# pfnet-research/superpixel-align

Hardware: AMD Instinct MI355X
Metric: images/sec superpixel-align labelling (1024x2048) (higher is better)
Workload: dtype f32 as 2 x f16 planes, f32 accumulate

## Files before the change

include/spalign.h:

```cpp
#ifndef SPALIGN_H
#define SPALIGN_H

#include <stddef.h>
#include <stdint.h>

#ifdef __cplusplus
extern "C" {
#endif

#define SPA_OK 0
#define SPA_ERR_ARG (-1)
#define SPA_ERR_HIP (-2)
#define SPA_ERR_NOGPU (-3)
#define SPA_ERR_LAYOUT (-4)
#define SPA_ERR_CAPACITY (-5)

#define SPA_ST_SLIC_EMPTY_SEGMENT 0x01u
#define SPA_ST_SLIC_UNCOVERED 0x02u
#define SPA_ST_CONN_OVERSIZE 0x04u
#define SPA_ST_POOL_SLOT_OVERFLOW 0x08u
#define SPA_ST_KMEANS_BARRIER 0x10u
#define SPA_ST_LABEL_RANGE 0x20u
#define SPA_ST_RNG_UNDERRUN 0x40u
#define SPA_ST_NP_SHUFFLE 0x80u

#define SPA_CELL_SLOTS 16

typedef struct spa_ctx spa_ctx;

int spa_version(void);
const char *spa_last_error(void);
int spa_ctx_create(int device, spa_ctx **out);
void spa_ctx_destroy(spa_ctx *ctx);
int spa_status(spa_ctx *ctx, uint32_t *status_host, void *stream);
int spa_status_peek_async(spa_ctx *ctx, uint32_t *status_pinned, void *stream);
int spa_status_take_async(spa_ctx *ctx, uint32_t *status_pinned, void *stream);

int spa_prof_enable(spa_ctx *ctx, int on);
int spa_prof_slots(void);
const char *spa_prof_name(int slot);
int spa_prof_read(spa_ctx *ctx, int slot, double *total_ms_host, int *launches_host);
int spa_debug_peek(spa_ctx *ctx, int which, size_t offset, size_t bytes, void *host);
int spa_ws_generation(spa_ctx *ctx);
int spa_debug_set(spa_ctx *ctx, int32_t key, int32_t value);
int spa_wino4_tile_decode(int32_t B, int32_t H, int32_t W, int32_t dilation, int32_t interleaved, int64_t t, int32_t *out);
int spa_debug_lds_probe(spa_ctx *ctx, float *out, int32_t n_wg, int32_t steps, int32_t mode, void *stream);

int spa_drn_normalise(spa_ctx *ctx, const float *x, int32_t B, int32_t H, int32_t W, void *out,
                      int32_t out_dtype, const double *mean3_host, const double *std3_host, void *stream);
int spa_bias_act(spa_ctx *ctx, void *y, int32_t dtype, int64_t rows, int32_t C, const void *bias,
                 const void *residual, int32_t relu, void *stream);
int spa_bias_act_amax(spa_ctx *ctx, float *y, int64_t rows, int32_t C, const float *bias,
                      const float *residual, int32_t relu, void *amax, void *stream);

int spa_drn_stem_d(spa_ctx *ctx, const float *x, int32_t B, int32_t H, int32_t W,
                   const float *w0, const float *b0, const float *w1, const float *b1,
                   const double *mean3_host, const double *std3_host, void *y, int32_t out_dtype,
                   float *xn_scratch, void *stream);

int spa_conv3x3_bf16(spa_ctx *ctx, const void *x, int32_t B, int32_t H, int32_t W, int32_t Cin,
                     const void *wt, int32_t Cout, const float *bias, const void *residual,
                     int32_t relu, int32_t dilation, void *y, void *stream);

int spa_conv_bf16_light(spa_ctx *ctx, const void *x, int32_t B, int32_t Hi, int32_t Wi, int32_t Cin, const void *wt,
                        int32_t taps, int32_t stride, int32_t Cout, const float *bias, const void *residual,
                        int32_t relu, int32_t dilation, void *y, void *stream);

int spa_conv3x3_f32(spa_ctx *ctx, const float *x, int32_t B, int32_t H, int32_t W, int32_t Cin,
                    const float *wt, int32_t Cout, const float *bias, const float *residual,
                    int32_t relu, int32_t dilation, float *y, void *stream);
int spa_conv1x1_f32(spa_ctx *ctx, const float *x, int32_t B, int32_t H, int32_t W, int32_t Cin,
                    const float *wt, int32_t Cout, const float *bias, const float *residual,
                    int32_t relu, float *y, void *stream);

int64_t spa_wino_tiles(int32_t B, int32_t H, int32_t W, int32_t dilation);
int spa_conv3x3_wino_f32(spa_ctx *ctx, const float *x, int32_t B, int32_t H, int32_t W, int32_t Cin,
                         const float *u, int32_t Cout, const float *bias, const float *residual,
                         int32_t relu, int32_t dilation, float *v_scratch, float *m_scratch, float *y,
                         void *stream);

int64_t spa_wino4_tiles(int32_t B, int32_t H, int32_t W, int32_t dilation);
int spa_conv3x3_wino4_f32(spa_ctx *ctx, const float *x, int32_t B, int32_t H, int32_t W, int32_t Cin,
                          const float *u, int32_t Cout, const float *bias, const float *residual,
                          int32_t relu, int32_t dilation, float *v_scratch, float *m_scratch, float *y,
                          void *stream);

int spa_amax_f32(spa_ctx *ctx, const float *x, int64_t n, void *amax, void *stream);
int spa_conv3x3_wino4_f16s(spa_ctx *ctx, const float *x, int32_t B, int32_t H, int32_t W, int32_t Cin,
                           const void *u2, const float *cs, int32_t Cout, const float *bias, const float *residual,
                           int32_t relu, int32_t dilation, const void *amax_in, void *amax_out, void *v_scratch,
                           float *m_scratch, float *y, void *stream);

int spa_conv3x3_f16s(spa_ctx *ctx, const float *x, int32_t B, int32_t H, int32_t W, int32_t Cin,
                     const void *wt2, float inv_t, int32_t Cout, const float *bias, const float *residual,
                     int32_t relu, int32_t dilation, const void *amax_in, void *amax_out, float *y, void *stream);
int spa_conv1x1_f16s(spa_ctx *ctx, const float *x, int32_t B, int32_t H, int32_t W, int32_t Cin,
                     const void *wt2, float inv_t, int32_t Cout, const float *bias, const float *residual,
                     int32_t relu, const void *amax_in, void *amax_out, float *y, void *stream);

int spa_conv3x3_s2_f16s(spa_ctx *ctx, const float *x, int32_t B, int32_t Hi, int32_t Wi, int32_t Cin,
                        const void *wt2, float inv_t, int32_t Cout, int32_t csplit, const float *bias,
                        int32_t relu, const void *amax_in, void *amax_out, float *y, float *y2, void *stream);
int spa_conv3x3_s2_f32(spa_ctx *ctx, const float *x, int32_t B, int32_t Hi, int32_t Wi, int32_t Cin,
                       const float *wt, int32_t Cout, int32_t csplit, const float *bias,
                       int32_t relu, float *y, float *y2, void *stream);

int spa_drn_stem_d_amax(spa_ctx *ctx, const float *x, int32_t B, int32_t H, int32_t W,
                        const float *w0, const float *b0, const float *w1, const float *b1,
                        const double *mean3_host, const double *std3_host, float *y,
                        float *xn_scratch, void *amax_out, void *stream);
int spa_drn_stem_c_amax(spa_ctx *ctx, const float *x, int32_t B, int32_t H, int32_t W,
                        const float *w0, const float *b0, const float *w1, const float *b1,
                        const double *mean3_host, const double *std3_host, float *y, float *y0,
                        float *xn_scratch, void *amax_out, void *stream);
int spa_drn_stem_c_bf16(spa_ctx *ctx, const float *x, int32_t B, int32_t H, int32_t W,
                        const float *w0, const float *b0, const float *w1, const float *b1,
                        const double *mean3_host, const double *std3_host, void *y, void *y0,
                        float *xn_scratch, void *stream);
int spa_conv_small_f16s(spa_ctx *ctx, const float *x, int32_t B, int32_t H, int32_t W, int32_t Cin, const void *wp,
                        float inv_t, int32_t Cout, int32_t stride, int32_t n_proj, const float *bias,
                        const float *residual, int32_t relu, const void *amax_in, void *amax_out, float *y, float *y2,
                        void *stream);
int spa_drn_layer2_f16s(spa_ctx *ctx, const float *x, int32_t B, int32_t H, int32_t W, const void *wp, float inv_t,
                        const float *bias, const void *amax_in, void *amax_out, float *y, void *stream);
int spa_drn_layer2_f32(spa_ctx *ctx, const float *x, int32_t B, int32_t H, int32_t W, const float *w9,
                       const float *bias, float *y, void *stream);

int spa_resize_bicubic_u8(spa_ctx *ctx, const uint8_t *src, int32_t B, int32_t H, int32_t W, int32_t C,
                          int32_t dst_h, int32_t dst_w, float *out, void *stream);
int spa_resize_cvcubic_u8(spa_ctx *ctx, const uint8_t *src, int32_t B, int32_t H, int32_t W, int32_t C,
                          int32_t dst_h, int32_t dst_w, float *out, void *stream);


typedef struct {
    int32_t n_centroids;
    int32_t grid_ny, grid_nx;
    int32_t start_y, start_x;
    int32_t step_y, step_x;
    int32_t win_step_y, win_step_x;
    float step;
    int32_t min_size, max_size;
    int32_t max_labels;
} spa_slic_plan;
int spa_slic_make_plan(int32_t H, int32_t W, int32_t n_segments, spa_slic_plan *plan_host);

int spa_rgb2lab(spa_ctx *ctx, const float *rgb, int32_t B, int32_t H, int32_t W,
                float ratio, float *lab, void *stream);

int spa_slic_core(spa_ctx *ctx, const float *lab, int32_t B, int32_t H, int32_t W,
                  int32_t n_segments, int32_t max_iter, int32_t *labels, float *centres,
                  void *stream);

int spa_enforce_connectivity(spa_ctx *ctx, const int32_t *labels_in, int32_t B, int32_t H,
                             int32_t W, int32_t min_size, int32_t max_size,
                             int32_t *labels_out, int32_t *n_labels, void *stream);

int spa_rgb2lab_u8_f64(spa_ctx *ctx, const float *rgb, int32_t B, int32_t H, int32_t W, double ratio,
                       double *lab, void *stream);
int spa_slic_core_f64(spa_ctx *ctx, const double *lab, int32_t B, int32_t H, int32_t W,
                      int32_t n_segments, int32_t max_iter, int32_t *labels, double *centres,
                      void *stream);
int spa_slic_u8(spa_ctx *ctx, const float *rgb, int32_t B, int32_t H, int32_t W, int32_t n_segments,
                double compactness, int32_t max_iter, int32_t *labels, int32_t *n_labels, void *stream);

int spa_slic(spa_ctx *ctx, const float *rgb, int32_t B, int32_t H, int32_t W,
             int32_t n_segments, float compactness, int32_t max_iter,
             int32_t *labels, int32_t *n_labels, void *stream);

int spa_felzenszwalb(spa_ctx *ctx, const float *rgb, int32_t B, int32_t H, int32_t W,
                     double scale, double sigma, int32_t min_size, int32_t *labels,
                     int32_t *n_labels, void *stream);

int spa_felzenszwalb_u8(spa_ctx *ctx, const float *rgb, int32_t B, int32_t H, int32_t W,
                        double scale, double sigma, int32_t min_size, int32_t *labels,
                        int32_t *n_labels, void *stream);


int spa_segment_offsets(spa_ctx *ctx, const int32_t *n_labels, int32_t B, int32_t *offsets,
                        void *stream);

int spa_segment_stats(spa_ctx *ctx, const int32_t *labels, int32_t B, int32_t H, int32_t W,
                      const int32_t *offsets, int32_t Ncap,
                      double y_rel_pos, double x_rel_pos, double y_rel_sigma, double x_rel_sigma,
                      int32_t *count, double *centroid, double *prior, void *stream);

typedef struct spa_pyrandom spa_pyrandom;
int spa_pyrandom_create(uint64_t seed, spa_pyrandom **out);
void spa_pyrandom_destroy(spa_pyrandom *rng);
int spa_pyrandom_shuffle_select_host(spa_pyrandom *rng, const int32_t *count_host, int32_t N,
                                     int32_t n_anchors, int32_t *ranks_host,
                                     int32_t *n_valid_host);
typedef struct spa_nprandom spa_nprandom;
int spa_nprandom_create(uint32_t seed, spa_nprandom **out);
void spa_nprandom_destroy(spa_nprandom *rng);
int spa_nprandom_shuffle_host(spa_nprandom *rng, int64_t *a_host, int64_t n);
int spa_nprandom_state(spa_nprandom *rng, uint32_t *state628_host);
int spa_nprandom_set_state(spa_nprandom *rng, const uint32_t *state628_host);
int spa_np_kmeans_init_dev(spa_ctx *ctx, void *state_dev, const double *w, const int32_t *n_ptr, int32_t Ncap,
                           int32_t k, const int32_t *gate, int64_t *init_other, int32_t *m_out, void *stream);
int spa_kmeans_retry_update(spa_ctx *ctx, const int32_t *assign, const int32_t *offsets, int32_t B, const int32_t *gate,
                            int32_t *pending, int32_t *made, uint8_t *fail_out, void *stream);

int spa_pyrandom_dev_seed(spa_ctx *ctx, uint64_t seed, void *stream);
int spa_pyrandom_dev_generate(spa_ctx *ctx, int64_t want, void *stream);
int spa_anchor_ranks_dev(spa_ctx *ctx, const int32_t *count, const int32_t *n_ptr, int32_t Ncap,
                         int32_t n_anchors, int64_t total_pixels, int32_t *ranks, int32_t *n_valid,
                         void *stream);

int spa_select_anchor_pixels(spa_ctx *ctx, const int32_t *labels, int32_t B, int32_t H,
                             int32_t W, const int32_t *offsets, int32_t Ncap,
                             const int32_t *ranks, const int32_t *n_valid, int32_t n_anchors,
                             int32_t *anchors, void *stream);

typedef struct {
    int32_t C, fh, fw;
    int64_t stride_b, stride_c, stride_y, stride_x;
    int32_t dtype;
} spa_fmap_desc;


int spa_pool_anchor(spa_ctx *ctx, const void *fmap, const spa_fmap_desc *desc,
                    int32_t B, int32_t img_h, const int32_t *offsets, int32_t Ncap,
                    const int32_t *anchors, const int32_t *n_valid, int32_t n_anchors,
                    int32_t n_neighbors, const double *centroid, int32_t append_pos,
                    void *X, int32_t x_dtype, int64_t ld, void *stream);

int spa_pool_mean(spa_ctx *ctx, const void *fmap, const spa_fmap_desc *desc,
                  const int32_t *labels, int32_t B, int32_t H, int32_t W,
                  const int32_t *offsets, int32_t Ncap, const int32_t *count,
                  int32_t sampling, const double *centroid, int32_t append_pos,
                  void *X, int32_t x_dtype, int64_t ld, void *stream);

int spa_kmeans_weighted(spa_ctx *ctx, const void *X, int32_t x_dtype, int64_t ld, int32_t D,
                        const double *w, const int32_t *n_ptr, int32_t Ncap, int32_t k,
                        int32_t max_iter, const int64_t *init_other, int32_t *assign,
                        int32_t *info, void *stream);
int spa_kmeans_weighted_gated(spa_ctx *ctx, const void *X, int32_t x_dtype, int64_t ld, int32_t D,
                              const double *w, const int32_t *n_ptr, int32_t Ncap, int32_t k,
                              int32_t max_iter, const int64_t *init_other, const int32_t *gate, int32_t *assign,
                              int32_t *info, void *stream);

int spa_paint(spa_ctx *ctx, const int32_t *labels, const int32_t *assign,
              const int32_t *offsets, int32_t B, int32_t H, int32_t W,
              uint8_t *cluster, uint8_t *road, void *stream);
// ... 129 lines not shown
```

superpixel-align_amd/_lib.py:

```python
import ctypes
import os
import subprocess

_HERE = os.path.dirname(os.path.abspath(__file__))
LIB_PATH = os.environ.get('SPA_LIB_PATH') or os.path.join(_HERE, 'libspalign.so')
_LIB = None

SPA_OK = 0
STATUS_BITS = {
    0x01: 'SLIC: a seed lost all of its pixels (NaN centre, dead for the rest of the sweeps, as in scikit-image)',
    0x02: 'SLIC: a pixel fell outside every 2S search window',
    0x04: 'connectivity: a component reached max_size (cut in BFS order by the exact replay path)',
    0x08: 'mean pooling: more than 16 superpixels touch one feature pixel',
    0x10: 'k-means: grid barrier timed out',
    0x20: 'a superpixel label outside [0, n_labels) was met',
    0x40: 'anchor selection: the device random stream ran dry',
    0x80: 'k-means initial assignment on the device: more than 65 536 points at or below the median weight',
}

INFO_BITS = 0x01 | 0x04

c_i32 = ctypes.c_int32
c_i64 = ctypes.c_int64
c_f32 = ctypes.c_float
c_f64 = ctypes.c_double
c_p = ctypes.c_void_p


class SlicPlan(ctypes.Structure):
    _fields_ = [('n_centroids', c_i32), ('grid_ny', c_i32), ('grid_nx', c_i32),
                ('start_y', c_i32), ('start_x', c_i32), ('step_y', c_i32), ('step_x', c_i32),
                ('win_step_y', c_i32), ('win_step_x', c_i32), ('step', c_f32),
                ('min_size', c_i32), ('max_size', c_i32), ('max_labels', c_i32)]


class FmapDesc(ctypes.Structure):
    _fields_ = [('C', c_i32), ('fh', c_i32), ('fw', c_i32),
                ('stride_b', c_i64), ('stride_c', c_i64), ('stride_y', c_i64), ('stride_x', c_i64),
                ('dtype', c_i32)]


PROTOTYPES = {
    'spa_version': (ctypes.c_int, []),
    'spa_last_error': (ctypes.c_char_p, []),
    'spa_ctx_create': (ctypes.c_int, [ctypes.c_int, ctypes.POINTER(c_p)]),
    'spa_ctx_destroy': (None, [c_p]),
    'spa_status': (ctypes.c_int, [c_p, ctypes.POINTER(ctypes.c_uint32), c_p]),
    'spa_status_peek_async': (ctypes.c_int, [c_p, c_p, c_p]),
    'spa_status_take_async': (ctypes.c_int, [c_p, c_p, c_p]),
    'spa_prof_enable': (ctypes.c_int, [c_p, ctypes.c_int]),
    'spa_prof_slots': (ctypes.c_int, []),
    'spa_prof_name': (ctypes.c_char_p, [ctypes.c_int]),
    'spa_prof_read': (ctypes.c_int, [c_p, ctypes.c_int, ctypes.POINTER(c_f64),
                                     ctypes.POINTER(ctypes.c_int)]),
    'spa_drn_normalise': (ctypes.c_int, [c_p, c_p, c_i32, c_i32, c_i32, c_p, c_i32, c_p, c_p, c_p]),
    'spa_bias_act': (ctypes.c_int, [c_p, c_p, c_i32, c_i64, c_i32, c_p, c_p, c_i32, c_p]),
    'spa_drn_stem_d': (ctypes.c_int, [c_p, c_p, c_i32, c_i32, c_i32, c_p, c_p, c_p, c_p, c_p, c_p, c_p, c_i32, c_p, c_p]),
    'spa_conv3x3_bf16': (ctypes.c_int, [c_p, c_p, c_i32, c_i32, c_i32, c_i32, c_p, c_i32, c_p, c_p, c_i32, c_i32, c_p, c_p]),
    'spa_conv_bf16_light': (ctypes.c_int, [c_p, c_p, c_i32, c_i32, c_i32, c_i32, c_p, c_i32, c_i32, c_i32, c_p, c_p, c_i32, c_i32, c_p, c_p]),
    'spa_conv3x3_f32': (ctypes.c_int, [c_p, c_p, c_i32, c_i32, c_i32, c_i32, c_p, c_i32, c_p, c_p, c_i32, c_i32, c_p, c_p]),
    'spa_conv1x1_f32': (ctypes.c_int, [c_p, c_p, c_i32, c_i32, c_i32, c_i32, c_p, c_i32, c_p, c_p, c_i32, c_p, c_p]),
    'spa_wino_tiles': (ctypes.c_int64, [c_i32, c_i32, c_i32, c_i32]),
    'spa_conv3x3_wino_f32': (ctypes.c_int, [c_p, c_p, c_i32, c_i32, c_i32, c_i32, c_p, c_i32, c_p, c_p, c_i32, c_i32, c_p, c_p, c_p, c_p]),
    'spa_wino4_tiles': (ctypes.c_int64, [c_i32, c_i32, c_i32, c_i32]),
    'spa_conv3x3_wino4_f32': (ctypes.c_int, [c_p, c_p, c_i32, c_i32, c_i32, c_i32, c_p, c_i32, c_p, c_p, c_i32, c_i32, c_p, c_p, c_p, c_p]),
    'spa_conv3x3_f16s': (ctypes.c_int, [c_p, c_p, c_i32, c_i32, c_i32, c_i32, c_p, c_f32, c_i32, c_p, c_p, c_i32, c_i32, c_p, c_p, c_p, c_p]),
    'spa_conv1x1_f16s': (ctypes.c_int, [c_p, c_p, c_i32, c_i32, c_i32, c_i32, c_p, c_f32, c_i32, c_p, c_p, c_i32, c_p, c_p, c_p, c_p]),
    'spa_conv3x3_s2_f16s': (ctypes.c_int, [c_p, c_p, c_i32, c_i32, c_i32, c_i32, c_p, c_f32, c_i32, c_i32, c_p, c_i32, c_p, c_p, c_p, c_p, c_p]),
    'spa_bias_act_amax': (ctypes.c_int, [c_p, c_p, c_i64, c_i32, c_p, c_p, c_i32, c_p, c_p]),
    'spa_drn_stem_d_amax': (ctypes.c_int, [c_p, c_p, c_i32, c_i32, c_i32, c_p, c_p, c_p, c_p, c_p, c_p, c_p, c_p, c_p, c_p]),
    'spa_drn_stem_c_amax': (ctypes.c_int, [c_p, c_p, c_i32, c_i32, c_i32, c_p, c_p, c_p, c_p, c_p, c_p, c_p, c_p, c_p, c_p, c_p]),
    'spa_drn_stem_c_bf16': (ctypes.c_int, [c_p, c_p, c_i32, c_i32, c_i32, c_p, c_p, c_p, c_p, c_p, c_p, c_p, c_p, c_p, c_p]),
    'spa_conv_small_f16s': (ctypes.c_int, [c_p, c_p, c_i32, c_i32, c_i32, c_i32, c_p, c_f32, c_i32, c_i32, c_i32, c_p, c_p, c_i32, c_p, c_p, c_p, c_p, c_p]),
    'spa_drn_layer2_f16s': (ctypes.c_int, [c_p, c_p, c_i32, c_i32, c_i32, c_p, c_f32, c_p, c_p, c_p, c_p, c_p]),
    'spa_drn_layer2_f32': (ctypes.c_int, [c_p, c_p, c_i32, c_i32, c_i32, c_p, c_p, c_p, c_p]),
    'spa_conv3x3_s2_f32': (ctypes.c_int, [c_p, c_p, c_i32, c_i32, c_i32, c_i32, c_p, c_i32, c_i32, c_p, c_i32, c_p, c_p, c_p]),
    'spa_amax_f32': (ctypes.c_int, [c_p, c_p, c_i64, c_p, c_p]),
    'spa_conv3x3_wino4_f16s': (ctypes.c_int, [c_p, c_p, c_i32, c_i32, c_i32, c_i32, c_p, c_p, c_i32, c_p, c_p, c_i32, c_i32, c_p, c_p, c_p, c_p, c_p, c_p]),
    'spa_resize_bicubic_u8': (ctypes.c_int, [c_p, c_p, c_i32, c_i32, c_i32, c_i32, c_i32, c_i32, c_p, c_p]),
    'spa_resize_cvcubic_u8': (ctypes.c_int, [c_p, c_p, c_i32, c_i32, c_i32, c_i32, c_i32, c_i32, c_p, c_p]),
    'spa_debug_peek': (ctypes.c_int, [c_p, ctypes.c_int, ctypes.c_size_t, ctypes.c_size_t, c_p]),
    'spa_debug_set': (ctypes.c_int, [c_p, ctypes.c_int32, ctypes.c_int32]),
    'spa_wino4_tile_decode': (ctypes.c_int, [c_i32, c_i32, c_i32, c_i32, c_i32, c_i64, ctypes.POINTER(ctypes.c_int32)]),
    'spa_ws_generation': (ctypes.c_int, [c_p]),
    'spa_debug_lds_probe': (ctypes.c_int, [c_p, c_p, c_i32, c_i32, c_i32, c_p]),
    'spa_slic_make_plan':(ctypes.c_int, [c_i32, c_i32, c_i32, ctypes.POINTER(SlicPlan)]),
    'spa_rgb2lab': (ctypes.c_int, [c_p, c_p, c_i32, c_i32, c_i32, c_f32, c_p, c_p]),
    'spa_slic_core': (ctypes.c_int, [c_p, c_p, c_i32, c_i32, c_i32, c_i32, c_i32, c_p, c_p, c_p]),
    'spa_enforce_connectivity': (ctypes.c_int, [c_p, c_p, c_i32, c_i32, c_i32, c_i32, c_i32, c_p,
                                                c_p, c_p]),
    'spa_slic': (ctypes.c_int, [c_p, c_p, c_i32, c_i32, c_i32, c_i32, c_f32, c_i32, c_p, c_p, c_p]),
    'spa_felzenszwalb': (ctypes.c_int, [c_p, c_p, c_i32, c_i32, c_i32, c_f64, c_f64, c_i32, c_p, c_p, c_p]),
    'spa_rgb2lab_u8_f64': (ctypes.c_int, [c_p, c_p, c_i32, c_i32, c_i32, c_f64, c_p, c_p]),
    'spa_slic_core_f64': (ctypes.c_int, [c_p, c_p, c_i32, c_i32, c_i32, c_i32, c_i32, c_p, c_p, c_p]),
    'spa_slic_u8': (ctypes.c_int, [c_p, c_p, c_i32, c_i32, c_i32, c_i32, c_f64, c_i32, c_p, c_p, c_p]),
    'spa_felzenszwalb_u8': (ctypes.c_int, [c_p, c_p, c_i32, c_i32, c_i32, c_f64, c_f64, c_i32, c_p, c_p, c_p]),
    'spa_overlap_refine': (ctypes.c_int, [c_p, c_p, c_p, c_i32, c_i64, c_i32, c_f64, c_p, c_p]),
    'spa_segment_offsets':(ctypes.c_int, [c_p, c_p, c_i32, c_p, c_p]),
    'spa_segment_stats': (ctypes.c_int, [c_p, c_p, c_i32, c_i32, c_i32, c_p, c_i32, c_f64, c_f64,
                                         c_f64, c_f64, c_p, c_p, c_p, c_p]),
    'spa_pyrandom_create': (ctypes.c_int, [ctypes.c_uint64, ctypes.POINTER(c_p)]),
    'spa_pyrandom_destroy': (None, [c_p]),
    'spa_pyrandom_shuffle_select_host': (ctypes.c_int, [c_p, c_p, c_i32, c_i32, c_p, c_p]),
    'spa_nprandom_create': (ctypes.c_int, [ctypes.c_uint32, ctypes.POINTER(c_p)]),
    'spa_nprandom_destroy': (None, [c_p]),
    'spa_nprandom_shuffle_host': (ctypes.c_int, [c_p, c_p, c_i64]),
    'spa_nprandom_state': (ctypes.c_int, [c_p, c_p]),
    'spa_nprandom_set_state': (ctypes.c_int, [c_p, c_p]),
    'spa_np_kmeans_init_dev': (ctypes.c_int, [c_p, c_p, c_p, c_p, c_i32, c_i32, c_p, c_p, c_p, c_p]),
    'spa_kmeans_retry_update': (ctypes.c_int, [c_p, c_p, c_p, c_i32, c_p, c_p, c_p, c_p, c_p]),
    'spa_pyrandom_dev_seed': (ctypes.c_int, [c_p, ctypes.c_uint64, c_p]),
    'spa_pyrandom_dev_generate': (ctypes.c_int, [c_p, c_i64, c_p]),
    'spa_anchor_ranks_dev': (ctypes.c_int, [c_p, c_p, c_p, c_i32, c_i32, c_i64, c_p, c_p, c_p]),
    'spa_select_anchor_pixels': (ctypes.c_int, [c_p, c_p, c_i32, c_i32, c_i32, c_p, c_i32, c_p, c_p,
                                                c_i32, c_p, c_p]),
    'spa_pool_anchor': (ctypes.c_int, [c_p, c_p, ctypes.POINTER(FmapDesc), c_i32, c_i32, c_p, c_i32,
                                       c_p, c_p, c_i32, c_i32, c_p, c_i32, c_p, c_i32, c_i64, c_p]),
    'spa_pool_mean': (ctypes.c_int, [c_p, c_p, ctypes.POINTER(FmapDesc), c_p, c_i32, c_i32, c_i32,
                                     c_p, c_i32, c_p, c_i32, c_p, c_i32, c_p, c_i32, c_i64, c_p]),
    'spa_kmeans_weighted': (ctypes.c_int, [c_p, c_p, c_i32, c_i64, c_i32, c_p, c_p, c_i32, c_i32,
                                           c_i32, c_p, c_p, c_p, c_p]),
    'spa_kmeans_weighted_gated': (ctypes.c_int, [c_p, c_p, c_i32, c_i64, c_i32, c_p, c_p, c_i32, c_i32,
                                                 c_i32, c_p, c_p, c_p, c_p, c_p]),
    'spa_paint': (ctypes.c_int, [c_p, c_p, c_p, c_p, c_i32, c_i32, c_i32, c_p, c_p, c_p]),
    'spa_confusion': (ctypes.c_int, [c_p, c_p, c_p, c_i32, c_i64, c_p, c_p]),
    'spa_png_deflate_u8': (ctypes.c_int, [c_p, c_p, c_i32, c_i32, c_i32, c_p, c_p, c_i32, c_i32, c_p, c_i64, c_p, c_p,
                                          c_p]),
    'spa_png_deflate_bound': (ctypes.c_int64, [c_i32, c_i32]),
    'spa_jpeg_encode_rgb8': (ctypes.c_int, [c_p, c_p, c_i32, c_i32, c_i32, c_i32, c_p, c_p, c_i64, c_p, c_p]),
    'spa_jpeg_scan_bound': (ctypes.c_int64, [c_i32, c_i32, c_i32]),
    'spa_figure_compose_u8': (ctypes.c_int, [c_p, c_p, c_i32, c_i32, c_i32, c_i32, c_p, c_p, c_p, c_i32, c_i32, c_i32, c_i32,
                                             c_p, c_i32, c_i32, c_p]),
    'spa_figure_canvas_shape': (ctypes.c_int, [c_i32, c_i32, c_i32, c_i32, c_i32, c_i32, ctypes.POINTER(c_i32),
                                               ctypes.POINTER(c_i32)]),
    'spa_segnet_encode': (ctypes.c_int, [c_p, c_p, c_i32, c_i32, c_i32, c_i32, c_i32, c_p, c_p, c_p, c_p, c_p, c_p, c_p]),
    'spa_segnet_decode': (ctypes.c_int, [c_p, c_p, c_p, c_i32, c_i32, c_i32, c_i32, c_p, c_p, c_p, c_p, c_p, c_p]),
    'spa_segnet_encode_bf16': (ctypes.c_int, [c_p, c_p, c_i32, c_i32, c_i32, c_i32, c_i32, c_p, c_p, c_p, c_p, c_p, c_p,
                                              c_p]),
    'spa_segnet_decode_bf16': (ctypes.c_int, [c_p, c_p, c_p, c_i32, c_i32, c_i32, c_i32, c_p, c_p, c_p, c_p, c_p, c_p]),
    'spa_segnet_encode_f16x3': (ctypes.c_int, [c_p, c_p, c_i32, c_i32, c_i32, c_i32, c_i32, c_p, c_p, c_p, c_p, c_p, c_p,
                                               c_p]),
    'spa_segnet_decode_f16x3': (ctypes.c_int, [c_p, c_p, c_p, c_i32, c_i32, c_i32, c_i32, c_p, c_p, c_p, c_p, c_p, c_p]),
    'spa_segnet_decode_logits': (ctypes.c_int, [c_p, c_p, c_p, c_i32, c_i32, c_i32, c_i32, c_p, c_p, c_p, c_p, c_p, c_p]),
    'spa_segnet_decode_logits_bf16': (ctypes.c_int, [c_p, c_p, c_p, c_i32, c_i32, c_i32, c_i32, c_p, c_p, c_p, c_p, c_p,
                                                     c_p]),
    'spa_segnet_decode_logits_f16x3': (ctypes.c_int, [c_p, c_p, c_p, c_i32, c_i32, c_i32, c_i32, c_p, c_p, c_p, c_p, c_p,
                                                      c_p]),
    'spa_segnet_overlay': (ctypes.c_int, [c_p, c_p, c_i32, c_i32, c_i32, c_i32, c_i32, c_p, c_p, c_f64, c_p, c_p, c_p]),
    'spa_segnet_score': (ctypes.c_int, [c_p, c_p, c_i32, c_i32, c_i32, c_i32, c_i32, c_p, c_p, c_p]),
    'spa_segnet_label_eval': (ctypes.c_int, [c_p, c_p, c_i32, c_i32, c_i32, c_i32, c_i32, c_p, c_p, c_p, c_p, c_p]),
    'spa_segnet_train_input': (ctypes.c_int, [c_p, c_p, c_i32, c_i32, c_i32, c_i32, c_i32, c_i32, c_p, c_p, c_i32, c_p,
                                              c_p, c_i32, c_p, c_p, c_p, c_p, c_p]),
    'spa_segnet_train_label': (ctypes.c_int, [c_p, c_p, c_i32, c_i32, c_i32, c_i32, c_i32, c_i32, c_i32, c_p, c_p, c_p,
                                              c_p, c_p]),
    'spa_segnet_train_input_ptrs': (ctypes.c_int, [c_p, c_p, c_i32, c_i32, c_i32, c_i32, c_i32, c_i32, c_p, c_p, c_i32,
                                                   c_p, c_p, c_i32, c_p, c_p, c_p, c_p, c_p]),
    'spa_segnet_train_label_ptrs': (ctypes.c_int, [c_p, c_p, c_i32, c_i32, c_i32, c_i32, c_i32, c_i32, c_i32, c_p, c_p,
                                                   c_p, c_p, c_p]),
    'spa_segnet_train_forward': (ctypes.c_int, [c_p, c_p, c_p, c_i32, c_i32, c_i32, c_i32, c_i32, c_p, c_p, c_p, c_p,
                                                c_p, c_p]),
    'spa_segnet_train_dgrad': (ctypes.c_int, [c_p, c_p, c_p, c_p, c_i32, c_i32, c_i32, c_p, c_p]),
    'spa_segnet_train_wgrad': (ctypes.c_int, [c_p, c_p, c_p, c_p, c_i32, c_i32, c_i32, c_i32, c_i32, c_p, c_p, c_p,
                                              c_p]),
    'spa_segnet_train_forward_bf16': (ctypes.c_int, [c_p, c_p, c_p, c_i32, c_i32, c_i32, c_i32, c_i32, c_p, c_p, c_p,
                                                     c_p, c_p, c_p]),
    'spa_segnet_train_dgrad_bf16': (ctypes.c_int, [c_p, c_p, c_p, c_p, c_i32, c_i32, c_i32, c_p, c_p]),
    'spa_segnet_train_wgrad_bf16': (ctypes.c_int, [c_p, c_p, c_p, c_p, c_i32, c_i32, c_i32, c_i32, c_i32, c_p, c_p,
                                                   c_p, c_p]),
    'spa_segnet_train_forward_f16x3': (ctypes.c_int, [c_p, c_p, c_p, c_i32, c_i32, c_i32, c_i32, c_i32, c_p, c_p, c_p,
                                                      c_p, c_p, c_p]),
    'spa_segnet_train_dgrad_f16x3': (ctypes.c_int, [c_p, c_p, c_p, c_p, c_i32, c_i32, c_i32, c_p, c_p]),
    'spa_segnet_train_wgrad_f16x3': (ctypes.c_int, [c_p, c_p, c_p, c_p, c_i32, c_i32, c_i32, c_i32, c_i32, c_p, c_p,
                                                    c_p, c_p]),
    'spa_segnet_train_bn_forward': (ctypes.c_int, [c_p, c_p, c_p, c_p, c_p, c_p, c_i32, c_i32, c_i32, c_p, c_p, c_p]),
    'spa_segnet_train_bn_backward_sums': (ctypes.c_int, [c_p, c_p, c_p, c_p, c_p, c_p, c_p, c_i32, c_i32, c_i32, c_p,
                                                         c_p]),
    'spa_segnet_train_bn_backward_dy': (ctypes.c_int, [c_p, c_p, c_p, c_p, c_p, c_p, c_p, c_p, c_p, c_f64, c_i32, c_i32,
                                                       c_i32, c_p, c_p]),
    'spa_segnet_train_classifier_forward': (ctypes.c_int, [c_p, c_p, c_p, c_p, c_i32, c_i32, c_i32, c_p, c_p]),
    'spa_segnet_train_classifier_backward': (ctypes.c_int, [c_p, c_p, c_p, c_p, c_i32, c_i32, c_i32, c_p, c_p, c_p,
                                                            c_p]),
}


class SpalignError(RuntimeError):
    pass


def build(force=False):
    csrc = os.path.join(_HERE, 'csrc')
    if force:
        subprocess.check_call(['make', '-s', '-C', csrc, 'clean'])
    subprocess.check_call(['make', '-s', '-j8', '-C', csrc])
    return LIB_PATH


def lib():
    global _LIB
    if _LIB is None:
        if not os.path.exists(LIB_PATH):
            raise SpalignError('%s is missing: run `python -c "import __graft_entry__ as g; '
                               'g.build()"` (there is no CPU fallback)' % LIB_PATH)
        import torch
        L = ctypes.CDLL(LIB_PATH)
        for name, (res, args) in PROTOTYPES.items():
            fn = getattr(L, name)
            fn.restype = res
            fn.argtypes = args
        _LIB = L
    return _LIB


def check(rc):
    if rc != SPA_OK:
        raise SpalignError('libspalign error %d: %s' % (rc, lib().spa_last_error().decode()))


def make_plan(H, W, n_segments):
    p = SlicPlan()
    check(lib().spa_slic_make_plan(H, W, n_segments, ctypes.byref(p)))
    return p
```

superpixel-align_amd/csrc/spa_common.h:

```cpp
#pragma once
#include <hip/hip_runtime.h>
#include <stdint.h>
#include <stdio.h>
#include <string.h>

#include "../../include/spalign.h"

#define SPA_WAVE 64

void spa_set_error(const char *fmt, ...);

#define SPA_HIP(call)                                                                  \
    do {                                                                               \
        hipError_t e_ = (call);                                                        \
        if (e_ != hipSuccess) {                                                        \
            spa_set_error("%s failed: %s (%s:%d)", #call, hipGetErrorString(e_),      \
                          __FILE__, __LINE__);                                         \
            return SPA_ERR_HIP;                                                        \
        }                                                                              \
    } while (0)

#define SPA_ARG(cond)                                                                  \
    do {                                                                               \
        if (!(cond)) {                                                                 \
            spa_set_error("invalid argument: %s (%s:%d)", #cond, __FILE__, __LINE__);  \
            return SPA_ERR_ARG;                                                        \
        }                                                                              \
    } while (0)

#define SPA_LAUNCH_CHECK()                                                             \
    do {                                                                               \
        hipError_t e_ = hipGetLastError();                                             \
        if (e_ != hipSuccess) {                                                        \
            spa_set_error("kernel launch failed: %s (%s:%d)", hipGetErrorString(e_),   \
                          __FILE__, __LINE__);                                         \
            return SPA_ERR_HIP;                                                        \
        }                                                                              \
    } while (0)

enum {
    WS_LAB = 0,
    WS_CENTRES,
    WS_PRE,
    WS_PARENT,
    WS_SIZE,
    WS_FINAL,
    WS_CLAIM,
    WS_QUEUE,
    WS_BLK,
    WS_SMALL,
    WS_CONNMISC,
    WS_BBOX,
    WS_CELLSLOT,
    WS_KM_PART,
    WS_KM_MISC,
    WS_NLABELS,
    WS_SBOX,
    WS_TODO,
    WS_ROWMASK,
    WS_FINEMASK,
    WS_SLIC_ORDER,
    WS_OVERLAP,
    WS_STEM_IN,
    WS_SRGB_LUT,
    WS_FZ_KEYS,
    WS_FZ_VALS,
    WS_FZ_STATE,
    WS_FZ_TMP,
    WS_STEM_WPACK,
    WS_ZERO_LINE,
    WS_RESIZE_TAB,
    WS_RESIZE_TMP,
    WS_RNG_STATE,
    WS_RNG_RING,
    WS_RNG_JBUF,
    WS_RNG_JOFF,
    WS_RUNS,
    WS_DEBUG,
    WS_SEGNET_BNPART,
    WS_SEGNET_WROT,
    WS_SEGNET_WGRAD,
    WS_SEGNET_WBF16,
    WS_SEGNET_WF16X3,
    WS_SEGNET_AMAX,
    WS_SEGNET_BNRED,
    WS_PNG_ROWS,
    WS_JPEG_INTERVALS,
    WS_COUNT
};

enum {
    PROF_RGB2LAB = 0, PROF_SLIC_ASSIGN, PROF_SLIC_UPDATE, PROF_CONNECT, PROF_STATS,
    PROF_CELL_WEIGHTS, PROF_POOL_MEAN, PROF_POOL_ANCHOR, PROF_KMEANS, PROF_PAINT,
    PROF_DRN_STEM, PROF_DRN_BIAS_ACT, PROF_DRN_CONV, PROF_DRN_CONV32, PROF_DRN_GEMM32, PROF_DRN_GEMM32_N, PROF_WINO_IN, PROF_WINO_OUT, PROF_DRN_GEMM16, PROF_DRN_GEMM16_N, PROF_DRN_CONV16, PROF_DRN_CONV16_128, PROF_DRN_CONV16_256, PROF_DRN_CONV16_1X1, PROF_DRN_CONV16_FRONT, PROF_DRN_CONV_LIGHT, PROF_SLOTS
};

struct spa_ctx {
    int device;
    int n_cu;
    uint32_t *d_status;
    unsigned status_takes;
    void *ws[WS_COUNT];
    size_t ws_bytes[WS_COUNT];
    int prof_on;
    hipEvent_t *prof_ev[PROF_SLOTS];
    int prof_cap[PROF_SLOTS], prof_used[PROF_SLOTS];
    hipStream_t aux[2];
    hipEvent_t ev_fork, ev_join[2];
    int aux_ready;
    int km_attr_done[2];
    int conn_attr_done;
    int conn_claim_ready;
    size_t conn_claim_bytes;
    int upd_wg_per_cu, upd_wg_per_cu8;
    int slic_force_general;
    int zero_line_ready, conv_attr_done, conv32_attr_done, fz_attr_done, gemm16_attr_done, gemm16s_attr_done, gemm16p_attr_done, nprng_attr_done;
    int rng_seeded;
    int ws_generation;
    int dbg_slic_ldsx;
    int convp_on;
    int wino_operands;
    int convs2_on;
    int convs2_attr_done;
    int rs_key[4], rs_ks[2];
};

#ifdef __HIPCC__
__device__ __forceinline__ unsigned spa_split16_pair(float x0, float x1, float sc, unsigned &l)
{
    unsigned h, lo;
    asm("v_fma_mixlo_f16 %0, %2, %4, 0 op_sel_hi:[0,0,0]\n\t"
        "v_fma_mixhi_f16 %0, %3, %4, 0 op_sel_hi:[0,0,0]\n\t"
        "v_fma_mixlo_f16 %1, %2, %4, -%0 op_sel_hi:[0,0,1]\n\t"
        "v_fma_mixhi_f16 %1, %3, %4, -%0 op_sel:[0,0,1] op_sel_hi:[0,0,1]"
        : "=&v"(h), "=&v"(lo) : "v"(x0), "v"(x1), "v"(sc));
    l = lo;
    return h;
}
#endif

int spa_aux_streams(spa_ctx *ctx);

void spa_prof_mark(spa_ctx *ctx, int slot, int end, hipStream_t s);
struct SpaProfScope {
    spa_ctx *c; int slot; hipStream_t s;
    SpaProfScope(spa_ctx *c_, int slot_, hipStream_t s_) : c(c_), slot(slot_), s(s_) { if (c->prof_on && slot >= 0) spa_prof_mark(c, slot, 0, s); }
    ~SpaProfScope() { if (c->prof_on && slot >= 0) spa_prof_mark(c, slot, 1, s); }
};

int spa_ws_reserve(spa_ctx *ctx, int which, size_t bytes, void **out);
void spa_zero_word(void *word, hipStream_t s);

static inline hipStream_t spa_stream(void *s) { return (hipStream_t)s; }

__device__ __forceinline__ double spa_det_log_pos(double x)
{
    unsigned long long b = (unsigned long long)__double_as_longlong(x);
    int e = (int)((b >> 52) & 0x7ff) - 1023;
    b = (b & 0x000fffffffffffffULL) | 0x3ff0000000000000ULL;
    double m = __longlong_as_double((long long)b);
    if (m > 1.4142135623730951) { m = m * 0.5; e += 1; }
    double s = (m - 1.0) / (m + 1.0);
    double z = s * s;
    double p = 1.0 / 25.0;
    p = p * z + 1.0 / 23.0;
    p = p * z + 1.0 / 21.0;
    p = p * z + 1.0 / 19.0;
    p = p * z + 1.0 / 17.0;
    p = p * z + 1.0 / 15.0;
    p = p * z + 1.0 / 13.0;
    p = p * z + 1.0 / 11.0;
    p = p * z + 1.0 / 9.0;
    p = p * z + 1.0 / 7.0;
    p = p * z + 1.0 / 5.0;
    p = p * z + 1.0 / 3.0;
    p = p * z + 1.0;
    double lnm = 2.0 * s * p;
    double ed = (double)e;
    return ed * 6.93147180369123816490e-01 + (ed * 1.90821492927058770002e-10 + lnm);
}

__device__ __forceinline__ double spa_det_exp(double t)
{
    double kf = floor(t * 1.44269504088896338700e+00 + 0.5);
    double r = (t - kf * 6.93147180369123816490e-01) - kf * 1.90821492927058770002e-10;
    double p = 1.0 / 87178291200.0;
    p = p * r + 1.0 / 6227020800.0;
    p = p * r + 1.0 / 479001600.0;
    p = p * r + 1.0 / 39916800.0;
    p = p * r + 1.0 / 3628800.0;
    p = p * r + 1.0 / 362880.0;
    p = p * r + 1.0 / 40320.0;
    p = p * r + 1.0 / 5040.0;
    p = p * r + 1.0 / 720.0;
    p = p * r + 1.0 / 120.0;
    p = p * r + 1.0 / 24.0;
    p = p * r + 1.0 / 6.0;
    p = p * r + 0.5;
    p = p * r + 1.0;
    p = p * r + 1.0;
    int k = (int)kf;
    unsigned long long b = (unsigned long long)(k + 1023) << 52;
    return p * __longlong_as_double((long long)b);
}

__device__ __forceinline__ unsigned spa_lane() { return __lane_id(); }
__device__ __forceinline__ unsigned spa_rank_in_mask(unsigned long long mask)
{
    return __builtin_amdgcn_mbcnt_hi((unsigned)(mask >> 32), __builtin_amdgcn_mbcnt_lo((unsigned)mask, 0u));
}
```

superpixel-align_amd/csrc/spa_conv32.hip:

```cpp
#include "spa_common.h"

typedef float f32x4 __attribute__((ext_vector_type(4)));
typedef float f32x8 __attribute__((ext_vector_type(8)));
typedef _Float16 f16x8 __attribute__((ext_vector_type(8)));

#define C32_BN 256
#define C32_BK 32
#define C32_THREADS 512
#define C32_TILE_BYTES (256 * C32_BK * 4)
#define C32_HALO 4
#define C32_XSEG_BYTES ((256 + 2 * C32_HALO) * C32_BK * 4)

template <int HAS_RES, int BM, int TAPS, int BN, bool SPLIT = false, int S = 1>
__global__ __launch_bounds__(C32_THREADS) void k_conv3x3_f32(const float *__restrict__ X, const float *__restrict__ Wt,
                                                             const float *__restrict__ bias,
                                                             const float *__restrict__ R, float *__restrict__ Y,
                                                             const char *__restrict__ zero_line, int B, int H, int W,
                                                             int Cin, int Cout, int dil, int relu, int xtiles,
                                                             int ntiles, int total_tiles, int zcount, long long xz,
                                                             long long wz, long long yz,
                                                             const unsigned *__restrict__ amax_in = nullptr,
                                                             unsigned *__restrict__ amax_out = nullptr, float inv_t = 1.f,
                                                             int Hi = 0, int Wi = 0, float *__restrict__ Y2 = nullptr, int csplit = 0)
{
// ... 349 lines not shown
        if (bm == 64 && bn == 256) {
            const int bit64 = TAPS == 9 ? 32 : 64;
            if (!(ctx->conv32_attr_done & bit64)) {
                SPA_HIP(hipFuncSetAttribute((const void *)k_conv3x3_f32<0, 64, TAPS, 256, true>, hipFuncAttributeMaxDynamicSharedMemorySize, 2 * 64 * 128 + 2 * (256 + 2 * C32_HALO) * 128));
                SPA_HIP(hipFuncSetAttribute((const void *)k_conv3x3_f32<1, 64, TAPS, 256, true>, hipFuncAttributeMaxDynamicSharedMemorySize, 2 * 64 * 128 + 2 * (256 + 2 * C32_HALO) * 128));
                ctx->conv32_attr_done |= bit64;
            }
            if (residual) C32_LAUNCH_S(1, 64, 256); else C32_LAUNCH_S(0, 64, 256);
            SPA_LAUNCH_CHECK();
            return SPA_OK;
        }
        SPA_ARG(bn == (bm == 256 ? 256 : 128));
        if (residual) { if (bm == 256) C32_LAUNCH_S(1, 256, 256); else if (bm == 128) C32_LAUNCH_S(1, 128, 128); else C32_LAUNCH_S(1, 64, 128); }
        else { if (bm == 256) C32_LAUNCH_S(0, 256, 256); else if (bm == 128) C32_LAUNCH_S(0, 128, 128); else C32_LAUNCH_S(0, 64, 128); }
        SPA_LAUNCH_CHECK();
        return SPA_OK;
    }
    if (residual) { if (bm == 256) C32_LAUNCH(1, 256, 256); else if (bm == 128) C32_LAUNCH(1, 128, 128); else C32_LAUNCH(1, 64, 128); }
    else { if (bm == 256) C32_LAUNCH(0, 256, 256); else if (bm == 128) C32_LAUNCH(0, 128, 128); else C32_LAUNCH(0, 64, 128); }
#undef C32_LAUNCH
    SPA_LAUNCH_CHECK();
    return SPA_OK;
}

extern "C" int spa_conv3x3_f32(spa_ctx *ctx, const float *x, int32_t B, int32_t H, int32_t W, int32_t Cin,
                               const float *wt, int32_t Cout, const float *bias, const float *residual,
                               int32_t relu, int32_t dilation, float *y, void *stream)
{
    return conv_f32_launch<9>(ctx, x, B, H, W, Cin, wt, Cout, bias, residual, relu, dilation, y, stream);
}

extern "C" int spa_conv1x1_f32(spa_ctx *ctx, const float *x, int32_t B, int32_t H, int32_t W, int32_t Cin,
                               const float *wt, int32_t Cout, const float *bias, const float *residual,
                               int32_t relu, float *y, void *stream)
{
    return conv_f32_launch<1>(ctx, x, B, H, W, Cin, wt, Cout, bias, residual, relu, 1, y, stream);
}

extern "C" int spa_conv3x3_f16s(spa_ctx *ctx, const float *x, int32_t B, int32_t H, int32_t W, int32_t Cin,
                                const void *wt2, float inv_t, int32_t Cout, const float *bias, const float *residual,
                                int32_t relu, int32_t dilation, const void *amax_in, void *amax_out, float *y, void *stream)
{
    SPA_ARG(amax_in);
    return conv_f32_launch<9>(ctx, x, B, H, W, Cin, (const float *)wt2, Cout, bias, residual, relu, dilation, y, stream, true, 1,
                              0, 0, 0, amax_in, amax_out, inv_t);
}

extern "C" int spa_conv1x1_f16s(spa_ctx *ctx, const float *x, int32_t B, int32_t H, int32_t W, int32_t Cin,
                                const void *wt2, float inv_t, int32_t Cout, const float *bias, const float *residual,
                                int32_t relu, const void *amax_in, void *amax_out, float *y, void *stream)
{
    SPA_ARG(amax_in);
    return conv_f32_launch<1>(ctx, x, B, H, W, Cin, (const float *)wt2, Cout, bias, residual, relu, 1, y, stream, true, 1,
                              0, 0, 0, amax_in, amax_out, inv_t);
}

bool conv3x3_s2_tile_takes(int32_t Cin, int32_t Cout, int32_t csplit, const float *y2);
int conv3x3_s2_tile_launch(spa_ctx *ctx, const float *x, int32_t B, int32_t Hi, int32_t Wi, int32_t Cin, const void *wt2, float inv_t,
                           int32_t csplit, const float *bias, int32_t relu, const void *amax_in, void *amax_out, float *y, float *y2,
                           hipStream_t s);

extern "C" int spa_conv3x3_s2_f16s(spa_ctx *ctx, const float *x, int32_t B, int32_t Hi, int32_t Wi, int32_t Cin,
                                   const void *wt2, float inv_t, int32_t Cout, int32_t csplit, const float *bias,
                                   int32_t relu, const void *amax_in, void *amax_out, float *y, float *y2, void *stream)
{
    SPA_ARG(ctx && x && wt2 && bias && y && amax_in && B > 0 && Hi > 0 && Wi > 0 && inv_t > 0.f);
    SPA_ARG(Cin % C32_BK == 0 && Cout % 128 == 0 && csplit % 64 == 0 && csplit > 0 && csplit <= Cout && (y2 || csplit == Cout));
    SPA_ARG(((uintptr_t)x % 16) == 0 && ((uintptr_t)wt2 % 16) == 0 && ((uintptr_t)y % 16) == 0 && ((uintptr_t)y2 % 16) == 0 && ((uintptr_t)bias % 16) == 0);
    hipStream_t s = spa_stream(stream);
    char *zero;
    int rc = spa_ws_reserve(ctx, WS_ZERO_LINE, 4096, (void **)&zero);
    if (rc != SPA_OK) return rc;
    if (!ctx->zero_line_ready) {
        SPA_HIP(hipMemsetAsync(zero, 0, 4096, s));
        ctx->zero_line_ready = 1;
    }
    if (amax_out) spa_zero_word(amax_out, s);
    if (ctx->convs2_on && conv3x3_s2_tile_takes(Cin, Cout, csplit, y2)) {
        SpaProfScope prof_(ctx, PROF_DRN_CONV16_FRONT, s);
        return conv3x3_s2_tile_launch(ctx, x, B, Hi, Wi, Cin, wt2, inv_t, csplit, bias, relu, amax_in, amax_out, y, y2, s);
    }
    const int H = (Hi + 1) / 2, W = (Wi + 1) / 2;
    const int bm = Cout % 256 == 0 ? 256 : 128, bn = 128;
    const int xtiles = (W + bn - 1) / bn, ntiles = Cout / bm;
    const long long total = (long long)B * H * xtiles * ntiles;
    SPA_ARG(total < (1ll << 31));
    SPA_ARG((long long)(2 * W + 1024) * Cin * 4 < (1ll << 31));
    const size_t lds = 2 * (size_t)bm * 128 + 2 * (size_t)(2 * bn + 2 * C32_HALO + 8) * 128;
    if (!(ctx->conv32_attr_done & 4)) {
        SPA_HIP(hipFuncSetAttribute((const void *)k_conv3x3_f32<0, 256, 9, 128, true, 2>, hipFuncAttributeMaxDynamicSharedMemorySize, 2 * 256 * 128 + 2 * (256 + 2 * C32_HALO + 8) * 128));
        SPA_HIP(hipFuncSetAttribute((const void *)k_conv3x3_f32<0, 128, 9, 128, true, 2>, hipFuncAttributeMaxDynamicSharedMemorySize, 2 * 128 * 128 + 2 * (256 + 2 * C32_HALO + 8) * 128));
        ctx->conv32_attr_done |= 4;
    }
    SpaProfScope prof_(ctx, PROF_DRN_CONV16_FRONT, s);
    const int per_cu = lds > 80 * 1024 ? 1 : (lds > 53 * 1024 ? 2 : 3);
    long long grid = (long long)ctx->n_cu * per_cu;
    if (grid > total) grid = total;
    if (bm == 256)
        hipLaunchKernelGGL((k_conv3x3_f32<0, 256, 9, 128, true, 2>), dim3((unsigned)grid), dim3(C32_THREADS), lds, s, x, (const float *)wt2, bias,
                           (const float *)nullptr, y, (const char *)zero, B, H, W, Cin, Cout, 1, relu, xtiles, ntiles, (int)total, 1, 0ll, 0ll, 0ll,
                           (const unsigned *)amax_in, (unsigned *)amax_out, inv_t, Hi, Wi, y2, csplit);
    else
        hipLaunchKernelGGL((k_conv3x3_f32<0, 128, 9, 128, true, 2>), dim3((unsigned)grid), dim3(C32_THREADS), lds, s, x, (const float *)wt2, bias,
                           (const float *)nullptr, y, (const char *)zero, B, H, W, Cin, Cout, 1, relu, xtiles, ntiles, (int)total, 1, 0ll, 0ll, 0ll,
                           (const unsigned *)amax_in, (unsigned *)amax_out, inv_t, Hi, Wi, y2, csplit);
    SPA_LAUNCH_CHECK();
    return SPA_OK;
}

extern "C" int spa_conv3x3_s2_f32(spa_ctx *ctx, const float *x, int32_t B, int32_t Hi, int32_t Wi, int32_t Cin,
                                  const float *wt, int32_t Cout, int32_t csplit, const float *bias,
                                  int32_t relu, float *y, float *y2, void *stream)
{
    SPA_ARG(ctx && x && wt && bias && y && B > 0 && Hi > 0 && Wi > 0);
    SPA_ARG(Cin % C32_BK == 0 && Cout % 128 == 0 && csplit % 64 == 0 && csplit > 0 && csplit <= Cout && (y2 || csplit == Cout));
    SPA_ARG(((uintptr_t)x % 16) == 0 && ((uintptr_t)wt % 16) == 0 && ((uintptr_t)y % 16) == 0 && ((uintptr_t)y2 % 16) == 0 && ((uintptr_t)bias % 16) == 0);
    hipStream_t s = spa_stream(stream);
    char *zero;
    int rc = spa_ws_reserve(ctx, WS_ZERO_LINE, 4096, (void **)&zero);
    if (rc != SPA_OK) return rc;
    if (!ctx->zero_line_ready) {
        SPA_HIP(hipMemsetAsync(zero, 0, 4096, s));
        ctx->zero_line_ready = 1;
    }
    const int H = (Hi + 1) / 2, W = (Wi + 1) / 2;
    const int bm = Cout % 256 == 0 ? 256 : 128, bn = 128;
    const int xtiles = (W + bn - 1) / bn, ntiles = Cout / bm;
    const long long total = (long long)B * H * xtiles * ntiles;
    SPA_ARG(total < (1ll << 31));
    SPA_ARG((long long)(2 * W + 1024) * Cin * 4 < (1ll << 31));
    const size_t lds = 2 * (size_t)bm * 128 + 2 * (size_t)(2 * bn + 2 * C32_HALO) * 128;
    if (!(ctx->conv32_attr_done & 128)) {
        SPA_HIP(hipFuncSetAttribute((const void *)k_conv3x3_f32<0, 256, 9, 128, false, 2>, hipFuncAttributeMaxDynamicSharedMemorySize, 2 * 256 * 128 + 2 * (256 + 2 * C32_HALO) * 128));
        SPA_HIP(hipFuncSetAttribute((const void *)k_conv3x3_f32<0, 128, 9, 128, false, 2>, hipFuncAttributeMaxDynamicSharedMemorySize, 2 * 128 * 128 + 2 * (256 + 2 * C32_HALO) * 128));
        ctx->conv32_attr_done |= 128;
    }
    SpaProfScope prof_(ctx, PROF_DRN_CONV32, s);
    const int per_cu = lds > 80 * 1024 ? 1 : (lds > 53 * 1024 ? 2 : 3);
    long long grid = (long long)ctx->n_cu * per_cu;
    if (grid > total) grid = total;
    if (bm == 256)
        hipLaunchKernelGGL((k_conv3x3_f32<0, 256, 9, 128, false, 2>), dim3((unsigned)grid), dim3(C32_THREADS), lds, s, x, wt, bias,
                           (const float *)nullptr, y, (const char *)zero, B, H, W, Cin, Cout, 1, relu, xtiles, ntiles, (int)total, 1, 0ll, 0ll, 0ll,
                           (const unsigned *)nullptr, (unsigned *)nullptr, 1.f, Hi, Wi, y2, csplit);
    else
        hipLaunchKernelGGL((k_conv3x3_f32<0, 128, 9, 128, false, 2>), dim3((unsigned)grid), dim3(C32_THREADS), lds, s, x, wt, bias,
                           (const float *)nullptr, y, (const char *)zero, B, H, W, Cin, Cout, 1, relu, xtiles, ntiles, (int)total, 1, 0ll, 0ll, 0ll,
                           (const unsigned *)nullptr, (unsigned *)nullptr, 1.f, Hi, Wi, y2, csplit);
    SPA_LAUNCH_CHECK();
    return SPA_OK;
}

int conv1x1_f32_raw(spa_ctx *ctx, const float *x, long long rows, int32_t Cin, const float *wt, int32_t Cout,
                    float *y, void *stream, int zcount)
{
    SPA_ARG(rows > 0 && rows % 256 == 0 && rows / 256 < (1ll << 31) && zcount >= 1);
    return conv_f32_launch<1>(ctx, x, 1, (int32_t)(rows / 256), 256, Cin, wt, Cout, nullptr, nullptr, 0, 1, y, stream, true,
                              zcount, rows * Cin, (long long)Cout * Cin, rows * Cout);
}
```

superpixel-align_amd/csrc/spa_ctx.hip:

```cpp
#include <math.h>
#include <stdarg.h>
#include <stdlib.h>

#include "spa_common.h"

static thread_local char g_err[512] = "";

void spa_set_error(const char *fmt, ...)
{
    va_list ap;
    va_start(ap, fmt);
    vsnprintf(g_err, sizeof(g_err), fmt, ap);
    va_end(ap);
}

extern "C" const char *spa_last_error(void) { return g_err; }
extern "C" int spa_version(void) { return 100; }

extern "C" int spa_ctx_create(int device, spa_ctx **out)
{
    SPA_ARG(out != nullptr);
    int n = 0;
    if (hipGetDeviceCount(&n) != hipSuccess || n <= 0) {
        spa_set_error("no HIP device visible: libspalign has no CPU fallback");
        return SPA_ERR_NOGPU;
    }
    if (device < 0) SPA_HIP(hipGetDevice(&device));
    SPA_ARG(device < n);
    SPA_HIP(hipSetDevice(device));
    hipDeviceProp_t prop;
    SPA_HIP(hipGetDeviceProperties(&prop, device));
    if (strncmp(prop.gcnArchName, "gfx950", 6) != 0) {
        spa_set_error("device %d is %s; libspalign is built for gfx950 (MI355X) only", device,
                      prop.gcnArchName);
        return SPA_ERR_NOGPU;
    }
    spa_ctx *ctx = (spa_ctx *)calloc(1, sizeof(spa_ctx));
    ctx->device = device;
    ctx->n_cu = prop.multiProcessorCount;
    if (const char *e = getenv("SPA_SLIC_GENERAL")) ctx->slic_force_general = atoi(e) != 0;
    ctx->convp_on = getenv("SPA_CONVP") ? atoi(getenv("SPA_CONVP")) != 0 : 1;
    ctx->convs2_on = 1;
    ctx->wino_operands = 2;
    SPA_HIP(hipMalloc((void **)&ctx->d_status, 32 * sizeof(uint32_t)));
    SPA_HIP(hipMemset(ctx->d_status, 0, 32 * sizeof(uint32_t)));
    *out = ctx;
    return SPA_OK;
}

extern "C" void spa_ctx_destroy(spa_ctx *ctx)
{
    if (!ctx) return;
    for (int i = 0; i < PROF_SLOTS; ++i) {
        for (int j = 0; j < ctx->prof_cap[i]; ++j) (void)hipEventDestroy(ctx->prof_ev[i][j]);
        free(ctx->prof_ev[i]);
    }
    for (int i = 0; i < WS_COUNT; ++i)
        if (ctx->ws[i]) (void)hipFree(ctx->ws[i]);
    if (ctx->d_status) (void)hipFree(ctx->d_status);
    if (ctx->aux_ready) {
        for (int i = 0; i < 2; ++i) { (void)hipStreamDestroy(ctx->aux[i]); (void)hipEventDestroy(ctx->ev_join[i]); }
        (void)hipEventDestroy(ctx->ev_fork);
    }
    free(ctx);
}

__global__ void k_zero_word(unsigned *w) { *w = 0u; }
void spa_zero_word(void *word, hipStream_t s) { hipLaunchKernelGGL(k_zero_word, dim3(1), dim3(1), 0, s, (unsigned *)word); }

int spa_ws_reserve(spa_ctx *ctx, int which, size_t bytes, void **out)
{
    if (bytes == 0) bytes = 16;
    if (ctx->ws_bytes[which] < bytes) {
        SPA_HIP(hipDeviceSynchronize());
        if (ctx->ws[which]) SPA_HIP(hipFree(ctx->ws[which]));
        ctx->ws[which] = nullptr;
        ctx->ws_bytes[which] = 0;
        size_t want = bytes + bytes / 8;
        SPA_HIP(hipMalloc(&ctx->ws[which], want));
        ctx->ws_bytes[which] = want;
        ++ctx->ws_generation;
    }
    *out = ctx->ws[which];
    return SPA_OK;
}

extern "C" int spa_status(spa_ctx *ctx, uint32_t *status_host, void *stream)
{
    SPA_ARG(ctx && status_host);
    hipStream_t s = spa_stream(stream);
    SPA_HIP(hipMemcpyAsync(status_host, ctx->d_status, sizeof(uint32_t), hipMemcpyDeviceToHost, s));
    SPA_HIP(hipMemsetAsync(ctx->d_status, 0, sizeof(uint32_t), s));
    SPA_HIP(hipStreamSynchronize(s));
    return SPA_OK;
}

extern "C" int spa_status_peek_async(spa_ctx *ctx, uint32_t *status_pinned, void *stream)
{
    SPA_ARG(ctx && status_pinned);
    SPA_HIP(hipMemcpyAsync(status_pinned, ctx->d_status, sizeof(uint32_t), hipMemcpyDeviceToHost, spa_stream(stream)));
    return SPA_OK;
}

__global__ void k_status_take(uint32_t *status, uint32_t *taken) { *taken = atomicExch(status, 0u); }

extern "C" int spa_status_take_async(spa_ctx *ctx, uint32_t *status_pinned, void *stream)
{
    SPA_ARG(ctx && status_pinned);
    uint32_t *slot = ctx->d_status + 16 + (ctx->status_takes++ & 15);
    hipLaunchKernelGGL(k_status_take, dim3(1), dim3(1), 0, spa_stream(stream), ctx->d_status, slot);
    SPA_HIP(hipMemcpyAsync(status_pinned, slot, sizeof(uint32_t), hipMemcpyDeviceToHost, spa_stream(stream)));
    return SPA_OK;
}

static int regular_grid_1hw(int64_t H, int64_t W, int64_t n_points, int64_t start[3],
                            int64_t step[3], int has_step[3])
{
    int64_t shape[3] = {1, H, W};
    int order[3] = {0, 1, 2};
    for (int i = 1; i < 3; ++i) {
        int o = order[i], j = i - 1;
        while (j >= 0 && shape[order[j]] > shape[o]) { order[j + 1] = order[j]; --j; }
        order[j + 1] = o;
    }
    double sorted[3];
    for (int i = 0; i < 3; ++i) sorted[i] = (double)shape[order[i]];
    double space = (double)H * (double)W;
    if (space <= (double)n_points) {
        for (int i = 0; i < 3; ++i) { start[i] = 0; step[i] = 1; has_step[i] = 0; }
        return 0;
    }
    double ss[3];
    ss[0] = ss[1] = ss[2] = pow(space / (double)n_points, 1.0 / 3.0);
    bool small = false;
    for (int i = 0; i < 3; ++i) small = small || (sorted[i] < ss[i]);
    if (small) {
        for (int dim = 0; dim < 3; ++dim) {
            ss[dim] = sorted[dim];
            double sp = 1.0;
            for (int j = dim + 1; j < 3; ++j) sp *= sorted[j];
            if (dim == 2) return -1;
            double v = pow(sp / (double)n_points, 1.0 / (double)(2 - dim));
            for (int j = dim + 1; j < 3; ++j) ss[j] = v;
            bool ok = true;
            for (int j = 0; j < 3; ++j) ok = ok && (sorted[j] >= ss[j]);
            if (ok) break;
        }
    }
    for (int p = 0; p < 3; ++p) {
        int d = order[p];
        start[d] = (int64_t)floor(ss[p] / 2.0);
        step[d] = (int64_t)nearbyint(ss[p]);
        has_step[d] = 1;
    }
    return 0;
}

static int64_t range_len(int64_t n, int64_t start, int64_t step)
{
    return start >= n ? 0 : (n - start + step - 1) / step;
}

extern "C" int spa_slic_make_plan(int32_t H, int32_t W, int32_t n_segments, spa_slic_plan *plan)
{
    SPA_ARG(plan && H > 0 && W > 0 && n_segments > 0);
    int64_t st[3], sp[3];
    int has[3];
    if (regular_grid_1hw(H, W, n_segments, st, sp, has) != 0) {
        spa_set_error("n_segments=%d too large for a %dx%d image", n_segments, H, W);
        return SPA_ERR_ARG;
    }
    int64_t ny = range_len(H, st[1], sp[1]), nx = range_len(W, st[2], sp[2]);
    SPA_ARG(ny > 0 && nx > 0);
    int64_t n = ny * nx;
    plan->n_centroids = (int32_t)n;
    plan->grid_ny = (int32_t)ny;
    plan->grid_nx = (int32_t)nx;
    plan->start_y = (int32_t)st[1];
    plan->start_x = (int32_t)st[2];
    plan->step_y = (int32_t)sp[1];
    plan->step_x = (int32_t)sp[2];
    double stmax = 1.0;
    if (has[1] && (double)sp[1] > stmax) stmax = (double)sp[1];
    if (has[2] && (double)sp[2] > stmax) stmax = (double)sp[2];
    plan->step = (float)stmax;
    int64_t st2[3], sp2[3];
    int has2[3];
    if (regular_grid_1hw(H, W, n, st2, sp2, has2) != 0) return SPA_ERR_ARG;
    plan->win_step_y = has2[1] ? (int32_t)sp2[1] : 1;
    plan->win_step_x = has2[2] ? (int32_t)sp2[2] : 1;
    double seg = ((double)H * (double)W) / (double)n;
    plan->min_size = (int32_t)(0.5 * seg);
    plan->max_size = (int32_t)(3.0 * seg);
    int64_t ml = plan->min_size > 0 ? ((int64_t)H * W) / plan->min_size + 1 : (int64_t)H * W;
    if (ml > (int64_t)H * W) ml = (int64_t)H * W;
    plan->max_labels = (int32_t)ml;
    return SPA_OK;
}

void spa_prof_mark(spa_ctx *ctx, int slot, int end, hipStream_t s)
{
    int idx = ctx->prof_used[slot] * 2 + end;
    if (idx >= ctx->prof_cap[slot]) {
        int ncap = ctx->prof_cap[slot] ? ctx->prof_cap[slot] * 2 : 256;
        ctx->prof_ev[slot] = (hipEvent_t *)realloc(ctx->prof_ev[slot], (size_t)ncap * sizeof(hipEvent_t));
        for (int j = ctx->prof_cap[slot]; j < ncap; ++j) (void)hipEventCreate(&ctx->prof_ev[slot][j]);
        ctx->prof_cap[slot] = ncap;
    }
    (void)hipEventRecord(ctx->prof_ev[slot][idx], s);
    if (end) ctx->prof_used[slot] += 1;
}

extern "C" int spa_prof_enable(spa_ctx *ctx, int on)
{
    SPA_ARG(ctx);
    ctx->prof_on = on ? 1 : 0;
    for (int i = 0; i < PROF_SLOTS; ++i) ctx->prof_used[i] = 0;
    return SPA_OK;
}

extern "C" int spa_prof_slots(void) { return PROF_SLOTS; }

extern "C" const char *spa_prof_name(int slot)
{
    static const char *names[PROF_SLOTS] = {"k_rgb2lab", "k_slic_assign", "k_slic_update",
        "connectivity(all)", "segment_stats(all)", "k_cell_weights", "k_pool_mean", "k_pool_anchor",
        "k_kmeans", "k_paint", "k_drn_stem_d(+normalise)", "k_bias_act(all)", "k_conv3x3_bf16(all)", "k_conv3x3_f32<taps 9>(all)", "k_conv3x3_f32<0, 256, 1, 256>", "k_conv3x3_f32<taps 1, narrow tiles>(all)", "k_wino_in", "k_wino_out", "k_gemm_f16x3_stag<256, 256>", "k_gemm_f16x3<128, 128>", "k_conv3x3_p16<64, 256> (split planes, 64-channel layers)", "k_conv3x3_p16<128, 128> (split planes, 128-channel layers)", "k_conv3x3_f32<split, 256-channel tile>", "k_conv3x3_f32<split, 1x1>", "split-plane front (stride-2 openers + projections, layer 2, DRN-C layers 1-2)", "k_conv_bf16_light(all)"};
    return (slot >= 0 && slot < PROF_SLOTS) ? names[slot] : "";
}

extern "C" int spa_prof_read(spa_ctx *ctx, int slot, double *total_ms, int *launches)
{
    SPA_ARG(ctx && total_ms && launches && slot >= 0 && slot < PROF_SLOTS);
    SPA_HIP(hipDeviceSynchronize());
    double t = 0.0;
    for (int j = 0; j < ctx->prof_used[slot]; ++j) {
        float ms = 0.0f;
        SPA_HIP(hipEventElapsedTime(&ms, ctx->prof_ev[slot][2 * j], ctx->prof_ev[slot][2 * j + 1]));
        t += ms;
    }
    *total_ms = t;
    *launches = ctx->prof_used[slot];
    return SPA_OK;
}

int spa_aux_streams(spa_ctx *ctx)
{
    if (ctx->aux_ready) return SPA_OK;
    int prio_lo = 0, prio_hi = 0;
    SPA_HIP(hipDeviceGetStreamPriorityRange(&prio_lo, &prio_hi));
    for (int i = 0; i < 2; ++i) {
        SPA_HIP(hipStreamCreateWithPriority(&ctx->aux[i], hipStreamNonBlocking, i == 1 ? prio_hi : prio_lo));
        SPA_HIP(hipEventCreateWithFlags(&ctx->ev_join[i], hipEventDisableTiming));
    }
    SPA_HIP(hipEventCreateWithFlags(&ctx->ev_fork, hipEventDisableTiming));
    ctx->aux_ready = 1;
    return SPA_OK;
}


typedef float dbg_f32x2 __attribute__((ext_vector_type(2)));
__global__ __launch_bounds__(256) void k_debug_lds_probe(float *__restrict__ out, int steps, int mode, float seed)
{
    __shared__ __attribute__((aligned(16))) float tab[32 * 32];
    __shared__ uint4 other[256 * 3];
    const int tid = threadIdx.x;
    other[tid * 3] = make_uint4(tid, blockIdx.x, 0u, 0u);
    for (int e = tid; e < steps * 32; e += 256) {
        const float t = seed * (float)(blockIdx.x % 977) - (float)(e & 31) * 1.25f - (float)(e >> 5);
        tab[e] = ((e * 7 + (int)blockIdx.x) % 11 == 0) ? INFINITY : t * t;
    }
    __syncthreads();
    dbg_f32x2 acc0 = {0.0f, 0.0f}, acc1 = {0.0f, 0.0f};
    float best[4] = {INFINITY, INFINITY, INFINITY, INFINITY};
    int bl[4] = {-1, -1, -1, -1};
    const float fy = (float)(tid >> 3);
#pragma unroll 1
    for (int jj = 0; jj < steps; ++jj) {
        const uint4 e0 = other[(jj * 3) % 768];
        const float *q = tab + jj * 32 + (mode == 2 ? 0 : (tid & 7) * 4);
        float4 d;
        if (mode == 1) { d.x = ((const volatile float *)q)[0]; d.y = ((const volatile float *)q)[1]; d.z = ((const volatile float *)q)[2]; d.w = ((const volatile float *)q)[3]; }
        else d = *(const float4 *)q;
        const float ty = (float)(e0.x & 31u) - fy;
        const float dy = (jj & 3) == 3 ? INFINITY : ty * ty;
        const dbg_f32x2 p0 = (dbg_f32x2{dy, dy} + dbg_f32x2{d.x, d.y}) * dbg_f32x2{0.37f, 0.37f} + acc0 * dbg_f32x2{0.001f, 0.001f};
        const dbg_f32x2 p1 = (dbg_f32x2{dy, dy} + dbg_f32x2{d.z, d.w}) * dbg_f32x2{0.37f, 0.37f} + acc1 * dbg_f32x2{0.001f, 0.001f};
        const float dd[4] = {p0.x, p0.y, p1.x, p1.y};
#pragma unroll
        for (int i = 0; i < 4; ++i) {
            const bool take = best[i] > dd[i];
            best[i] = take ? dd[i] : best[i];
            bl[i] = take ? jj : bl[i];
        }
        if (p0.x < 1e30f) acc0 = p0;
        if (p1.x < 1e30f) acc1 = p1;
    }
    float4 r = make_float4(best[0] + (float)bl[0], best[1] + (float)bl[1], best[2] + (float)bl[2], best[3] + (float)bl[3]);
    *(float4 *)(out + ((long long)blockIdx.x * 256 + tid) * 4) = r;
}

extern "C" int spa_debug_lds_probe(spa_ctx *ctx, float *out, int32_t n_wg, int32_t steps, int32_t mode, void *stream)
{
    SPA_ARG(ctx && out && n_wg > 0 && steps > 0 && steps <= 32 && mode >= 0 && mode <= 2);
    hipLaunchKernelGGL(k_debug_lds_probe, dim3((unsigned)n_wg), dim3(256), 0, spa_stream(stream), out, steps, mode, 0.731f);
    SPA_LAUNCH_CHECK();
    return SPA_OK;
}

extern "C" int spa_ws_generation(spa_ctx *ctx) { return ctx ? ctx->ws_generation : -1; }

extern "C" int spa_debug_set(spa_ctx *ctx, int32_t key, int32_t value)
{
    SPA_ARG(ctx && (key == 1 || key == 2 || key == 3 || key == 4) && (value == 0 || value == 1 || (key == 4 && value == 2)));
    if (key == 1) ctx->convp_on = value;
    else if (key == 4) ctx->wino_operands = value;
    else if (key == 3) ctx->convs2_on = value;
    else {
#ifdef SPA_DIAG
        ctx->dbg_slic_ldsx = value;
#else
        SPA_ARG(!"spa_debug_set key 2 (the reproducer variant of k_slic_assign) exists in diagnostic builds only: make EXTRA=-DSPA_DIAG");
#endif
    }
    return SPA_OK;
}

extern "C" int spa_debug_peek(spa_ctx *ctx, int which, size_t offset, size_t bytes, void *host)
{
    if (which == -1) which = WS_DEBUG;
    SPA_ARG(ctx && host && which >= 0 && which < WS_COUNT && offset + bytes <= ctx->ws_bytes[which]);
    SPA_HIP(hipDeviceSynchronize());
    SPA_HIP(hipMemcpy(host, (const char *)ctx->ws[which] + offset, bytes, hipMemcpyDeviceToHost));
    return SPA_OK;
}
```

superpixel-align_amd/csrc/spa_gemm16.hip:

```cpp
#include "spa_common.h"
#include "spa_wino_dev.h"

typedef _Float16 f16x8 __attribute__((ext_vector_type(8)));
typedef float f32x4 __attribute__((ext_vector_type(4)));
typedef float f32x8 __attribute__((ext_vector_type(8)));

#define G16_THREADS 512
__device__ __forceinline__ void g16_lds_barrier()
{
    __builtin_amdgcn_sched_barrier(0);
    asm volatile("s_waitcnt lgkmcnt(0)\n\ts_barrier" ::: "memory");
    __builtin_amdgcn_sched_barrier(0);
}

template <int BM, int BN>
__global__ __launch_bounds__(G16_THREADS, 2) void k_gemm_f16x3(const char *__restrict__ X, const char *__restrict__ Wt,
                                                            float *__restrict__ Y, int rows_per_z, int Cin, int Cout,
                                                            int ntiles, int total_tiles, int zcount, long long xz,
                                                            long long wz, long long yz, const unsigned *__restrict__ amax)
{
    extern __shared__ __attribute__((aligned(1024))) char lds16[];
    const int tid = threadIdx.x, lane = tid & 63;
    const int wave = __builtin_amdgcn_readfirstlane(tid >> 6);
    const long long all_tiles = (long long)zcount * total_tiles;
// ... 171 lines not shown
        const int nt = id % ntiles, pt = id / ntiles;
        zz = __builtin_amdgcn_readfirstlane(z);
        r0 = __builtin_amdgcn_readfirstlane(pt * BN);
        n0 = __builtin_amdgcn_readfirstlane(nt * BM);
        if (!PLANES) zscale_s = __uint_as_float(__builtin_amdgcn_readfirstlane(__float_as_uint(sb * __uint_as_float((unsigned)(127 - psum) << 23))));
    };
    constexpr int WN = 4;
    constexpr int MI = BM == 256 ? 8 : 4;
    constexpr int NJ = BN / WN / 16;
    constexpr int WROWS = MI * 16;
    constexpr int RS = 3;
    static_assert(BM / WROWS * WN == 8, "8 waves");
    static_assert(MI * NJ <= 63, "vmcnt range");
    static_assert(RS <= NJ && MI == 8, "split schedule: 4 element pairs over 8 groups of matrix instructions");

    char *wbuf = lds16, *xbuf = lds16 + 2 * (BM * 128);
    const int sub = lane >> 3, cs = lane & 7;
    const int chunk_byte = (cs ^ sub) << 4;
    const int nk = Cin / 32;
    const char *s_w = nullptr, *s_x = nullptr;
    const unsigned lane_off = (unsigned)((wave * 8 + sub) * Cin * 4 + chunk_byte);
    auto stage_bases = [&]() {
        s_w = Wt + ((long long)zz * wz + (long long)n0 * Cin) * 4;
        s_x = X + ((long long)zz * xz + (long long)r0 * Cin) * 4;
    };
    auto stage = [&](int t, int buf) {
        const char *wk = s_w + (long long)t * 128;
        char *dw = wbuf + buf * (BM * 128) + wave * 1024;
#pragma unroll
        for (int r = 0; r < BM / 64; ++r)
            __builtin_amdgcn_global_load_lds((const __attribute__((address_space(1))) void *)(wk + (long long)r * 64 * Cin * 4 + lane_off),
                                             (__attribute__((address_space(3))) void *)(dw + r * 8192), 16, 0, 0);
        const char *xk = s_x + (long long)t * 128;
        char *dx = xbuf + buf * (BN * 128) + wave * 1024;
#pragma unroll
        for (int r = 0; r < BN / 64; ++r)
            __builtin_amdgcn_global_load_lds((const __attribute__((address_space(1))) void *)(xk + (long long)r * 64 * Cin * 4 + lane_off),
                                             (__attribute__((address_space(3))) void *)(dx + r * 8192), 16, 0, 0);
    };
    const int wm = wave / WN, wn = wave % WN;
    const int frow = lane & 15, fk = lane >> 4;
    if ((int)blockIdx.x >= all_i) return;
    const int my_tiles = (all_i - (int)blockIdx.x + gstep - 1) / gstep;
    const int S = my_tiles * nk;

    int s_vid = (int)blockIdx.x, s_t = 0, s_q = 0;
    locate(s_vid);
    stage_bases();
    int c_r0 = r0, c_n0 = n0, c_z = zz, c_t = 0, c_vid = s_vid;
    float c_zscale = zscale_s;
    auto stage_next = [&]() {
        if (s_q < S) {
            stage(s_t, s_q & 1);
            ++s_q;
            if (++s_t == nk) { s_t = 0; s_vid += gstep; if (s_vid < all_i) { locate(s_vid); stage_bases(); } }
        }
    };
    stage_next();
    asm volatile("s_waitcnt vmcnt(0)" ::: "memory");
    g16_lds_barrier();
    if (late) g16_lds_barrier();
    bool stored = false;

    typedef unsigned u32x4 __attribute__((ext_vector_type(4)));
    f32x4 acc[MI][NJ];
#pragma unroll
    for (int i = 0; i < MI; ++i)
#pragma unroll
        for (int j = 0; j < NJ; ++j) acc[i][j] = (f32x4){0.f, 0.f, 0.f, 0.f};
    for (int q = 0; q < S; ++q) {
        const int buf = q & 1;
        stage_next();
        const char *lw = wbuf + buf * (BM * 128), *lx = xbuf + buf * (BN * 128);
        f16x8 wh[MI], wl[MI];
        f32x4 ra[NJ], rb[NJ];
#pragma unroll
        for (int i = 0; i < MI; ++i) {
            const int row = wm * WROWS + i * 16 + frow;
            wh[i] = *(const f16x8 *)(lw + row * 128 + ((fk ^ (row & 7)) << 4));
            wl[i] = *(const f16x8 *)(lw + row * 128 + (((4 + fk) ^ (row & 7)) << 4));
        }
#pragma unroll
        for (int j = 0; j < NJ; ++j) {
            const int row = wn * (NJ * 16) + j * 16 + frow;
            ra[j] = *(const f32x4 *)(lx + row * 128 + (((2 * fk) ^ (row & 7)) << 4));
            rb[j] = *(const f32x4 *)(lx + row * 128 + (((2 * fk + 1) ^ (row & 7)) << 4));
        }
        const float sc = c_zscale;
        u32x4 hu[NJ], lu[NJ];
        auto split_h = [&](int j, int e) {
            const float x0 = e < 2 ? ra[j][2 * e] : rb[j][2 * e - 4], x1 = e < 2 ? ra[j][2 * e + 1] : rb[j][2 * e - 3];
            hu[j][e] = wino_split_h(x0, x1, sc);
        };
        auto split_l = [&](int j, int e) {
            const float x0 = e < 2 ? ra[j][2 * e] : rb[j][2 * e - 4], x1 = e < 2 ? ra[j][2 * e + 1] : rb[j][2 * e - 3];
            lu[j][e] = wino_split_l(x0, x1, sc, hu[j][e]);
        };
        if (PLANES) {
#pragma unroll
            for (int j = 0; j < NJ; ++j) { hu[j] = __builtin_bit_cast(u32x4, ra[j]); lu[j] = __builtin_bit_cast(u32x4, rb[j]); }
        } else {
#pragma unroll
            for (int j = 0; j < RS; ++j)
#pragma unroll
                for (int e = 0; e < 4; ++e) { split_h(j, e); split_l(j, e); }
        }
        if (late) asm volatile("s_waitcnt vmcnt(0)" ::: "memory");
        g16_lds_barrier();
        float *const e_y = Y + (long long)c_z * yz + ((long long)c_r0 + wn * (NJ * 16) + (lane & 15)) * Cout + (c_n0 + wm * WROWS + (lane >> 4) * 4);
        auto store_acc = [&](int i, int j) {
            *(float4 *)(e_y + (long long)(j * 16) * Cout + i * 16) = make_float4(acc[i][j][0], acc[i][j][1], acc[i][j][2], acc[i][j][3]);
            acc[i][j] = (f32x4){0.f, 0.f, 0.f, 0.f};
        };
#pragma unroll
        for (int j = 0; j < NJ; ++j) {
            const f16x8 phj = __builtin_bit_cast(f16x8, hu[j]), plj = __builtin_bit_cast(f16x8, lu[j]);
#pragma unroll
            for (int i = 0; i < MI; ++i) {
                acc[i][j] = __builtin_amdgcn_mfma_f32_16x16x32_f16(wl[i], phj, acc[i][j], 0, 0, 0);
                acc[i][j] = __builtin_amdgcn_mfma_f32_16x16x32_f16(wh[i], plj, acc[i][j], 0, 0, 0);
                acc[i][j] = __builtin_amdgcn_mfma_f32_16x16x32_f16(wh[i], phj, acc[i][j], 0, 0, 0);
                if (!PLANES && j + RS < NJ) { if ((i & 1) == 0) split_h(j + RS, i >> 1); else split_l(j + RS, i >> 1); }
                __builtin_amdgcn_sched_barrier(0);
            }
        }
        if (++c_t == nk) {
#pragma unroll
            for (int j = 0; j < NJ; ++j)
#pragma unroll
                for (int i = 0; i < MI; ++i) store_acc(i, j);
            stored = true;
            c_t = 0; c_vid += gstep;
            if (c_vid < all_i) {
                const int sr0 = r0, sn0 = n0, sz = zz; const float szs = zscale_s;
                locate(c_vid);
                c_r0 = r0; c_n0 = n0; c_z = zz; c_zscale = zscale_s;
                r0 = sr0; n0 = sn0; zz = sz; zscale_s = szs;
            }
        }
        if (!late) {
            if (stored) asm volatile("s_waitcnt vmcnt(%0)" ::"n"(MI * NJ) : "memory");
            else asm volatile("s_waitcnt vmcnt(0)" ::: "memory");
            g16_lds_barrier();
        } else if (q + 1 < S) {
            g16_lds_barrier();
        }
        stored = false;
    }
}

int gemm_f16x3_tile(int32_t Cout) { return Cout % 256 == 0 ? 256 : 128; }

int gemm_f16x3_raw(spa_ctx *ctx, const float *x, long long rows, int32_t Cin, const void *wt, int32_t Cout, float *y,
                   void *stream, int zcount, const void *amax, int planes)
{
    SPA_ARG(ctx && x && wt && y && amax && rows > 0 && rows % 256 == 0 && rows < (1ll << 31) && zcount == 36);
    SPA_ARG(Cin % 32 == 0 && Cout % 128 == 0);
    SPA_ARG(((uintptr_t)x % 16) == 0 && ((uintptr_t)wt % 16) == 0 && ((uintptr_t)y % 16) == 0);
    hipStream_t s = spa_stream(stream);
    const int bm = gemm_f16x3_tile(Cout), bn = bm;
    SPA_ARG(!planes || bm == 256);
    const int ntiles = Cout / bm;
    const long long total = rows / bn * ntiles;
    SPA_ARG(total < (1ll << 31));
    const size_t lds = 2 * (size_t)(bm + bn) * 128;
    SpaProfScope prof_(ctx, bm == 256 ? PROF_DRN_GEMM16 : PROF_DRN_GEMM16_N, s);
    const int per_cu = lds > 80 * 1024 ? 1 : 2;
    long long grid = (long long)ctx->n_cu * per_cu;
    if (grid > total * zcount) grid = total * zcount;
    if (bm == 256) {
        if (!ctx->gemm16s_attr_done) {
            SPA_HIP(hipFuncSetAttribute((const void *)k_gemm_f16x3_stag<256, 256>, hipFuncAttributeMaxDynamicSharedMemorySize, 2 * 512 * 128));
            ctx->gemm16s_attr_done = 1;
        }
        if (planes) {
            if (!ctx->gemm16p_attr_done) {
                SPA_HIP(hipFuncSetAttribute((const void *)k_gemm_f16x3_stag<256, 256, true>, hipFuncAttributeMaxDynamicSharedMemorySize, 2 * 512 * 128));
                ctx->gemm16p_attr_done = 1;
            }
            hipLaunchKernelGGL((k_gemm_f16x3_stag<256, 256, true>), dim3((unsigned)grid), dim3(G16_THREADS), lds, s, (const char *)x, (const char *)wt, y,
                               (int)rows, Cin, Cout, ntiles, (int)total, zcount, rows * Cin, (long long)Cout * Cin, rows * Cout, (const unsigned *)amax);
        } else
        hipLaunchKernelGGL((k_gemm_f16x3_stag<256, 256>), dim3((unsigned)grid), dim3(G16_THREADS), lds, s, (const char *)x, (const char *)wt, y,
                           (int)rows, Cin, Cout, ntiles, (int)total, zcount, rows * Cin, (long long)Cout * Cin, rows * Cout, (const unsigned *)amax);
    } else {
        if (!ctx->gemm16_attr_done) {
            SPA_HIP(hipFuncSetAttribute((const void *)k_gemm_f16x3<128, 128>, hipFuncAttributeMaxDynamicSharedMemorySize, 2 * 256 * 128));
            ctx->gemm16_attr_done = 1;
        }
        hipLaunchKernelGGL((k_gemm_f16x3<128, 128>), dim3((unsigned)grid), dim3(G16_THREADS), lds, s, (const char *)x, (const char *)wt, y,
                           (int)rows, Cin, Cout, ntiles, (int)total, zcount, rows * Cin, (long long)Cout * Cin, rows * Cout, (const unsigned *)amax);
    }
    SPA_LAUNCH_CHECK();
    return SPA_OK;
}
```

superpixel-align_amd/csrc/spa_wino.hip:

```cpp
#include "spa_common.h"
#include "spa_wino_dev.h"

int conv1x1_f32_raw(spa_ctx *ctx, const float *x, long long rows, int32_t Cin, const float *wt, int32_t Cout,
                    float *y, void *stream, int zcount);

extern "C" int spa_wino4_tile_decode(int32_t B, int32_t H, int32_t W, int32_t dilation, int32_t interleaved, int64_t t, int32_t *out)
{
    SPA_ARG(out && B > 0 && H > 0 && W > 0 && dilation >= 1);
    WinoGeom g;
    wino4_geom(B, H, W, dilation, &g);
    SPA_ARG(t >= 0 && t < g.T);
    g.interleaved = interleaved != 0;
    wino_tile(g, t, out[0], out[1], out[2], out[3], out[4]);
    return SPA_OK;
}


__device__ __forceinline__ float4 f4add(float4 a, float4 b) { return make_float4(a.x + b.x, a.y + b.y, a.z + b.z, a.w + b.w); }
__device__ __forceinline__ float4 f4sub(float4 a, float4 b) { return make_float4(a.x - b.x, a.y - b.y, a.z - b.z, a.w - b.w); }

__device__ __forceinline__ long long wino_block()
{
    const long long nb = gridDim.x, id = blockIdx.x;
    const long long q = nb / 8, rem = nb % 8, xcd = id % 8, idx = id / 8;
    return (xcd < rem ? xcd * (q + 1) : rem * (q + 1) + (xcd - rem) * q) + idx;
}


__global__ __launch_bounds__(256) void k_wino_in(const float *__restrict__ X, float *__restrict__ V, WinoGeom g, int C,
                                                 long long Tpad)
{
    const int c4 = C >> 2;
    const long long id = wino_block() * 256 + threadIdx.x;
    if (id >= g.T * c4) return;
    const long long t = id / c4;
    const int c = (int)(id - t * c4) << 2;
    int b, sy, sx, ty, tx;
    wino_tile(g, t, b, sy, sx, ty, tx);
    float4 dv[4][4];
#pragma unroll
    for (int i = 0; i < 4; ++i) {
        const int y = sy + (2 * ty - 1 + i) * g.d;
#pragma unroll
        for (int j = 0; j < 4; ++j) {
            const int x = sx + (2 * tx - 1 + j) * g.d;
            const bool ok = y >= 0 && y < g.H && x >= 0 && x < g.W;
            dv[i][j] = ok ? *(const float4 *)(X + (((long long)b * g.H + y) * g.W + x) * C + c) : make_float4(0.f, 0.f, 0.f, 0.f);
        }
    }
    float4 r[4][4];
#pragma unroll
    for (int j = 0; j < 4; ++j) {
        r[0][j] = f4sub(dv[0][j], dv[2][j]);
        r[1][j] = f4add(dv[1][j], dv[2][j]);
        r[2][j] = f4sub(dv[2][j], dv[1][j]);
        r[3][j] = f4sub(dv[1][j], dv[3][j]);
    }
#pragma unroll
    for (int i = 0; i < 4; ++i) {
        const float4 v0 = f4sub(r[i][0], r[i][2]), v1 = f4add(r[i][1], r[i][2]);
        const float4 v2 = f4sub(r[i][2], r[i][1]), v3 = f4sub(r[i][1], r[i][3]);
        float *o = V + ((long long)(i * 4) * Tpad + t) * C + c;
        *(float4 *)(o) = v0;
        *(float4 *)(o + Tpad * C) = v1;
        *(float4 *)(o + 2 * Tpad * C) = v2;
        *(float4 *)(o + 3 * Tpad * C) = v3;
    }
}

template <int HAS_RES>
__global__ __launch_bounds__(256) void k_wino_out(const float *__restrict__ M, float *__restrict__ Y,
                                                  const float *__restrict__ bias, const float *__restrict__ R,
                                                  WinoGeom g, int K, long long Tpad, int relu)
{
    const int k4 = K >> 2;
    const long long id = wino_block() * 256 + threadIdx.x;
    if (id >= g.T * k4) return;
    const long long t = id / k4;
    const int k = (int)(id - t * k4) << 2;
    int b, sy, sx, ty, tx;
    wino_tile(g, t, b, sy, sx, ty, tx);
    float4 m[4][4];
#pragma unroll
    for (int i = 0; i < 4; ++i)
#pragma unroll
        for (int j = 0; j < 4; ++j) m[i][j] = *(const float4 *)(M + ((long long)(i * 4 + j) * Tpad + t) * K + k);
    float4 s[2][4];
#pragma unroll
    for (int j = 0; j < 4; ++j) {
        s[0][j] = f4add(f4add(m[0][j], m[1][j]), m[2][j]);
        s[1][j] = f4sub(f4sub(m[1][j], m[2][j]), m[3][j]);
    }
    const float4 bv = *(const float4 *)(bias + k);
#pragma unroll
    for (int i = 0; i < 2; ++i) {
        const int y = sy + (2 * ty + i) * g.d;
        if (y >= g.H) continue;
        const float4 o0 = f4add(f4add(s[i][0], s[i][1]), s[i][2]);
        const float4 o1 = f4sub(f4sub(s[i][1], s[i][2]), s[i][3]);
#pragma unroll
        for (int j = 0; j < 2; ++j) {
            const int x = sx + (2 * tx + j) * g.d;
            if (x >= g.W) continue;
            float4 v = f4add(j == 0 ? o0 : o1, bv);
            const long long off = (((long long)b * g.H + y) * g.W + x) * K + k;
            if (HAS_RES) v = f4add(v, *(const float4 *)(R + off));
            if (relu) { v.x = fmaxf(v.x, 0.f); v.y = fmaxf(v.y, 0.f); v.z = fmaxf(v.z, 0.f); v.w = fmaxf(v.w, 0.f); }
            *(float4 *)(Y + off) = v;
        }
    }
}

static void wino_geom(int B, int H, int W, int d, WinoGeom *g)
{
    g->B = B; g->H = H; g->W = W; g->d = d; g->interleaved = wino_interleave(d);
    const int hs = (H + d - 1) / d, ws = (W + d - 1) / d;
    g->th = (hs + 1) / 2; g->tw = (ws + 1) / 2;
    g->T = (long long)B * d * d * g->th * g->tw;
}

extern "C" int64_t spa_wino_tiles(int32_t B, int32_t H, int32_t W, int32_t dilation)
{
    WinoGeom g;
    wino_geom(B, H, W, dilation, &g);
    return (g.T + 255) / 256 * 256;
}

extern "C" int spa_conv3x3_wino_f32(spa_ctx *ctx, const float *x, int32_t B, int32_t H, int32_t W, int32_t Cin,
                                    const float *u, int32_t Cout, const float *bias, const float *residual,
                                    int32_t relu, int32_t dilation, float *v_scratch, float *m_scratch, float *y,
                                    void *stream)
{
    SPA_ARG(ctx && x && u && bias && y && v_scratch && m_scratch && B > 0 && H > 0 && W > 0 && dilation >= 1);
    SPA_ARG(Cin % 32 == 0 && Cout % 64 == 0);
    SPA_ARG((((uintptr_t)x | (uintptr_t)u | (uintptr_t)y | (uintptr_t)bias | (uintptr_t)residual | (uintptr_t)v_scratch |
              (uintptr_t)m_scratch) % 16) == 0);
    hipStream_t s = spa_stream(stream);
    WinoGeom g;
    wino_geom(B, H, W, dilation, &g);
    g.interleaved = ctx->wino_operands >= 1 && wino_interleave(dilation);
    const long long Tpad = (g.T + 255) / 256 * 256;
    SPA_ARG(g.T * (Cin > Cout ? Cin : Cout) / 4 < (1ll << 31) * 256);
    {
        SpaProfScope prof_(ctx, PROF_WINO_IN, s);
        const long long n = g.T * (Cin / 4);
        hipLaunchKernelGGL(k_wino_in, dim3((unsigned)((n + 255) / 256)), dim3(256), 0, s, x, v_scratch, g, Cin, Tpad);
    }
    {
        int rc = conv1x1_f32_raw(ctx, v_scratch, Tpad, Cin, u, Cout, m_scratch, stream, 16);
        if (rc != SPA_OK) return rc;
    }
    {
        SpaProfScope prof_(ctx, PROF_WINO_OUT, s);
        const long long n = g.T * (Cout / 4);
        if (residual)
            hipLaunchKernelGGL(k_wino_out<1>, dim3((unsigned)((n + 255) / 256)), dim3(256), 0, s, (const float *)m_scratch, y,
                               bias, residual, g, Cout, Tpad, relu);
        else
            hipLaunchKernelGGL(k_wino_out<0>, dim3((unsigned)((n + 255) / 256)), dim3(256), 0, s, (const float *)m_scratch, y,
                               bias, residual, g, Cout, Tpad, relu);
    }
    SPA_LAUNCH_CHECK();
    return SPA_OK;
}



template <typename V, bool PLANES = false>
__global__ __launch_bounds__(256) void k_wino4_in(const float *__restrict__ X, float *__restrict__ Vout, WinoGeom g, int C,
                                                  long long Tpad, const unsigned *__restrict__ amax = nullptr)
{
    constexpr int VN = sizeof(V) / 4;
    const int c2 = C / VN;
    const long long id = wino_block() * 256 + threadIdx.x;
    if (id >= g.T * c2) return;
    const long long t = id / c2;
    const int c = (int)(id - t * c2) * VN;
    int b, sy, sx, ty, tx;
    wino_tile(g, t, b, sy, sx, ty, tx);
    V r[6][6];
#pragma unroll
    for (int a = 0; a < 6; ++a) {
        const int y = sy + (4 * ty - 1 + a) * g.d;
        V dv[6];
#pragma unroll
        for (int j = 0; j < 6; ++j) {
            const int x = sx + (4 * tx - 1 + j) * g.d;
            const bool ok = y >= 0 && y < g.H && x >= 0 && x < g.W;
            dv[j] = ok ? *(const V *)(X + (((long long)b * g.H + y) * g.W + x) * C + c) : wino_zero<V>();
        }
        wino4_bt(dv, r[a]);
    }
#pragma unroll
    for (int j = 0; j < 6; ++j) {
        const V col[6] = {r[0][j], r[1][j], r[2][j], r[3][j], r[4][j], r[5][j]};
        V o[6];
        wino4_bt(col, o);
#pragma unroll
        for (int i = 0; i < 6; ++i) {
            if constexpr (PLANES) {
                static_assert(sizeof(V) == 16, "a thread owns half an 8-channel chunk");
                const float sc = wino_pow2(14 - wino_amax_exp(*amax) - wino4_psum(i * 6 + j));
                const unsigned h0 = wino_split_h(o[i].x, o[i].y, sc), h1 = wino_split_h(o[i].z, o[i].w, sc);
                const unsigned l0 = wino_split_l(o[i].x, o[i].y, sc, h0), l1 = wino_split_l(o[i].z, o[i].w, sc, h1);
                const bool odd = (c >> 2) & 1;
                const unsigned r0 = wino_lane_swap(odd ? h0 : l0), r1 = wino_lane_swap(odd ? h1 : l1);
                float *chunk = Vout + ((long long)(i * 6 + j) * Tpad + t) * C + (c & ~7);
                *((uint4 *)chunk + (odd ? 1 : 0)) = odd ? make_uint4(r0, r1, l0, l1) : make_uint4(h0, h1, r0, r1);
            } else {
                *(V *)(Vout + ((long long)(i * 6 + j) * Tpad + t) * C + c) = o[i];
            }
        }
    }
}

template <int HAS_RES, typename V>
__global__ __launch_bounds__(256) void k_wino4_out(const float *__restrict__ M, float *__restrict__ Y,
                                                   const float *__restrict__ bias, const float *__restrict__ R,
                                                   WinoGeom g, int K, long long Tpad, int relu)
{
    constexpr int VN = sizeof(V) / 4;
    const int k2 = K / VN;
    const long long id = wino_block() * 256 + threadIdx.x;
    if (id >= g.T * k2) return;
    const long long t = id / k2;
    const int k = (int)(id - t * k2) * VN;
    int b, sy, sx, ty, tx;
    wino_tile(g, t, b, sy, sx, ty, tx);
    V s[4][6];
#pragma unroll
    for (int j = 0; j < 6; ++j) {
        V col[6];
#pragma unroll
        for (int i = 0; i < 6; ++i) col[i] = *(const V *)(M + ((long long)(i * 6 + j) * Tpad + t) * K + k);
        V o[4];
        wino4_at(col, o);
#pragma unroll
        for (int i = 0; i < 4; ++i) s[i][j] = o[i];
    }
    const V bv = *(const V *)(bias + k);
#pragma unroll
    for (int i = 0; i < 4; ++i) {
        const int y = sy + (4 * ty + i) * g.d;
        V o[4];
        wino4_at(s[i], o);
        if (y >= g.H) continue;
#pragma unroll
        for (int j = 0; j < 4; ++j) {
            const int x = sx + (4 * tx + j) * g.d;
            if (x >= g.W) continue;
            V v = o[j] + bv;
            const long long off = (((long long)b * g.H + y) * g.W + x) * K + k;
            if (HAS_RES) v = v + *(const V *)(R + off);
            if (relu) v = wino_relu(v);
            *(V *)(Y + off) = v;
        }
    }
}


__global__ __launch_bounds__(256) void k_amax(const float4 *__restrict__ x, long long n4, unsigned *__restrict__ amax)
{
    __shared__ unsigned red[4];
    unsigned m = 0;
    for (long long i = (long long)blockIdx.x * 256 + threadIdx.x; i < n4; i += (long long)gridDim.x * 256) {
        const float4 v = x[i];
        m = max(max(m, __float_as_uint(v.x) & 0x7fffffffu), max(__float_as_uint(v.y) & 0x7fffffffu,
                max(__float_as_uint(v.z) & 0x7fffffffu, __float_as_uint(v.w) & 0x7fffffffu)));
    }
    for (int o = 32; o > 0; o >>= 1) m = max(m, (unsigned)__shfl_xor((int)m, o));
    if ((threadIdx.x & 63) == 0) red[threadIdx.x >> 6] = m;
    __syncthreads();
    if (threadIdx.x == 0) {
        m = max(max(red[0], red[1]), max(red[2], red[3]));
        if (m > *(volatile unsigned *)amax) atomicMax(amax, m);
    }
}

template <int HAS_RES, typename V = float4>
__global__ __launch_bounds__(256, 2) void k_wino4_out_s(const float *__restrict__ M, float *__restrict__ Y,
                                                     const float *__restrict__ bias, const float *__restrict__ R,
                                                     WinoGeom g, int K, long long Tpad, int relu, WinoScale cs,
                                                     const unsigned *__restrict__ amax_in, unsigned *__restrict__ amax_out)
{
    constexpr int VN = sizeof(V) / 4;
    const int k2 = K / VN;
    const long long id = wino_block() * 256 + threadIdx.x;
    unsigned mx = 0;
    if (id < g.T * k2) {
        const long long t = id / k2;
        const int k = (int)(id - t * k2) * VN;
        int b, sy, sx, ty, tx;
        wino_tile(g, t, b, sy, sx, ty, tx);
        const float inv = wino_pow2(wino_amax_exp(*amax_in) - 14);
        V s[4][6];
#pragma unroll
        for (int j = 0; j < 6; ++j) {
            V col[6];
#pragma unroll
            for (int i = 0; i < 6; ++i)
                col[i] = (cs.c[i * 6 + j] * inv) * wino_nt_load((const V *)(M + ((long long)(i * 6 + j) * Tpad + t) * K + k));
            V o[4];
            wino4_at(col, o);
#pragma unroll
            for (int i = 0; i < 4; ++i) s[i][j] = o[i];
        }
        const V bv = *(const V *)(bias + k);
#pragma unroll
        for (int i = 0; i < 4; ++i) {
            const int y = sy + (4 * ty + i) * g.d;
            V o[4];
            wino4_at(s[i], o);
            if (y >= g.H) continue;
#pragma unroll
            for (int j = 0; j < 4; ++j) {
                const int x = sx + (4 * tx + j) * g.d;
                if (x >= g.W) continue;
                V v = o[j] + bv;
                const long long off = (((long long)b * g.H + y) * g.W + x) * K + k;
                if (HAS_RES) v = v + *(const V *)(R + off);
                if (relu) v = wino_relu(v);
                *(V *)(Y + off) = v;
                mx = max(mx, wino_absmax_bits(v));
            }
        }
    }
    if (amax_out) {
        for (int o = 32; o > 0; o >>= 1) mx = max(mx, (unsigned)__shfl_xor((int)mx, o));
        if ((threadIdx.x & 63) == 0 && mx > *(volatile unsigned *)amax_out) atomicMax(amax_out, mx);
    }
}

extern "C" int64_t spa_wino4_tiles(int32_t B, int32_t H, int32_t W, int32_t dilation)
{
    WinoGeom g;
    wino4_geom(B, H, W, dilation, &g);
    return (g.T + 255) / 256 * 256;
}

extern "C" int spa_conv3x3_wino4_f32(spa_ctx *ctx, const float *x, int32_t B, int32_t H, int32_t W, int32_t Cin,
                                     const float *u, int32_t Cout, const float *bias, const float *residual,
                                     int32_t relu, int32_t dilation, float *v_scratch, float *m_scratch, float *y,
                                     void *stream)
{
    SPA_ARG(ctx && x && u && bias && y && v_scratch && m_scratch && B > 0 && H > 0 && W > 0 && dilation >= 1);
    SPA_ARG(Cin % 32 == 0 && Cout % 64 == 0);
    SPA_ARG((((uintptr_t)x | (uintptr_t)u | (uintptr_t)y | (uintptr_t)bias | (uintptr_t)residual | (uintptr_t)v_scratch |
              (uintptr_t)m_scratch) % 16) == 0);
    hipStream_t s = spa_stream(stream);
    WinoGeom g;
    wino4_geom(B, H, W, dilation, &g);
    g.interleaved = ctx->wino_operands >= 1 && wino_interleave(dilation);
    const long long Tpad = (g.T + 255) / 256 * 256;
    SPA_ARG(g.T * (Cin > Cout ? Cin : Cout) / 2 < (1ll << 31) * 256);
    {
        SpaProfScope prof_(ctx, PROF_WINO_IN, s);
        const long long n = g.T * (Cin / 4);
        hipLaunchKernelGGL((k_wino4_in<float4, false>), dim3((unsigned)((n + 255) / 256)), dim3(256), 0, s, x, v_scratch, g, Cin, Tpad,
                           (const unsigned *)nullptr);
    }
    {
        int rc = conv1x1_f32_raw(ctx, v_scratch, Tpad, Cin, u, Cout, m_scratch, stream, 36);
        if (rc != SPA_OK) return rc;
    }
    {
        SpaProfScope prof_(ctx, PROF_WINO_OUT, s);
        const long long n = g.T * (Cout / 4);
        if (residual)
            hipLaunchKernelGGL((k_wino4_out<1, float4>), dim3((unsigned)((n + 255) / 256)), dim3(256), 0, s, (const float *)m_scratch, y,
                               bias, residual, g, Cout, Tpad, relu);
        else
            hipLaunchKernelGGL((k_wino4_out<0, float4>), dim3((unsigned)((n + 255) / 256)), dim3(256), 0, s, (const float *)m_scratch, y,
                               bias, residual, g, Cout, Tpad, relu);
    }
    SPA_LAUNCH_CHECK();
    return SPA_OK;
}

int gemm_f16x3_raw(spa_ctx *ctx, const float *x, long long rows, int32_t Cin, const void *wt, int32_t Cout, float *y,
                   void *stream, int zcount, const void *amax, int planes);
int gemm_f16x3_tile(int32_t Cout);

extern "C" int spa_amax_f32(spa_ctx *ctx, const float *x, int64_t n, void *amax, void *stream)
{
    SPA_ARG(ctx && x && amax && n > 0 && n % 4 == 0 && ((uintptr_t)x % 16) == 0);
    hipStream_t s = spa_stream(stream);
    spa_zero_word(amax, s);
    long long blocks = (n / 4 + 255) / 256;
    if (blocks > 4096) blocks = 4096;
    hipLaunchKernelGGL(k_amax, dim3((unsigned)blocks), dim3(256), 0, s, (const float4 *)x, (long long)(n / 4), (unsigned *)amax);
    SPA_LAUNCH_CHECK();
    return SPA_OK;
}

extern "C" int spa_conv3x3_wino4_f16s(spa_ctx *ctx, const float *x, int32_t B, int32_t H, int32_t W, int32_t Cin,
                                      const void *u2, const float *cs, int32_t Cout, const float *bias,
                                      const float *residual, int32_t relu, int32_t dilation, const void *amax_in,
                                      void *amax_out, void *v_scratch, float *m_scratch, float *y, void *stream)
{
    SPA_ARG(ctx && x && u2 && cs && bias && y && v_scratch && m_scratch && amax_in && B > 0 && H > 0 && W > 0 && dilation >= 1);
    SPA_ARG(Cin % 32 == 0 && Cout % 128 == 0);
    SPA_ARG((((uintptr_t)x | (uintptr_t)u2 | (uintptr_t)y | (uintptr_t)bias | (uintptr_t)residual | (uintptr_t)v_scratch |
              (uintptr_t)m_scratch) % 16) == 0);
    hipStream_t s = spa_stream(stream);
    WinoGeom g;
    wino4_geom(B, H, W, dilation, &g);
    g.interleaved = ctx->wino_operands >= 1 && wino_interleave(dilation);
    const int planes = ctx->wino_operands >= 2 && gemm_f16x3_tile(Cout) == 256 && Cout >= 512;
    const long long Tpad = (g.T + 255) / 256 * 256;
    SPA_ARG(g.T * (Cin > Cout ? Cin : Cout) / 4 < (1ll << 31) * 256);
    WinoScale sc;
    for (int i = 0; i < 36; ++i) sc.c[i] = cs[i];
    if (amax_out) spa_zero_word(amax_out, s);
    {
        SpaProfScope prof_(ctx, PROF_WINO_IN, s);
        const long long n = g.T * (Cin / 4);
        if (planes)
            hipLaunchKernelGGL((k_wino4_in<float4, true>), dim3((unsigned)((n + 255) / 256)), dim3(256), 0, s, x, (float *)v_scratch, g, Cin, Tpad,
                               (const unsigned *)amax_in);
        else
            hipLaunchKernelGGL((k_wino4_in<float4, false>), dim3((unsigned)((n + 255) / 256)), dim3(256), 0, s, x, (float *)v_scratch, g, Cin, Tpad,
                               (const unsigned *)nullptr);
    }
    {
        int rc = gemm_f16x3_raw(ctx, (const float *)v_scratch, Tpad, Cin, u2, Cout, m_scratch, stream, 36, amax_in, planes);
        if (rc != SPA_OK) return rc;
    }
    {
        SpaProfScope prof_(ctx, PROF_WINO_OUT, s);
        const long long n = g.T * (Cout / 4);
        if (residual)
            hipLaunchKernelGGL((k_wino4_out_s<1>), dim3((unsigned)((n + 255) / 256)), dim3(256), 0, s, (const float *)m_scratch, y,
                               bias, residual, g, Cout, Tpad, relu, sc, (const unsigned *)amax_in, (unsigned *)amax_out);
        else
            hipLaunchKernelGGL((k_wino4_out_s<0>), dim3((unsigned)((n + 255) / 256)), dim3(256), 0, s, (const float *)m_scratch, y,
                               bias, residual, g, Cout, Tpad, relu, sc, (const unsigned *)amax_in, (unsigned *)amax_out);
    }
    SPA_LAUNCH_CHECK();
    return SPA_OK;
}
```

superpixel-align_amd/csrc/spa_wino_dev.h:

```cpp
#pragma once
#include "spa_common.h"

struct WinoGeom { int B, H, W, d, th, tw; long long T; int interleaved; };
typedef float wino_v4 __attribute__((ext_vector_type(4)));
__device__ __forceinline__ float4 wino_nt_load(const float4 *p) { const wino_v4 v = __builtin_nontemporal_load((const wino_v4 *)p); return make_float4(v[0], v[1], v[2], v[3]); }

__host__ __device__ __forceinline__ void wino_tile(const WinoGeom &g, long long t, int &b, int &sy, int &sx, int &ty, int &tx)
{
    if (g.interleaved) {
        const int rw = g.tw * g.d;
        const int gx = (int)(t % rw); t /= rw;
        sx = gx % g.d; tx = gx / g.d;
        ty = (int)(t % g.th); t /= g.th;
        sy = (int)(t % g.d);
        b = (int)(t / g.d);
        return;
    }
    tx = (int)(t % g.tw); t /= g.tw;
    ty = (int)(t % g.th); t /= g.th;
    sx = (int)(t % g.d); t /= g.d;
    sy = (int)(t % g.d);
    b = (int)(t / g.d);
}

__device__ __forceinline__ unsigned wino_absmax_bits(float4 v) { return max(max(__float_as_uint(v.x) & 0x7fffffffu, __float_as_uint(v.y) & 0x7fffffffu), max(__float_as_uint(v.z) & 0x7fffffffu, __float_as_uint(v.w) & 0x7fffffffu)); }
__device__ __forceinline__ float4 operator+(float4 a, float4 b) { return make_float4(a.x + b.x, a.y + b.y, a.z + b.z, a.w + b.w); }
__device__ __forceinline__ float4 operator-(float4 a, float4 b) { return make_float4(a.x - b.x, a.y - b.y, a.z - b.z, a.w - b.w); }
__device__ __forceinline__ float4 operator*(float s, float4 a) { return make_float4(s * a.x, s * a.y, s * a.z, s * a.w); }
template <typename V> __device__ __forceinline__ V wino_zero();
template <> __device__ __forceinline__ float4 wino_zero<float4>() { return make_float4(0.f, 0.f, 0.f, 0.f); }
__device__ __forceinline__ float4 wino_relu(float4 v) { return make_float4(fmaxf(v.x, 0.f), fmaxf(v.y, 0.f), fmaxf(v.z, 0.f), fmaxf(v.w, 0.f)); }

template <typename V>
__device__ __forceinline__ void wino4_bt(const V (&x)[6], V (&y)[6])
{
    y[0] = 2.0f * (x[0] + x[4]) + 3.0f * (x[3] - x[1]) - 4.0f * x[2];
    y[1] = 2.0f * (x[4] - x[1]) + x[2] + 5.0f * x[3];
    y[2] = 5.0f * x[2] - 2.0f * (x[1] + x[4]) - x[3];
    y[3] = 2.0f * (x[1] - x[3]) + x[2] - x[4];
    y[4] = (x[1] - x[3]) + 2.0f * (x[4] - x[2]);
    y[5] = 2.0f * (x[1] + x[5]) + 3.0f * (x[4] - x[2]) - 4.0f * x[3];
}

template <typename V>
__device__ __forceinline__ void wino4_at(const V (&x)[6], V (&y)[4])
{
    y[0] = ((x[0] + x[1]) + x[2]) + (x[3] + x[4]);
    y[1] = (x[1] - x[2]) + (0.5f * x[3] - 2.0f * x[4]);
    y[2] = (x[1] + x[2]) + (0.25f * x[3] + 4.0f * x[4]);
    y[3] = ((x[1] - x[2]) + (0.125f * x[3] - 8.0f * x[4])) + x[5];
}

struct WinoScale { float c[36]; };

__device__ __forceinline__ int wino_amax_exp(unsigned bits)
{
    int e = (int)(bits >> 23) - 127;
    e = e < -100 ? -100 : (e > 100 ? 100 : e);
    return bits == 0u ? 0 : e;
}
__device__ __forceinline__ float wino_pow2(int k) { return __uint_as_float((unsigned)(127 + k) << 23); }

__device__ __forceinline__ unsigned wino_split_h(float x0, float x1, float sc)
{
    unsigned h;
    asm volatile("v_fma_mixlo_f16 %0, %1, %3, 0 op_sel_hi:[0,0,0]\n\t"
                 "v_fma_mixhi_f16 %0, %2, %3, 0 op_sel_hi:[0,0,0]"
                 : "=&v"(h) : "v"(x0), "v"(x1), "s"(sc));
    return h;
}
__device__ __forceinline__ unsigned wino_split_l(float x0, float x1, float sc, unsigned h)
{
    unsigned l;
    asm volatile("v_fma_mixlo_f16 %0, %1, %3, -%4 op_sel_hi:[0,0,1]\n\t"
                 "v_fma_mixhi_f16 %0, %2, %3, -%4 op_sel:[0,0,1] op_sel_hi:[0,0,1]"
                 : "=&v"(l) : "v"(x0), "v"(x1), "s"(sc), "v"(h));
    return l;
}
__device__ __forceinline__ unsigned wino_lane_swap(unsigned v)
{
    return (unsigned)__builtin_amdgcn_update_dpp(0, (int)v, 0xB1 , 0xF, 0xF, false);
}
__host__ __device__ __forceinline__ int wino4_psum(int z)
{
    const int zi = z / 6, zj = z - zi * 6;
    return ((0x433444 >> (4 * zi)) & 15) + ((0x433444 >> (4 * zj)) & 15);
}

static inline int wino_interleave(int d) { return d > 2; }

static inline void wino4_geom(int B, int H, int W, int d, WinoGeom *g)
{
    g->B = B; g->H = H; g->W = W; g->d = d; g->interleaved = wino_interleave(d);
    const int hs = (H + d - 1) / d, ws = (W + d - 1) / d;
    g->th = (hs + 3) / 4; g->tw = (ws + 3) / 4;
    g->T = (long long)B * d * d * g->th * g->tw;
}
```

superpixel-align_amd/engine.py:

```python
import ctypes

import numpy as np
import torch

from . import _lib
from ._lib import FmapDesc, SpalignError, check


def _ptr(t):
    return ctypes.c_void_p(t.data_ptr()) if t is not None else ctypes.c_void_p(0)


def _stream(device=None):
    return ctypes.c_void_p(torch.cuda.current_stream(device).cuda_stream)


def _req(t, dtype, what):
    if not (isinstance(t, torch.Tensor) and t.is_cuda and t.dtype == dtype and t.is_contiguous()):
        raise SpalignError('%s must be a contiguous CUDA tensor of dtype %s' % (what, dtype))
    return t


def _out(out, shape, dtype, device):
    if out is None:
        return torch.empty(shape, dtype=dtype, device=device, memory_format=torch.channels_last)
    if not (out.is_cuda and out.dtype == dtype and tuple(out.shape) == tuple(shape) and out.is_contiguous(memory_format=torch.channels_last)):
        raise SpalignError('out must be a channels-last CUDA tensor of dtype %s and shape %s' % (dtype, tuple(shape)))
    return out


def _scratch(scratch, v_shape, m_shape, device):
    if scratch is None:
        return (torch.empty(v_shape, dtype=torch.float32, device=device), torch.empty(m_shape, dtype=torch.float32, device=device))
    v, m = scratch
    for t, shape in ((v, v_shape), (m, m_shape)):
        if not (t.is_cuda and t.dtype == torch.float32 and tuple(t.shape) == tuple(shape) and t.is_contiguous()):
            raise SpalignError('scratch must be two contiguous float32 CUDA tensors of shapes %s, %s' % (v_shape, m_shape))
    return v, m


class Engine(object):

    def __init__(self, device=None):
        if not torch.cuda.is_available():
            raise SpalignError('no GPU visible: the superpixel-align hot path has no CPU fallback')
        self.device = torch.device('cuda', torch.cuda.current_device() if device is None else device)
        self._lib = _lib.lib()
        h = ctypes.c_void_p()
        check(self._lib.spa_ctx_create(self.device.index, ctypes.byref(h)))
        self._ctx = h
        self._in_tables = {}
        self._stream_own = {}

    def _s(self):
        return _stream(self.device)

    def close(self):
        if getattr(self, '_ctx', None):
            self._lib.spa_ctx_destroy(self._ctx)
            self._ctx = None

    def __del__(self):
        try:
            self.close()
        except Exception:
            pass

    def status(self):
        v = ctypes.c_uint32(0)
        check(self._lib.spa_status(self._ctx, ctypes.byref(v), self._s()))
        return v.value

    def status_peek_async(self, word=None):
        if word is None:
            word = torch.zeros(1, dtype=torch.int32).pin_memory()
        check(self._lib.spa_status_peek_async(self._ctx, ctypes.c_void_p(word.data_ptr()), self._s()))
        return word

    def status_take_async(self, word=None):
        if word is None:
            word = torch.zeros(1, dtype=torch.int32).pin_memory()
        check(self._lib.spa_status_take_async(self._ctx, ctypes.c_void_p(word.data_ptr()), self._s()))
        return word

    def raise_on_word(self, word, ignore=_lib.INFO_BITS):
        st = int(word.item()) & 0xffffffff
        self.last_info = st & _lib.INFO_BITS
        st &= ~ignore
        if st:
            self.status()
            msgs = [m for bit, m in _lib.STATUS_BITS.items() if st & bit]
            raise SpalignError('device status 0x%x: %s' % (st, '; '.join(msgs)))

    def raise_on_status(self, ignore=_lib.INFO_BITS):
        st = self.status()
        self.last_info = st & _lib.INFO_BITS
        st &= ~ignore
        if st:
            msgs = [m for bit, m in _lib.STATUS_BITS.items() if st & bit]
            raise SpalignError('device status 0x%x: %s' % (st, '; '.join(msgs)))

    def ws_generation(self):
        return int(self._lib.spa_ws_generation(self._ctx))

    def debug_set(self, key, value):
        check(self._lib.spa_debug_set(self._ctx, int(key), int(value)))
        self.__dict__.setdefault('_debug', {})[int(key)] = int(value)

    def debug_get(self, key, default):
        return self.__dict__.get('_debug', {}).get(int(key), default)

    def prof_enable(self, on=True):
        check(self._lib.spa_prof_enable(self._ctx, 1 if on else 0))
        self._prof_on = bool(on)

    def prof_is_on(self):
        return bool(getattr(self, '_prof_on', False))

    def prof_read(self):
        out = {}
        for slot in range(self._lib.spa_prof_slots()):
            ms, n = ctypes.c_double(0), ctypes.c_int(0)
            check(self._lib.spa_prof_read(self._ctx, slot, ctypes.byref(ms), ctypes.byref(n)))
            if n.value:
                out[self._lib.spa_prof_name(slot).decode()] = (ms.value, n.value)
        return out

    def drn_normalise(self, x, dtype=torch.float32):
        x = _req(x, torch.float32, 'x')
        B, C, H, W = x.shape
        assert C == 3
        out = torch.empty((B, 3, H, W), dtype=dtype, device=x.device, memory_format=torch.channels_last)
        mean = (ctypes.c_double * 3)(0.485, 0.456, 0.406)
        std = (ctypes.c_double * 3)(0.229, 0.224, 0.225)
        check(self._lib.spa_drn_normalise(self._ctx, _ptr(x), B, H, W, _ptr(out),
                                          0 if dtype == torch.float32 else 1, mean, std, self._s()))
        return out

    def drn_stem_d(self, x, w0, b0, w1p, b1, dtype=torch.float32, split=False, want_layer0=False):
        x = _req(x, torch.float32, 'x')
        B, C, H, W = x.shape
        assert C == 3
        for t, shape in ((w0, (16, 147)), (b0, (16,)), (w1p, (16, 144)), (b1, (16,))):
            _req(t, torch.float32, 'stem weights')
            assert tuple(t.shape) == shape
        out = torch.empty((B, 16, H, W), dtype=dtype, device=x.device, memory_format=torch.channels_last)
        mean = (ctypes.c_double * 3)(0.485, 0.456, 0.406)
        std = (ctypes.c_double * 3)(0.229, 0.224, 0.225)
        scratch = torch.empty((B, H, W, 3), dtype=dtype, device=x.device)
        if split and dtype == torch.float32:
            am = torch.empty(1, dtype=torch.int32, device=x.device)
            if want_layer0:
                out0 = torch.empty((B, 16, H, W), dtype=dtype, device=x.device, memory_format=torch.channels_last)
                check(self._lib.spa_drn_stem_c_amax(self._ctx, _ptr(x), B, H, W, _ptr(w0), _ptr(b0), _ptr(w1p), _ptr(b1),
                                                    mean, std, _ptr(out), _ptr(out0), _ptr(scratch), _ptr(am), self._s()))
                out._spa_amax = am
                return out, out0
            check(self._lib.spa_drn_stem_d_amax(self._ctx, _ptr(x), B, H, W, _ptr(w0), _ptr(b0), _ptr(w1p), _ptr(b1),
                                                mean, std, _ptr(out), _ptr(scratch), _ptr(am), self._s()))
            out._spa_amax = am
            return out
        if want_layer0:
            assert dtype == torch.bfloat16, 'want_layer0: the split-plane float32 kernel or the bf16 kernel'
            out0 = torch.empty((B, 16, H, W), dtype=dtype, device=x.device, memory_format=torch.channels_last)
            check(self._lib.spa_drn_stem_c_bf16(self._ctx, _ptr(x), B, H, W, _ptr(w0), _ptr(b0), _ptr(w1p), _ptr(b1),
                                                mean, std, _ptr(out), _ptr(out0), _ptr(scratch), self._s()))
            return out, out0
        check(self._lib.spa_drn_stem_d(self._ctx, _ptr(x), B, H, W, _ptr(w0), _ptr(b0), _ptr(w1p), _ptr(b1),
                                       mean, std, _ptr(out), 0 if dtype == torch.float32 else 1, _ptr(scratch),
                                       self._s()))
        return out

    @staticmethod
    def layer2_planes(weight):
        assert tuple(weight.shape) == (32, 16, 3, 3)
        w = weight.detach().float()
        amax = float(w.abs().max().clamp_min(1e-30))
        t = 2.0 ** (14 - int(np.floor(np.log2(amax))))
        ws = (w.double() * t).float().reshape(32, 16, 9)
        frag = torch.zeros((2, 5, 64, 8), dtype=torch.float32, device=w.device)
        for s_ in range(5):
            for g in range(4):
                tap = 2 * s_ + g // 2
                if tap > 8:
                    continue
                c0 = 8 * (g & 1)
                for ct in range(2):
                    frag[ct, s_, g * 16:(g + 1) * 16, :] = ws[ct * 16:(ct + 1) * 16, c0:c0 + 8, tap]
        h = frag.half()
        l = (frag - h.float()).half()
        return torch.stack([h, l], dim=1).contiguous(), float(1.0 / t)
# ... 27 lines not shown
        assert x.dtype == torch.float32 and x.is_contiguous(memory_format=torch.channels_last)
        assert wt.dtype == torch.float32 and wt.is_contiguous() and tuple(wt.shape) == (Cout, 9, Cin)
        assert bias.dtype == torch.float32 and bias.is_contiguous() and bias.numel() == Cout
        Ho, Wo = (Hi + 1) // 2, (Wi + 1) // 2
        y = _out(out, (B, csplit, Ho, Wo), torch.float32, x.device)
        y2 = _out(out2, (B, Cout - csplit, Ho, Wo), torch.float32, x.device) if csplit < Cout else None
        check(self._lib.spa_conv3x3_s2_f32(self._ctx, _ptr(x), B, Hi, Wi, Cin, _ptr(wt), Cout, int(csplit), _ptr(bias),
                                           1 if relu else 0, _ptr(y), _ptr(y2), self._s()))
        return y, y2

    @staticmethod
    def small_planes(weight, proj_weight=None):
        Cout, Cin = int(weight.shape[0]), int(weight.shape[1])
        assert tuple(weight.shape[2:]) == (3, 3) and Cin in (16, 32) and Cout % 16 == 0
        w = weight.detach().float()
        amax = float(w.abs().max())
        if proj_weight is not None:
            assert tuple(proj_weight.shape[1:]) == (Cin, 1, 1) and proj_weight.shape[0] % 16 == 0 and Cin == 16
            amax = max(amax, float(proj_weight.detach().float().abs().max()))
        t = 2.0 ** (14 - int(np.floor(np.log2(max(amax, 1e-30)))))
        ws = (w.double() * t).float().reshape(Cout, Cin, 9)
        steps = 5 if Cin == 16 else 9
        frag = torch.zeros((Cout // 16, steps, 64, 8), dtype=torch.float32, device=w.device)
        for s_ in range(steps):
            for g in range(4):
                tap, c0 = (2 * s_ + g // 2, 8 * (g & 1)) if Cin == 16 else (s_, 8 * g)
                if tap > 8:
                    continue
                for ct in range(Cout // 16):
                    frag[ct, s_, g * 16:(g + 1) * 16, :] = ws[ct * 16:(ct + 1) * 16, c0:c0 + 8, tap]
        h = frag.half()
        parts = [torch.stack([h, (frag - h.float()).half()], dim=1).reshape(-1)]
        if proj_weight is not None:
            Cp = int(proj_weight.shape[0])
            ps = (proj_weight.detach().double() * t).float().reshape(Cp, Cin)
            pf = torch.zeros((Cp // 16, 64, 8), dtype=torch.float32, device=w.device)
            for g in range(2):
                for pt in range(Cp // 16):
                    pf[pt, g * 16:(g + 1) * 16, :] = ps[pt * 16:(pt + 1) * 16, 8 * g:8 * g + 8]
            ph = pf.half()
            parts.append(torch.stack([ph, (pf - ph.float()).half()], dim=1).reshape(-1))
        return torch.cat(parts).contiguous(), float(1.0 / t)

    def conv_small_f16s(self, x, wp, inv_t, bias, cout, stride=1, n_proj=0, residual=None, relu=True, amax_in=None, out=None, out2=None):
        B, Cin, H, W = x.shape
        assert x.dtype == torch.float32 and x.is_contiguous(memory_format=torch.channels_last)
        assert wp.dtype == torch.float16 and wp.is_contiguous() and bias.dtype == torch.float32 and bias.numel() == cout + n_proj
        Ho, Wo = (H + stride - 1) // stride, (W + stride - 1) // stride
        if amax_in is None:
            amax_in = self.amax(x)
        y = _out(out, (B, cout, Ho, Wo), torch.float32, x.device)
        y2 = _out(out2, (B, n_proj, Ho, Wo), torch.float32, x.device) if n_proj else None
        if residual is not None:
            assert residual.dtype == torch.float32 and residual.shape == y.shape and residual.is_contiguous(memory_format=torch.channels_last)
        am = torch.empty(1, dtype=torch.int32, device=x.device)
        check(self._lib.spa_conv_small_f16s(self._ctx, _ptr(x), B, H, W, Cin, _ptr(wp), ctypes.c_float(inv_t), int(cout), int(stride),
                                            int(n_proj), _ptr(bias), _ptr(residual), 1 if relu else 0, _ptr(amax_in), _ptr(am),
                                            _ptr(y), _ptr(y2), self._s()))
        y._spa_amax = am
        return y, y2

    def bias_act_(self, y, bias, residual=None, relu=True, track_amax=False):
        B, C, H, W = y.shape
        if track_amax and y.dtype == torch.float32:
            am = torch.empty(1, dtype=torch.int32, device=y.device)
            check(self._lib.spa_bias_act_amax(self._ctx, _ptr(y), B * H * W, C, _ptr(bias), _ptr(residual), 1 if relu else 0,
                                              _ptr(am), self._s()))
            y._spa_amax = am
            return y
        check(self._lib.spa_bias_act(self._ctx, _ptr(y), 0 if y.dtype == torch.float32 else 1, B * H * W, C,
                                     _ptr(bias), _ptr(residual), 1 if relu else 0, self._s()))
        return y

    def conv3x3_f32(self, x, wt, bias, residual=None, relu=True, dilation=1, out=None):
        B, Cin, H, W = x.shape
        Cout = wt.shape[0]
        assert x.dtype == torch.float32 and x.is_contiguous(memory_format=torch.channels_last)
        taps = wt.shape[1]
        assert wt.dtype == torch.float32 and wt.is_contiguous() and tuple(wt.shape) == (Cout, taps, Cin) and taps in (1, 9)
        assert bias.dtype == torch.float32 and bias.is_contiguous()
        y = _out(out, (B, Cout, H, W), torch.float32, x.device)
        if residual is not None:
            assert residual.dtype == torch.float32 and residual.shape == y.shape and \
                residual.is_contiguous(memory_format=torch.channels_last)
        if taps == 1:
            check(self._lib.spa_conv1x1_f32(self._ctx, _ptr(x), B, H, W, Cin, _ptr(wt), Cout, _ptr(bias),
                                            _ptr(residual), 1 if relu else 0, _ptr(y), self._s()))
        else:
            check(self._lib.spa_conv3x3_f32(self._ctx, _ptr(x), B, H, W, Cin, _ptr(wt), Cout, _ptr(bias),
                                            _ptr(residual), 1 if relu else 0, int(dilation), _ptr(y), self._s()))
        return y

    @staticmethod
    def split_planes(wt):
        Cout, taps, Cin = wt.shape
        amax = float(wt.abs().max().clamp_min(1e-30))
        t = 2.0 ** (14 - int(np.floor(np.log2(amax))))
        ws = (wt.double() * t).float()
        h = ws.half()
        l = (ws - h.float()).half()
        wt2 = torch.stack([h.view(Cout, taps, Cin // 32, 32), l.view(Cout, taps, Cin // 32, 32)], dim=3).contiguous()
        return wt2, float(1.0 / t)

    def conv3x3_f16s(self, x, wt2, inv_t, bias, residual=None, relu=True, dilation=1, amax_in=None, track_amax=True, out=None):
        B, Cin, H, W = x.shape
        Cout, taps = wt2.shape[0], wt2.shape[1]
        assert x.dtype == torch.float32 and x.is_contiguous(memory_format=torch.channels_last)
        assert wt2.dtype == torch.float16 and wt2.is_contiguous() and tuple(wt2.shape) == (Cout, taps, Cin // 32, 2, 32) and taps in (1, 9)
        assert bias.dtype == torch.float32 and bias.is_contiguous()
        y = _out(out, (B, Cout, H, W), torch.float32, x.device)
        if residual is not None:
            assert residual.dtype == torch.float32 and residual.shape == y.shape and \
                residual.is_contiguous(memory_format=torch.channels_last)
        if amax_in is None:
            amax_in = self.amax(x)
        amax_out = torch.empty(1, dtype=torch.int32, device=x.device) if track_amax else None
        if taps == 1:
            H, W = 1, H * W
            check(self._lib.spa_conv1x1_f16s(self._ctx, _ptr(x), B, H, W, Cin, _ptr(wt2), ctypes.c_float(inv_t), Cout, _ptr(bias),
                                             _ptr(residual), 1 if relu else 0, _ptr(amax_in), _ptr(amax_out), _ptr(y), self._s()))
        else:
            check(self._lib.spa_conv3x3_f16s(self._ctx, _ptr(x), B, H, W, Cin, _ptr(wt2), ctypes.c_float(inv_t), Cout, _ptr(bias),
                                             _ptr(residual), 1 if relu else 0, int(dilation), _ptr(amax_in), _ptr(amax_out),
                                             _ptr(y), self._s()))
        return y, amax_out

    def conv3x3_s2_f16s(self, x, wt2, inv_t, bias, csplit, relu=True, amax_in=None, out=None, out2=None):
        B, Cin, Hi, Wi = x.shape
        Cout = wt2.shape[0]
        assert x.dtype == torch.float32 and x.is_contiguous(memory_format=torch.channels_last)
        assert wt2.dtype == torch.float16 and wt2.is_contiguous() and tuple(wt2.shape) == (Cout, 9, Cin // 32, 2, 32)
        assert bias.dtype == torch.float32 and bias.is_contiguous() and bias.numel() == Cout
        Ho, Wo = (Hi + 1) // 2, (Wi + 1) // 2
        y = _out(out, (B, csplit, Ho, Wo), torch.float32, x.device)
        y2 = _out(out2, (B, Cout - csplit, Ho, Wo), torch.float32, x.device) if csplit < Cout else None
        if amax_in is None:
            amax_in = self.amax(x)
        amax_out = torch.empty(1, dtype=torch.int32, device=x.device)
        check(self._lib.spa_conv3x3_s2_f16s(self._ctx, _ptr(x), B, Hi, Wi, Cin, _ptr(wt2), ctypes.c_float(inv_t), Cout, int(csplit),
                                            _ptr(bias), 1 if relu else 0, _ptr(amax_in), _ptr(amax_out), _ptr(y), _ptr(y2), self._s()))
        return y, y2, amax_out

    @staticmethod
    def winograd_weights(weight, tile=2):
        if tile == 2:
            G = [[1, 0, 0], [.5, .5, .5], [.5, -.5, .5], [0, 0, 1]]
        else:
            G = [[1 / 2, 0, 0], [1 / 6, 1 / 6, 1 / 6], [1 / 6, -1 / 6, 1 / 6], [16 / 15, 8 / 15, 4 / 15],
                 [1 / 30, -1 / 15, 2 / 15], [0, 0, 1 / 2]]
        G = torch.tensor(G, dtype=torch.float64, device=weight.device)
        u = torch.einsum('ij,kcjl,ml->imkc', G, weight.detach().double(), G)
        return u.reshape(G.shape[0] ** 2, weight.shape[0], weight.shape[1]).float().contiguous()

    def conv3x3_wino_f32(self, x, u, bias, residual=None, relu=True, dilation=1, out=None, scratch=None):
        B, Cin, H, W = x.shape
        npos, Cout = u.shape[0], u.shape[1]
        assert npos in (16, 36)
        assert x.dtype == torch.float32 and x.is_contiguous(memory_format=torch.channels_last)
        assert u.dtype == torch.float32 and u.is_contiguous() and tuple(u.shape) == (npos, Cout, Cin)
        assert bias.dtype == torch.float32 and bias.is_contiguous()
        y = _out(out, (B, Cout, H, W), torch.float32, x.device)
        if residual is not None:
            assert residual.dtype == torch.float32 and residual.shape == y.shape and \
                residual.is_contiguous(memory_format=torch.channels_last)
        tiles, fn = (self._lib.spa_wino_tiles, self._lib.spa_conv3x3_wino_f32) if npos == 16 else \
            (self._lib.spa_wino4_tiles, self._lib.spa_conv3x3_wino4_f32)
        T = int(tiles(B, H, W, int(dilation)))
        v, m = _scratch(scratch, (npos, T, Cin), (npos, T, Cout), x.device)
        check(fn(self._ctx, _ptr(x), B, H, W, Cin, _ptr(u), Cout, _ptr(bias), _ptr(residual),
                 1 if relu else 0, int(dilation), _ptr(v), _ptr(m), _ptr(y), self._s()))
        return y

    @staticmethod
    def winograd_weights_split(weight):
        u = Engine.winograd_weights(weight, 4)
        Cout, Cin = u.shape[1], u.shape[2]
        amax = u.abs().amax(dim=(1, 2)).double().clamp_min(1e-30)
        t = torch.exp2(14.0 - torch.floor(torch.log2(amax)))
        us = (u.double() * t.view(36, 1, 1)).float()
        h = us.half()
        l = (us - h.float()).half()
        u2 = torch.stack([h.view(36, Cout, Cin // 32, 32), l.view(36, Cout, Cin // 32, 32)], dim=3).contiguous()
        p = torch.tensor([4, 4, 4, 3, 3, 4], dtype=torch.float64, device=u.device)
        cs = (torch.exp2(p.view(6, 1) + p.view(1, 6)).reshape(36) / t).float().cpu().numpy().copy()
        return u2, cs

    def amax(self, x):
        assert x.dtype == torch.float32 and x.numel() % 4 == 0
        a = torch.empty(1, dtype=torch.int32, device=x.device)
        check(self._lib.spa_amax_f32(self._ctx, _ptr(x), x.numel(), _ptr(a), self._s()))
        return a

    def conv3x3_wino_f16s(self, x, u2, cs, bias, residual=None, relu=True, dilation=1, amax_in=None, track_amax=True, _keep=None,
                          out=None, scratch=None):
        B, Cin, H, W = x.shape
        Cout = u2.shape[1]
        assert x.dtype == torch.float32 and x.is_contiguous(memory_format=torch.channels_last)
        assert u2.dtype == torch.float16 and u2.is_contiguous() and tuple(u2.shape) == (36, Cout, Cin // 32, 2, 32)
        assert bias.dtype == torch.float32 and bias.is_contiguous() and cs.dtype == np.float32 and cs.shape == (36,)
        y = _out(out, (B, Cout, H, W), torch.float32, x.device)
        if residual is not None:
            assert residual.dtype == torch.float32 and residual.shape == y.shape and \
                residual.is_contiguous(memory_format=torch.channels_last)
        if amax_in is None:
            amax_in = self.amax(x)
        amax_out = torch.empty(1, dtype=torch.int32, device=x.device) if track_amax else None
        T = int(self._lib.spa_wino4_tiles(B, H, W, int(dilation)))
        v, m = _scratch(scratch, (36, T, Cin), (36, T, Cout), x.device)
        if _keep is not None:
            _keep['v'], _keep['m'] = v, m
        check(self._lib.spa_conv3x3_wino4_f16s(self._ctx, _ptr(x), B, H, W, Cin, _ptr(u2), cs.ctypes.data, Cout, _ptr(bias),
                                               _ptr(residual), 1 if relu else 0, int(dilation), _ptr(amax_in), _ptr(amax_out),
                                               _ptr(v), _ptr(m), _ptr(y), self._s()))
        return y, amax_out

    def conv3x3_bf16(self, x, wt, bias, residual=None, relu=True, dilation=1):
        B, Cin, H, W = x.shape
        Cout = wt.shape[0]
        assert x.dtype == torch.bfloat16 and x.is_contiguous(memory_format=torch.channels_last)
        assert wt.dtype == torch.bfloat16 and wt.is_contiguous() and tuple(wt.shape) == (Cout, 9, Cin)
        assert bias.dtype == torch.float32 and bias.is_contiguous()
        y = torch.empty((B, Cout, H, W), dtype=torch.bfloat16, device=x.device, memory_format=torch.channels_last)
        if residual is not None:
            assert residual.dtype == torch.bfloat16 and residual.shape == y.shape and \
                residual.is_contiguous(memory_format=torch.channels_last)
        check(self._lib.spa_conv3x3_bf16(self._ctx, _ptr(x), B, H, W, Cin, _ptr(wt), Cout, _ptr(bias),
                                         _ptr(residual), 1 if relu else 0, int(dilation), _ptr(y), self._s()))
        return y

    def conv_bf16_light(self, x, wt, bias, residual=None, relu=True, stride=1, dilation=1, out=None):
        B, Cin, H, W = x.shape
        Cout, taps = wt.shape[0], wt.shape[1]
        assert x.dtype == torch.bfloat16 and x.is_contiguous(memory_format=torch.channels_last)
        assert wt.dtype == torch.bfloat16 and wt.is_contiguous() and tuple(wt.shape) == (Cout, taps, Cin) and taps in (1, 9)
        assert bias.dtype == torch.float32 and bias.is_contiguous()
        Ho, Wo = (H + stride - 1) // stride, (W + stride - 1) // stride
        y = _out(out, (B, Cout, Ho, Wo), torch.bfloat16, x.device)
        if residual is not None:
            assert residual.dtype == torch.bfloat16 and residual.shape == y.shape and \
                residual.is_contiguous(memory_format=torch.channels_last)
        check(self._lib.spa_conv_bf16_light(self._ctx, _ptr(x), B, H, W, Cin, _ptr(wt), int(taps), int(stride), Cout, _ptr(bias),
                                            _ptr(residual), 1 if relu else 0, int(dilation), _ptr(y), self._s()))
        return y

    def resize_bicubic_u8(self, src, shape):
        src = _req(src, torch.uint8, 'src')
        B, H, W, C = src.shape
        h, w = int(shape[0]), int(shape[1])
        out = torch.empty((B, C, h, w), dtype=torch.float32, device=src.device)
        check(self._lib.spa_resize_bicubic_u8(self._ctx, _ptr(src), B, H, W, C, h, w, _ptr(out), self._s()))
        return out

    def resize_cvcubic_u8(self, src, shape):
        src = _req(src, torch.uint8, 'src')
        B, H, W, C = src.shape
        h, w = int(shape[0]), int(shape[1])
        out = torch.empty((B, C, h, w), dtype=torch.float32, device=src.device)
        check(self._lib.spa_resize_cvcubic_u8(self._ctx, _ptr(src), B, H, W, C, h, w, _ptr(out), self._s()))
        return out

    def resize_u8(self, src, shape, backend='pil'):
        return self.resize_cvcubic_u8(src, shape) if backend == 'cv2' else self.resize_bicubic_u8(src, shape)

    def rgb2lab(self, rgb, ratio=0.1):
        rgb = _req(rgb, torch.float32, 'rgb')
        B, C, H, W = rgb.shape
        assert C == 3
        lab = torch.empty_like(rgb)
        check(self._lib.spa_rgb2lab(self._ctx, _ptr(rgb), B, H, W, ratio, _ptr(lab), self._s()))
        return lab

    def slic_core(self, lab, n_segments, max_iter=10, want_centres=False):
        lab = _req(lab, torch.float32, 'lab')
        B, C, H, W = lab.shape
        assert C == 3
        labels = torch.empty((B, H, W), dtype=torch.int32, device=lab.device)
        centres = None
        if want_centres:
            nC = _lib.make_plan(H, W, n_segments).n_centroids
            centres = torch.empty((B, nC, 6), dtype=torch.float32, device=lab.device)
        check(self._lib.spa_slic_core(self._ctx, _ptr(lab), B, H, W, n_segments, max_iter,
                                      _ptr(labels), _ptr(centres), self._s()))
        return (labels, centres) if want_centres else labels

    def enforce_connectivity(self, labels, min_size, max_size):
        labels = _req(labels, torch.int32, 'labels')
        B, H, W = labels.shape
        out = torch.empty_like(labels)
        n_labels = torch.empty((B,), dtype=torch.int32, device=labels.device)
        check(self._lib.spa_enforce_connectivity(self._ctx, _ptr(labels), B, H, W, min_size, max_size,
                                                 _ptr(out), _ptr(n_labels), self._s()))
        return out, n_labels

    def slic(self, rgb, n_segments, compactness=10.0, max_iter=10):
        rgb = _req(rgb, torch.float32, 'rgb')
        B, C, H, W = rgb.shape
        assert C == 3
        labels = torch.empty((B, H, W), dtype=torch.int32, device=rgb.device)
        n_labels = torch.empty((B,), dtype=torch.int32, device=rgb.device)
        check(self._lib.spa_slic(self._ctx, _ptr(rgb), B, H, W, n_segments, compactness, max_iter,
                                 _ptr(labels), _ptr(n_labels), self._s()))
        return labels, n_labels

    def slic_u8(self, rgb, n_segments, compactness=10.0, max_iter=10):
        rgb = _req(rgb, torch.float32, 'rgb')
        B, C, H, W = rgb.shape
        assert C == 3
        labels = torch.empty((B, H, W), dtype=torch.int32, device=rgb.device)
        n_labels = torch.empty((B,), dtype=torch.int32, device=rgb.device)
        check(self._lib.spa_slic_u8(self._ctx, _ptr(rgb), B, H, W, n_segments, float(compactness), max_iter,
                                    _ptr(labels), _ptr(n_labels), self._s()))
        return labels, n_labels

    def rgb2lab_u8_f64(self, rgb, compactness=10.0):
        rgb = _req(rgb, torch.float32, 'rgb')
        B, C, H, W = rgb.shape
        lab = torch.empty((B, 3, H, W), dtype=torch.float64, device=rgb.device)
        check(self._lib.spa_rgb2lab_u8_f64(self._ctx, _ptr(rgb), B, H, W, 1.0 / float(compactness), _ptr(lab), self._s()))
        return lab

    def slic_core_f64(self, lab, n_segments, max_iter=10, want_centres=False):
        lab = _req(lab, torch.float64, 'lab')
        B, C, H, W = lab.shape
        labels = torch.empty((B, H, W), dtype=torch.int32, device=lab.device)
        cen = None
        if want_centres:
            cen = torch.empty((B, _lib.make_plan(H, W, n_segments).n_centroids, 6), dtype=torch.float64, device=lab.device)
        check(self._lib.spa_slic_core_f64(self._ctx, _ptr(lab), B, H, W, n_segments, max_iter, _ptr(labels),
                                          _ptr(cen), self._s()))
        return (labels, cen) if want_centres else labels

    def felzenszwalb(self, rgb, scale=300.0, sigma=0.8, min_size=20, uint8_image=False, out=None):
        rgb = _req(rgb, torch.float32, 'rgb')
        B, C, H, W = rgb.shape
        assert C == 3
        if out is not None:
            labels, n_labels = _req(out[0], torch.int32, 'labels'), _req(out[1], torch.int32, 'n_labels')
            assert labels.shape == (B, H, W) and n_labels.shape == (B,)
        else:
            labels = torch.empty((B, H, W), dtype=torch.int32, device=rgb.device)
            n_labels = torch.empty((B,), dtype=torch.int32, device=rgb.device)
        fn = self._lib.spa_felzenszwalb_u8 if uint8_image else self._lib.spa_felzenszwalb
        check(fn(self._ctx, _ptr(rgb), B, H, W, scale, sigma, min_size, _ptr(labels), _ptr(n_labels), self._s()))
        return labels, n_labels

    def overlap_refine(self, labels, road, max_labels, threshold):
        labels = _req(labels, torch.int32, 'labels')
        road = _req(road, torch.uint8, 'road')
        B = labels.shape[0]
        npix = labels[0].numel()
        assert road.shape == labels.shape
        out = torch.empty(labels.shape, dtype=torch.uint8, device=labels.device)
        check(self._lib.spa_overlap_refine(self._ctx, _ptr(labels), _ptr(road), B, npix, int(max_labels),
                                           float(threshold), _ptr(out), self._s()))
        return out

    def segment_offsets(self, n_labels):
        n_labels = _req(n_labels, torch.int32, 'n_labels')
        B = n_labels.numel()
        off = torch.empty((B + 1,), dtype=torch.int32, device=n_labels.device)
        check(self._lib.spa_segment_offsets(self._ctx, _ptr(n_labels), B, _ptr(off), self._s()))
        return off

    def segment_stats(self, labels, offsets, ncap, prior_params=None, want_centroid=True):
        labels = _req(labels, torch.int32, 'labels')
        offsets = _req(offsets, torch.int32, 'offsets')
# ... 727 lines not shown
```

Measured before the change: 443.7.

## Pad Winograd scratch plane pitch and map tiles per wavefront in F(4x4) transforms

Adds a per-plane pitch to the F(4x4,3x3) Winograd V/M scratch buffers so the 36 transform planes can be padded apart, likely to avoid cache or channel aliasing between planes. The GEMM and conv1x1 raw launchers take explicit plane strides. Input and output transform kernels gain a wave-mode indexing where each 64-lane wavefront handles one tile, decoded once via readfirstlane with magic-number division instead of 64-bit per-lane division. Both modes are on by default, can be switched off with environment variables, and change the scratch allocation API.

```diff
diff --git a/include/spalign.h b/include/spalign.h
--- a/include/spalign.h
+++ b/include/spalign.h
@@ -44,6 +44,7 @@
 int spa_ws_generation(spa_ctx *ctx);
 int spa_debug_set(spa_ctx *ctx, int32_t key, int32_t value);
 int spa_wino4_tile_decode(int32_t B, int32_t H, int32_t W, int32_t dilation, int32_t interleaved, int64_t t, int32_t *out);
+int spa_wino4_tile_decode_wave(int32_t B, int32_t H, int32_t W, int32_t dilation, int32_t interleaved, int64_t t, int32_t *out);
 int spa_debug_lds_probe(spa_ctx *ctx, float *out, int32_t n_wg, int32_t steps, int32_t mode, void *stream);
 
 int spa_drn_normalise(spa_ctx *ctx, const float *x, int32_t B, int32_t H, int32_t W, void *out,
@@ -80,16 +81,18 @@
                          void *stream);
 
 int64_t spa_wino4_tiles(int32_t B, int32_t H, int32_t W, int32_t dilation);
+int64_t spa_wino4_pitch(int32_t B, int32_t H, int32_t W, int32_t dilation, int32_t C);
+int64_t spa_wino4_scratch_pitch(spa_ctx *ctx, int32_t B, int32_t H, int32_t W, int32_t dilation, int32_t C);
 int spa_conv3x3_wino4_f32(spa_ctx *ctx, const float *x, int32_t B, int32_t H, int32_t W, int32_t Cin,
                           const float *u, int32_t Cout, const float *bias, const float *residual,
-                          int32_t relu, int32_t dilation, float *v_scratch, float *m_scratch, float *y,
-                          void *stream);
+                          int32_t relu, int32_t dilation, float *v_scratch, float *m_scratch, int64_t v_pitch,
+                          int64_t m_pitch, float *y, void *stream);
 
 int spa_amax_f32(spa_ctx *ctx, const float *x, int64_t n, void *amax, void *stream);
 int spa_conv3x3_wino4_f16s(spa_ctx *ctx, const float *x, int32_t B, int32_t H, int32_t W, int32_t Cin,
                            const void *u2, const float *cs, int32_t Cout, const float *bias, const float *residual,
                            int32_t relu, int32_t dilation, const void *amax_in, void *amax_out, void *v_scratch,
-                           float *m_scratch, float *y, void *stream);
+                           float *m_scratch, int64_t v_pitch, int64_t m_pitch, float *y, void *stream);
 
 int spa_conv3x3_f16s(spa_ctx *ctx, const float *x, int32_t B, int32_t H, int32_t W, int32_t Cin,
                      const void *wt2, float inv_t, int32_t Cout, const float *bias, const float *residual,
diff --git a/superpixel-align_amd/_lib.py b/superpixel-align_amd/_lib.py
--- a/superpixel-align_amd/_lib.py
+++ b/superpixel-align_amd/_lib.py
@@ -63,7 +63,9 @@
     'spa_wino_tiles': (ctypes.c_int64, [c_i32, c_i32, c_i32, c_i32]),
     'spa_conv3x3_wino_f32': (ctypes.c_int, [c_p, c_p, c_i32, c_i32, c_i32, c_i32, c_p, c_i32, c_p, c_p, c_i32, c_i32, c_p, c_p, c_p, c_p]),
     'spa_wino4_tiles': (ctypes.c_int64, [c_i32, c_i32, c_i32, c_i32]),
-    'spa_conv3x3_wino4_f32': (ctypes.c_int, [c_p, c_p, c_i32, c_i32, c_i32, c_i32, c_p, c_i32, c_p, c_p, c_i32, c_i32, c_p, c_p, c_p, c_p]),
+    'spa_wino4_pitch': (ctypes.c_int64, [c_i32, c_i32, c_i32, c_i32, c_i32]),
+    'spa_wino4_scratch_pitch': (ctypes.c_int64, [c_p, c_i32, c_i32, c_i32, c_i32, c_i32]),
+    'spa_conv3x3_wino4_f32': (ctypes.c_int, [c_p, c_p, c_i32, c_i32, c_i32, c_i32, c_p, c_i32, c_p, c_p, c_i32, c_i32, c_p, c_p, c_i64, c_i64, c_p, c_p]),
     'spa_conv3x3_f16s': (ctypes.c_int, [c_p, c_p, c_i32, c_i32, c_i32, c_i32, c_p, c_f32, c_i32, c_p, c_p, c_i32, c_i32, c_p, c_p, c_p, c_p]),
     'spa_conv1x1_f16s': (ctypes.c_int, [c_p, c_p, c_i32, c_i32, c_i32, c_i32, c_p, c_f32, c_i32, c_p, c_p, c_i32, c_p, c_p, c_p, c_p]),
     'spa_conv3x3_s2_f16s': (ctypes.c_int, [c_p, c_p, c_i32, c_i32, c_i32, c_i32, c_p, c_f32, c_i32, c_i32, c_p, c_i32, c_p, c_p, c_p, c_p, c_p]),
@@ -76,12 +78,13 @@
     'spa_drn_layer2_f32': (ctypes.c_int, [c_p, c_p, c_i32, c_i32, c_i32, c_p, c_p, c_p, c_p]),
     'spa_conv3x3_s2_f32': (ctypes.c_int, [c_p, c_p, c_i32, c_i32, c_i32, c_i32, c_p, c_i32, c_i32, c_p, c_i32, c_p, c_p, c_p]),
     'spa_amax_f32': (ctypes.c_int, [c_p, c_p, c_i64, c_p, c_p]),
-    'spa_conv3x3_wino4_f16s': (ctypes.c_int, [c_p, c_p, c_i32, c_i32, c_i32, c_i32, c_p, c_p, c_i32, c_p, c_p, c_i32, c_i32, c_p, c_p, c_p, c_p, c_p, c_p]),
+    'spa_conv3x3_wino4_f16s': (ctypes.c_int, [c_p, c_p, c_i32, c_i32, c_i32, c_i32, c_p, c_p, c_i32, c_p, c_p, c_i32, c_i32, c_p, c_p, c_p, c_p, c_i64, c_i64, c_p, c_p]),
     'spa_resize_bicubic_u8': (ctypes.c_int, [c_p, c_p, c_i32, c_i32, c_i32, c_i32, c_i32, c_i32, c_p, c_p]),
     'spa_resize_cvcubic_u8': (ctypes.c_int, [c_p, c_p, c_i32, c_i32, c_i32, c_i32, c_i32, c_i32, c_p, c_p]),
     'spa_debug_peek': (ctypes.c_int, [c_p, ctypes.c_int, ctypes.c_size_t, ctypes.c_size_t, c_p]),
     'spa_debug_set': (ctypes.c_int, [c_p, ctypes.c_int32, ctypes.c_int32]),
     'spa_wino4_tile_decode': (ctypes.c_int, [c_i32, c_i32, c_i32, c_i32, c_i32, c_i64, ctypes.POINTER(ctypes.c_int32)]),
+    'spa_wino4_tile_decode_wave': (ctypes.c_int, [c_i32, c_i32, c_i32, c_i32, c_i32, c_i64, ctypes.POINTER(ctypes.c_int32)]),
     'spa_ws_generation': (ctypes.c_int, [c_p]),
     'spa_debug_lds_probe': (ctypes.c_int, [c_p, c_p, c_i32, c_i32, c_i32, c_p]),
     'spa_slic_make_plan':(ctypes.c_int, [c_i32, c_i32, c_i32, ctypes.POINTER(SlicPlan)]),
diff --git a/superpixel-align_amd/csrc/spa_common.h b/superpixel-align_amd/csrc/spa_common.h
--- a/superpixel-align_amd/csrc/spa_common.h
+++ b/superpixel-align_amd/csrc/spa_common.h
@@ -120,6 +120,8 @@
     int dbg_slic_ldsx;
     int convp_on;
     int wino_operands;
+    int wino_pad;
+    int wino_wave;
     int convs2_on;
     int convs2_attr_done;
     int rs_key[4], rs_ks[2];
diff --git a/superpixel-align_amd/csrc/spa_conv32.hip b/superpixel-align_amd/csrc/spa_conv32.hip
--- a/superpixel-align_amd/csrc/spa_conv32.hip
+++ b/superpixel-align_amd/csrc/spa_conv32.hip
@@ -525,9 +525,10 @@
 }
 
 int conv1x1_f32_raw(spa_ctx *ctx, const float *x, long long rows, int32_t Cin, const float *wt, int32_t Cout,
-                    float *y, void *stream, int zcount)
+                    float *y, void *stream, int zcount, long long xz, long long yz)
 {
     SPA_ARG(rows > 0 && rows % 256 == 0 && rows / 256 < (1ll << 31) && zcount >= 1);
+    SPA_ARG(xz >= rows * Cin && yz >= rows * Cout && xz % 4 == 0 && yz % 4 == 0);
     return conv_f32_launch<1>(ctx, x, 1, (int32_t)(rows / 256), 256, Cin, wt, Cout, nullptr, nullptr, 0, 1, y, stream, true,
-                              zcount, rows * Cin, (long long)Cout * Cin, rows * Cout);
-}
+                              zcount, xz, (long long)Cout * Cin, yz);
+}
diff --git a/superpixel-align_amd/csrc/spa_ctx.hip b/superpixel-align_amd/csrc/spa_ctx.hip
--- a/superpixel-align_amd/csrc/spa_ctx.hip
+++ b/superpixel-align_amd/csrc/spa_ctx.hip
@@ -42,6 +42,8 @@
     ctx->convp_on = getenv("SPA_CONVP") ? atoi(getenv("SPA_CONVP")) != 0 : 1;
     ctx->convs2_on = 1;
     ctx->wino_operands = 2;
+    ctx->wino_wave = getenv("SPA_WINO_WAVE") ? atoi(getenv("SPA_WINO_WAVE")) != 0 : 1;
+    ctx->wino_pad = getenv("SPA_WINO_PAD") ? atoi(getenv("SPA_WINO_PAD")) != 0 : 1;
     SPA_HIP(hipMalloc((void **)&ctx->d_status, 32 * sizeof(uint32_t)));
     SPA_HIP(hipMemset(ctx->d_status, 0, 32 * sizeof(uint32_t)));
     *out = ctx;
@@ -312,8 +314,11 @@
 
 extern "C" int spa_debug_set(spa_ctx *ctx, int32_t key, int32_t value)
 {
-    SPA_ARG(ctx && (key == 1 || key == 2 || key == 3 || key == 4) && (value == 0 || value == 1 || (key == 4 && value == 2)));
+    SPA_ARG(ctx && key >= 1 && key <= 6);
+    SPA_ARG(value == 0 || value == 1 || (key == 4 && value == 2));
     if (key == 1) ctx->convp_on = value;
+    else if (key == 6) ctx->wino_wave = value;
+    else if (key == 5) ctx->wino_pad = value;
     else if (key == 4) ctx->wino_operands = value;
     else if (key == 3) ctx->convs2_on = value;
     else {
diff --git a/superpixel-align_amd/csrc/spa_gemm16.hip b/superpixel-align_amd/csrc/spa_gemm16.hip
--- a/superpixel-align_amd/csrc/spa_gemm16.hip
+++ b/superpixel-align_amd/csrc/spa_gemm16.hip
@@ -347,9 +347,10 @@
 int gemm_f16x3_tile(int32_t Cout) { return Cout % 256 == 0 ? 256 : 128; }
 
 int gemm_f16x3_raw(spa_ctx *ctx, const float *x, long long rows, int32_t Cin, const void *wt, int32_t Cout, float *y,
-                   void *stream, int zcount, const void *amax, int planes)
+                   void *stream, int zcount, const void *amax, int planes, long long xz, long long yz)
 {
     SPA_ARG(ctx && x && wt && y && amax && rows > 0 && rows % 256 == 0 && rows < (1ll << 31) && zcount == 36);
+    SPA_ARG(xz >= rows * Cin && yz >= rows * Cout && xz % 4 == 0 && yz % 4 == 0);
     SPA_ARG(Cin % 32 == 0 && Cout % 128 == 0);
     SPA_ARG(((uintptr_t)x % 16) == 0 && ((uintptr_t)wt % 16) == 0 && ((uintptr_t)y % 16) == 0);
     hipStream_t s = spa_stream(stream);
@@ -374,17 +375,17 @@
                 ctx->gemm16p_attr_done = 1;
             }
             hipLaunchKernelGGL((k_gemm_f16x3_stag<256, 256, true>), dim3((unsigned)grid), dim3(G16_THREADS), lds, s, (const char *)x, (const char *)wt, y,
-                               (int)rows, Cin, Cout, ntiles, (int)total, zcount, rows * Cin, (long long)Cout * Cin, rows * Cout, (const unsigned *)amax);
+                               (int)rows, Cin, Cout, ntiles, (int)total, zcount, xz, (long long)Cout * Cin, yz, (const unsigned *)amax);
         } else
         hipLaunchKernelGGL((k_gemm_f16x3_stag<256, 256>), dim3((unsigned)grid), dim3(G16_THREADS), lds, s, (const char *)x, (const char *)wt, y,
-                           (int)rows, Cin, Cout, ntiles, (int)total, zcount, rows * Cin, (long long)Cout * Cin, rows * Cout, (const unsigned *)amax);
+                           (int)rows, Cin, Cout, ntiles, (int)total, zcount, xz, (long long)Cout * Cin, yz, (const unsigned *)amax);
     } else {
         if (!ctx->gemm16_attr_done) {
             SPA_HIP(hipFuncSetAttribute((const void *)k_gemm_f16x3<128, 128>, hipFuncAttributeMaxDynamicSharedMemorySize, 2 * 256 * 128));
             ctx->gemm16_attr_done = 1;
         }
         hipLaunchKernelGGL((k_gemm_f16x3<128, 128>), dim3((unsigned)grid), dim3(G16_THREADS), lds, s, (const char *)x, (const char *)wt, y,
-                           (int)rows, Cin, Cout, ntiles, (int)total, zcount, rows * Cin, (long long)Cout * Cin, rows * Cout, (const unsigned *)amax);
+                           (int)rows, Cin, Cout, ntiles, (int)total, zcount, xz, (long long)Cout * Cin, yz, (const unsigned *)amax);
     }
     SPA_LAUNCH_CHECK();
     return SPA_OK;
diff --git a/superpixel-align_amd/csrc/spa_wino.hip b/superpixel-align_amd/csrc/spa_wino.hip
--- a/superpixel-align_amd/csrc/spa_wino.hip
+++ b/superpixel-align_amd/csrc/spa_wino.hip
@@ -2,7 +2,7 @@
 #include "spa_wino_dev.h"
 
 int conv1x1_f32_raw(spa_ctx *ctx, const float *x, long long rows, int32_t Cin, const float *wt, int32_t Cout,
-                    float *y, void *stream, int zcount);
+                    float *y, void *stream, int zcount, long long xz, long long yz);
 
 extern "C" int spa_wino4_tile_decode(int32_t B, int32_t H, int32_t W, int32_t dilation, int32_t interleaved, int64_t t, int32_t *out)
 {
@@ -15,6 +15,18 @@
     return SPA_OK;
 }
 
+extern "C" int spa_wino4_tile_decode_wave(int32_t B, int32_t H, int32_t W, int32_t dilation, int32_t interleaved, int64_t t, int32_t *out)
+{
+    SPA_ARG(out && B > 0 && H > 0 && W > 0 && dilation >= 1);
+    WinoGeom g;
+    wino4_geom(B, H, W, dilation, &g);
+    SPA_ARG(t >= 0 && t < g.T && g.T < (1ll << 31));
+    g.interleaved = interleaved != 0;
+    wino_wave_setup(&g);
+    wino_tile_wave(g, (unsigned)t, out[0], out[1], out[2], out[3], out[4]);
+    return SPA_OK;
+}
+
 
 __device__ __forceinline__ float4 f4add(float4 a, float4 b) { return make_float4(a.x + b.x, a.y + b.y, a.z + b.z, a.w + b.w); }
 __device__ __forceinline__ float4 f4sub(float4 a, float4 b) { return make_float4(a.x - b.x, a.y - b.y, a.z - b.z, a.w - b.w); }
@@ -24,6 +36,36 @@
     const long long nb = gridDim.x, id = blockIdx.x;
     const long long q = nb / 8, rem = nb % 8, xcd = id % 8, idx = id / 8;
     return (xcd < rem ? xcd * (q + 1) : rem * (q + 1) + (xcd - rem) * q) + idx;
+}
+
+__device__ __forceinline__ bool wino_thread_wave(const WinoGeom &g, int c2, int VN, WinoDiv wdiv, long long &t, int &c, int &b, int &sy,
+                                                 int &sx, int &ty, int &tx)
+{
+    const unsigned w = (unsigned)__builtin_amdgcn_readfirstlane((int)((unsigned)wino_block() * 4u + (threadIdx.x >> 6)));
+    const unsigned wpt = (unsigned)c2 >> 6;
+    const unsigned tt = wino_div(w, wdiv);
+    if ((long long)tt >= g.T) return false;
+    t = tt;
+    c = (int)((w - tt * wpt) * 64u + (threadIdx.x & 63)) * VN;
+    wino_tile_wave(g, tt, b, sy, sx, ty, tx);
+    return true;
+}
+__device__ __forceinline__ bool wino_thread_lane(const WinoGeom &g, int c2, int VN, long long &t, int &c, int &b, int &sy, int &sx,
+                                                 int &ty, int &tx)
+{
+    const long long id = wino_block() * 256 + threadIdx.x;
+    if (id >= g.T * c2) return false;
+    t = id / c2;
+    c = (int)(id - t * c2) * VN;
+    wino_tile(g, t, b, sy, sx, ty, tx);
+    return true;
+}
+template <bool WAVE>
+__device__ __forceinline__ bool wino_thread(const WinoGeom &g, int c2, int VN, WinoDiv wdiv, long long &t, int &c, int &b, int &sy, int &sx,
+                                            int &ty, int &tx)
+{
+    if constexpr (WAVE) return wino_thread_wave(g, c2, VN, wdiv, t, c, b, sy, sx, ty, tx);
+    else return wino_thread_lane(g, c2, VN, t, c, b, sy, sx, ty, tx);
 }
 
 
@@ -117,6 +159,8 @@
     const int hs = (H + d - 1) / d, ws = (W + d - 1) / d;
     g->th = (hs + 1) / 2; g->tw = (ws + 1) / 2;
     g->T = (long long)B * d * d * g->th * g->tw;
+    g->wave = 0;
+    g->row = g->sub = g->rows = wino_div_make(1);
 }
 
 extern "C" int64_t spa_wino_tiles(int32_t B, int32_t H, int32_t W, int32_t dilation)
@@ -147,7 +191,7 @@
         hipLaunchKernelGGL(k_wino_in, dim3((unsigned)((n + 255) / 256)), dim3(256), 0, s, x, v_scratch, g, Cin, Tpad);
     }
     {
-        int rc = conv1x1_f32_raw(ctx, v_scratch, Tpad, Cin, u, Cout, m_scratch, stream, 16);
+        int rc = conv1x1_f32_raw(ctx, v_scratch, Tpad, Cin, u, Cout, m_scratch, stream, 16, Tpad * Cin, Tpad * Cout);
         if (rc != SPA_OK) return rc;
     }
     {
@@ -166,18 +210,10 @@
 
 
 
-template <typename V, bool PLANES = false>
-__global__ __launch_bounds__(256) void k_wino4_in(const float *__restrict__ X, float *__restrict__ Vout, WinoGeom g, int C,
-                                                  long long Tpad, const unsigned *__restrict__ amax = nullptr)
-{
-    constexpr int VN = sizeof(V) / 4;
-    const int c2 = C / VN;
-    const long long id = wino_block() * 256 + threadIdx.x;
-    if (id >= g.T * c2) return;
-    const long long t = id / c2;
-    const int c = (int)(id - t * c2) * VN;
-    int b, sy, sx, ty, tx;
-    wino_tile(g, t, b, sy, sx, ty, tx);
+template <typename V, bool PLANES>
+__device__ __forceinline__ void wino4_in_tile(const float *__restrict__ X, float *__restrict__ Vout, const WinoGeom &g, int C, long long vz,
+                                              const unsigned *__restrict__ amax, long long t, int c, int b, int sy, int sx, int ty, int tx)
+{
     V r[6][6];
 #pragma unroll
     for (int a = 0; a < 6; ++a) {
@@ -205,34 +241,37 @@
                 const unsigned l0 = wino_split_l(o[i].x, o[i].y, sc, h0), l1 = wino_split_l(o[i].z, o[i].w, sc, h1);
                 const bool odd = (c >> 2) & 1;
                 const unsigned r0 = wino_lane_swap(odd ? h0 : l0), r1 = wino_lane_swap(odd ? h1 : l1);
-                float *chunk = Vout + ((long long)(i * 6 + j) * Tpad + t) * C + (c & ~7);
+                float *chunk = Vout + (long long)(i * 6 + j) * vz + t * C + (c & ~7);
                 *((uint4 *)chunk + (odd ? 1 : 0)) = odd ? make_uint4(r0, r1, l0, l1) : make_uint4(h0, h1, r0, r1);
             } else {
-                *(V *)(Vout + ((long long)(i * 6 + j) * Tpad + t) * C + c) = o[i];
+                *(V *)(Vout + (long long)(i * 6 + j) * vz + t * C + c) = o[i];
             }
         }
     }
 }
 
+template <typename V, bool PLANES = false, bool WAVE = false>
+__global__ __launch_bounds__(256) void k_wino4_in(const float *__restrict__ X, float *__restrict__ Vout, WinoGeom g, int C,
+                                                  long long vz, WinoDiv wdiv, const unsigned *__restrict__ amax = nullptr)
+{
+    constexpr int VN = sizeof(V) / 4;
+    const int c2 = C / VN;
+    long long t;
+    int c, b, sy, sx, ty, tx;
+    if (wino_thread<WAVE>(g, c2, VN, wdiv, t, c, b, sy, sx, ty, tx)) wino4_in_tile<V, PLANES>(X, Vout, g, C, vz, amax, t, c, b, sy, sx, ty, tx);
+}
+
 template <int HAS_RES, typename V>
-__global__ __launch_bounds__(256) void k_wino4_out(const float *__restrict__ M, float *__restrict__ Y,
-                                                   const float *__restrict__ bias, const float *__restrict__ R,
-                                                   WinoGeom g, int K, long long Tpad, int relu)
-{
-    constexpr int VN = sizeof(V) / 4;
-    const int k2 = K / VN;
-    const long long id = wino_block() * 256 + threadIdx.x;
-    if (id >= g.T * k2) return;
-    const long long t = id / k2;
-    const int k = (int)(id - t * k2) * VN;
-    int b, sy, sx, ty, tx;
-    wino_tile(g, t, b, sy, sx, ty, tx);
+__device__ __forceinline__ void wino4_out_tile(const float *__restrict__ M, float *__restrict__ Y, const float *__restrict__ bias,
+                                               const float *__restrict__ R, const WinoGeom &g, int K, long long mz, int relu,
+                                               long long t, int k, int b, int sy, int sx, int ty, int tx)
+{
     V s[4][6];
 #pragma unroll
     for (int j = 0; j < 6; ++j) {
         V col[6];
 #pragma unroll
-        for (int i = 0; i < 6; ++i) col[i] = *(const V *)(M + ((long long)(i * 6 + j) * Tpad + t) * K + k);
+        for (int i = 0; i < 6; ++i) col[i] = *(const V *)(M + (long long)(i * 6 + j) * mz + t * K + k);
         V o[4];
         wino4_at(col, o);
 #pragma unroll
@@ -258,6 +297,18 @@
     }
 }
 
+template <int HAS_RES, typename V, bool WAVE>
+__global__ __launch_bounds__(256) void k_wino4_out(const float *__restrict__ M, float *__restrict__ Y,
+                                                   const float *__restrict__ bias, const float *__restrict__ R,
+                                                   WinoGeom g, int K, long long mz, WinoDiv wdiv, int relu)
+{
+    constexpr int VN = sizeof(V) / 4;
+    const int k2 = K / VN;
+    long long t;
+    int k, b, sy, sx, ty, tx;
+    if (wino_thread<WAVE>(g, k2, VN, wdiv, t, k, b, sy, sx, ty, tx)) wino4_out_tile<HAS_RES, V>(M, Y, bias, R, g, K, mz, relu, t, k, b, sy, sx, ty, tx);
+}
+
 
 __global__ __launch_bounds__(256) void k_amax(const float4 *__restrict__ x, long long n4, unsigned *__restrict__ amax)
 {
@@ -277,54 +328,61 @@
     }
 }
 
-template <int HAS_RES, typename V = float4>
+template <int HAS_RES, typename V>
+__device__ __forceinline__ unsigned wino4_out_s_tile(const float *__restrict__ M, float *__restrict__ Y, const float *__restrict__ bias,
+                                                     const float *__restrict__ R, const WinoGeom &g, int K, long long mz, int relu,
+                                                     const WinoScale &cs, const unsigned *__restrict__ amax_in,
+                                                     long long t, int k, int b, int sy, int sx, int ty, int tx)
+{
+    unsigned mx = 0;
+    const float inv = wino_pow2(wino_amax_exp(*amax_in) - 14);
+    V s[4][6];
+#pragma unroll
+    for (int j = 0; j < 6; ++j) {
+        V col[6];
+#pragma unroll
+        for (int i = 0; i < 6; ++i)
+            col[i] = (cs.c[i * 6 + j] * inv) * wino_nt_load((const V *)(M + (long long)(i * 6 + j) * mz + t * K + k));
+        V o[4];
+        wino4_at(col, o);
+#pragma unroll
+        for (int i = 0; i < 4; ++i) s[i][j] = o[i];
+    }
+    const V bv = *(const V *)(bias + k);
+#pragma unroll
+    for (int i = 0; i < 4; ++i) {
+        const int y = sy + (4 * ty + i) * g.d;
+        V o[4];
+        wino4_at(s[i], o);
+        if (y >= g.H) continue;
+#pragma unroll
+        for (int j = 0; j < 4; ++j) {
+            const int x = sx + (4 * tx + j) * g.d;
+            if (x >= g.W) continue;
+            V v = o[j] + bv;
+            const long long off = (((long long)b * g.H + y) * g.W + x) * K + k;
+            if (HAS_RES) v = v + *(const V *)(R + off);
+            if (relu) v = wino_relu(v);
+            *(V *)(Y + off) = v;
+            mx = max(mx, wino_absmax_bits(v));
+        }
+    }
+    return mx;
+}
+
+template <int HAS_RES, bool WAVE, typename V = float4>
 __global__ __launch_bounds__(256, 2) void k_wino4_out_s(const float *__restrict__ M, float *__restrict__ Y,
                                                      const float *__restrict__ bias, const float *__restrict__ R,
-                                                     WinoGeom g, int K, long long Tpad, int relu, WinoScale cs,
+                                                     WinoGeom g, int K, long long mz, WinoDiv wdiv, int relu, WinoScale cs,
                                                      const unsigned *__restrict__ amax_in, unsigned *__restrict__ amax_out)
 {
     constexpr int VN = sizeof(V) / 4;
     const int k2 = K / VN;
-    const long long id = wino_block() * 256 + threadIdx.x;
     unsigned mx = 0;
-    if (id < g.T * k2) {
-        const long long t = id / k2;
-        const int k = (int)(id - t * k2) * VN;
-        int b, sy, sx, ty, tx;
-        wino_tile(g, t, b, sy, sx, ty, tx);
-        const float inv = wino_pow2(wino_amax_exp(*amax_in) - 14);
-        V s[4][6];
-#pragma unroll
-        for (int j = 0; j < 6; ++j) {
-            V col[6];
-#pragma unroll
-            for (int i = 0; i < 6; ++i)
-                col[i] = (cs.c[i * 6 + j] * inv) * wino_nt_load((const V *)(M + ((long long)(i * 6 + j) * Tpad + t) * K + k));
-            V o[4];
-            wino4_at(col, o);
-#pragma unroll
-            for (int i = 0; i < 4; ++i) s[i][j] = o[i];
-        }
-        const V bv = *(const V *)(bias + k);
-#pragma unroll
-        for (int i = 0; i < 4; ++i) {
-            const int y = sy + (4 * ty + i) * g.d;
-            V o[4];
-            wino4_at(s[i], o);
-            if (y >= g.H) continue;
-#pragma unroll
-            for (int j = 0; j < 4; ++j) {
-                const int x = sx + (4 * tx + j) * g.d;
-                if (x >= g.W) continue;
-                V v = o[j] + bv;
-                const long long off = (((long long)b * g.H + y) * g.W + x) * K + k;
-                if (HAS_RES) v = v + *(const V *)(R + off);
-                if (relu) v = wino_relu(v);
-                *(V *)(Y + off) = v;
-                mx = max(mx, wino_absmax_bits(v));
-            }
-        }
-    }
+    long long t;
+    int k, b, sy, sx, ty, tx;
+    if (wino_thread<WAVE>(g, k2, VN, wdiv, t, k, b, sy, sx, ty, tx))
+        mx = wino4_out_s_tile<HAS_RES, V>(M, Y, bias, R, g, K, mz, relu, cs, amax_in, t, k, b, sy, sx, ty, tx);
     if (amax_out) {
         for (int o = 32; o > 0; o >>= 1) mx = max(mx, (unsigned)__shfl_xor((int)mx, o));
         if ((threadIdx.x & 63) == 0 && mx > *(volatile unsigned *)amax_out) atomicMax(amax_out, mx);
@@ -338,47 +396,78 @@
     return (g.T + 255) / 256 * 256;
 }
 
+#define WINO_PLANE_PAD_BYTES (64 * 1024)
+extern "C" int64_t spa_wino4_pitch(int32_t B, int32_t H, int32_t W, int32_t dilation, int32_t C)
+{
+    return spa_wino4_tiles(B, H, W, dilation) * C + WINO_PLANE_PAD_BYTES / 4;
+}
+extern "C" int64_t spa_wino4_scratch_pitch(spa_ctx *ctx, int32_t B, int32_t H, int32_t W, int32_t dilation, int32_t C)
+{
+    if (!ctx) return -1;
+    return ctx->wino_pad ? spa_wino4_pitch(B, H, W, dilation, C) : spa_wino4_tiles(B, H, W, dilation) * C;
+}
+
+#define WINO_LAUNCH(wave, kwave, klane, ...) \
+    do { if (wave) hipLaunchKernelGGL(kwave, __VA_ARGS__); else hipLaunchKernelGGL(klane, __VA_ARGS__); } while (0)
+
+static void wino4_launch_geom(spa_ctx *ctx, int B, int H, int W, int d, int Cin, int Cout, WinoGeom *gi, WinoGeom *go, WinoDiv *wi, WinoDiv *wo)
+{
+    WinoGeom g;
+    wino4_geom(B, H, W, d, &g);
+    g.interleaved = ctx->wino_operands >= 1 && wino_interleave(d);
+    wino_wave_setup(&g);
+    *gi = *go = g;
+    for (int side = 0; side < 2; ++side) {
+        WinoGeom *p = side ? go : gi;
+        const int c4 = (side ? Cout : Cin) / 4;
+        const bool fits = c4 % 64 == 0 && g.T * (c4 / 64) < (1ll << 31) - 4;
+        p->wave = ctx->wino_wave && fits;
+        *(side ? wo : wi) = wino_div_make(fits ? (unsigned)(c4 / 64) : 1u);
+    }
+}
+
 extern "C" int spa_conv3x3_wino4_f32(spa_ctx *ctx, const float *x, int32_t B, int32_t H, int32_t W, int32_t Cin,
                                      const float *u, int32_t Cout, const float *bias, const float *residual,
-                                     int32_t relu, int32_t dilation, float *v_scratch, float *m_scratch, float *y,
-                                     void *stream)
+                                     int32_t relu, int32_t dilation, float *v_scratch, float *m_scratch, int64_t v_pitch,
+                                     int64_t m_pitch, float *y, void *stream)
 {
     SPA_ARG(ctx && x && u && bias && y && v_scratch && m_scratch && B > 0 && H > 0 && W > 0 && dilation >= 1);
     SPA_ARG(Cin % 32 == 0 && Cout % 64 == 0);
     SPA_ARG((((uintptr_t)x | (uintptr_t)u | (uintptr_t)y | (uintptr_t)bias | (uintptr_t)residual | (uintptr_t)v_scratch |
               (uintptr_t)m_scratch) % 16) == 0);
     hipStream_t s = spa_stream(stream);
-    WinoGeom g;
-    wino4_geom(B, H, W, dilation, &g);
-    g.interleaved = ctx->wino_operands >= 1 && wino_interleave(dilation);
+    WinoGeom g, go;
+    WinoDiv wi, wo;
+    wino4_launch_geom(ctx, B, H, W, dilation, Cin, Cout, &g, &go, &wi, &wo);
     const long long Tpad = (g.T + 255) / 256 * 256;
     SPA_ARG(g.T * (Cin > Cout ? Cin : Cout) / 2 < (1ll << 31) * 256);
+    SPA_ARG(v_pitch >= Tpad * Cin && m_pitch >= Tpad * Cout && v_pitch % 64 == 0 && m_pitch % 64 == 0);
     {
         SpaProfScope prof_(ctx, PROF_WINO_IN, s);
         const long long n = g.T * (Cin / 4);
-        hipLaunchKernelGGL((k_wino4_in<float4, false>), dim3((unsigned)((n + 255) / 256)), dim3(256), 0, s, x, v_scratch, g, Cin, Tpad,
-                           (const unsigned *)nullptr);
-    }
-    {
-        int rc = conv1x1_f32_raw(ctx, v_scratch, Tpad, Cin, u, Cout, m_scratch, stream, 36);
+        WINO_LAUNCH(g.wave, (k_wino4_in<float4, false, true>), (k_wino4_in<float4, false, false>), dim3((unsigned)((n + 255) / 256)), dim3(256), 0, s, x, v_scratch, g, Cin,
+                           (long long)v_pitch, wi, (const unsigned *)nullptr);
+    }
+    {
+        int rc = conv1x1_f32_raw(ctx, v_scratch, Tpad, Cin, u, Cout, m_scratch, stream, 36, v_pitch, m_pitch);
         if (rc != SPA_OK) return rc;
     }
     {
         SpaProfScope prof_(ctx, PROF_WINO_OUT, s);
         const long long n = g.T * (Cout / 4);
         if (residual)
-            hipLaunchKernelGGL((k_wino4_out<1, float4>), dim3((unsigned)((n + 255) / 256)), dim3(256), 0, s, (const float *)m_scratch, y,
-                               bias, residual, g, Cout, Tpad, relu);
+            WINO_LAUNCH(go.wave, (k_wino4_out<1, float4, true>), (k_wino4_out<1, float4, false>), dim3((unsigned)((n + 255) / 256)), dim3(256), 0, s, (const float *)m_scratch, y,
+                               bias, residual, go, Cout, (long long)m_pitch, wo, relu);
         else
-            hipLaunchKernelGGL((k_wino4_out<0, float4>), dim3((unsigned)((n + 255) / 256)), dim3(256), 0, s, (const float *)m_scratch, y,
-                               bias, residual, g, Cout, Tpad, relu);
+            WINO_LAUNCH(go.wave, (k_wino4_out<0, float4, true>), (k_wino4_out<0, float4, false>), dim3((unsigned)((n + 255) / 256)), dim3(256), 0, s, (const float *)m_scratch, y,
+                               bias, residual, go, Cout, (long long)m_pitch, wo, relu);
     }
     SPA_LAUNCH_CHECK();
     return SPA_OK;
 }
 
 int gemm_f16x3_raw(spa_ctx *ctx, const float *x, long long rows, int32_t Cin, const void *wt, int32_t Cout, float *y,
-                   void *stream, int zcount, const void *amax, int planes);
+                   void *stream, int zcount, const void *amax, int planes, long long xz, long long yz);
 int gemm_f16x3_tile(int32_t Cout);
 
 extern "C" int spa_amax_f32(spa_ctx *ctx, const float *x, int64_t n, void *amax, void *stream)
@@ -396,19 +485,21 @@
 extern "C" int spa_conv3x3_wino4_f16s(spa_ctx *ctx, const float *x, int32_t B, int32_t H, int32_t W, int32_t Cin,
                                       const void *u2, const float *cs, int32_t Cout, const float *bias,
                                       const float *residual, int32_t relu, int32_t dilation, const void *amax_in,
-                                      void *amax_out, void *v_scratch, float *m_scratch, float *y, void *stream)
+                                      void *amax_out, void *v_scratch, float *m_scratch, int64_t v_pitch, int64_t m_pitch,
+                                      float *y, void *stream)
 {
     SPA_ARG(ctx && x && u2 && cs && bias && y && v_scratch && m_scratch && amax_in && B > 0 && H > 0 && W > 0 && dilation >= 1);
     SPA_ARG(Cin % 32 == 0 && Cout % 128 == 0);
     SPA_ARG((((uintptr_t)x | (uintptr_t)u2 | (uintptr_t)y | (uintptr_t)bias | (uintptr_t)residual | (uintptr_t)v_scratch |
               (uintptr_t)m_scratch) % 16) == 0);
     hipStream_t s = spa_stream(stream);
-    WinoGeom g;
-    wino4_geom(B, H, W, dilation, &g);
-    g.interleaved = ctx->wino_operands >= 1 && wino_interleave(dilation);
+    WinoGeom g, go;
+    WinoDiv wi, wo;
+    wino4_launch_geom(ctx, B, H, W, dilation, Cin, Cout, &g, &go, &wi, &wo);
     const int planes = ctx->wino_operands >= 2 && gemm_f16x3_tile(Cout) == 256 && Cout >= 512;
     const long long Tpad = (g.T + 255) / 256 * 256;
     SPA_ARG(g.T * (Cin > Cout ? Cin : Cout) / 4 < (1ll << 31) * 256);
+    SPA_ARG(v_pitch >= Tpad * Cin && m_pitch >= Tpad * Cout && v_pitch % 64 == 0 && m_pitch % 64 == 0);
     WinoScale sc;
     for (int i = 0; i < 36; ++i) sc.c[i] = cs[i];
     if (amax_out) spa_zero_word(amax_out, s);
@@ -416,25 +507,25 @@
         SpaProfScope prof_(ctx, PROF_WINO_IN, s);
         const long long n = g.T * (Cin / 4);
         if (planes)
-            hipLaunchKernelGGL((k_wino4_in<float4, true>), dim3((unsigned)((n + 255) / 256)), dim3(256), 0, s, x, (float *)v_scratch, g, Cin, Tpad,
-                               (const unsigned *)amax_in);
+            WINO_LAUNCH(g.wave, (k_wino4_in<float4, true, true>), (k_wino4_in<float4, true, false>), dim3((unsigned)((n + 255) / 256)), dim3(256), 0, s, x, (float *)v_scratch, g, Cin,
+                               (long long)v_pitch, wi, (const unsigned *)amax_in);
         else
-            hipLaunchKernelGGL((k_wino4_in<float4, false>), dim3((unsigned)((n + 255) / 256)), dim3(256), 0, s, x, (float *)v_scratch, g, Cin, Tpad,
-                               (const unsigned *)nullptr);
-    }
-    {
-        int rc = gemm_f16x3_raw(ctx, (const float *)v_scratch, Tpad, Cin, u2, Cout, m_scratch, stream, 36, amax_in, planes);
+            WINO_LAUNCH(g.wave, (k_wino4_in<float4, false, true>), (k_wino4_in<float4, false, false>), dim3((unsigned)((n + 255) / 256)), dim3(256), 0, s, x, (float *)v_scratch, g, Cin,
+                               (long long)v_pitch, wi, (const unsigned *)nullptr);
+    }
+    {
+        int rc = gemm_f16x3_raw(ctx, (const float *)v_scratch, Tpad, Cin, u2, Cout, m_scratch, stream, 36, amax_in, planes, v_pitch, m_pitch);
         if (rc != SPA_OK) return rc;
     }
     {
         SpaProfScope prof_(ctx, PROF_WINO_OUT, s);
         const long long n = g.T * (Cout / 4);
         if (residual)
-            hipLaunchKernelGGL((k_wino4_out_s<1>), dim3((unsigned)((n + 255) / 256)), dim3(256), 0, s, (const float *)m_scratch, y,
-                               bias, residual, g, Cout, Tpad, relu, sc, (const unsigned *)amax_in, (unsigned *)amax_out);
+            WINO_LAUNCH(go.wave, (k_wino4_out_s<1, true>), (k_wino4_out_s<1, false>), dim3((unsigned)((n + 255) / 256)), dim3(256), 0, s, (const float *)m_scratch, y,
+                               bias, residual, go, Cout, (long long)m_pitch, wo, relu, sc, (const unsigned *)amax_in, (unsigned *)amax_out);
         else
-            hipLaunchKernelGGL((k_wino4_out_s<0>), dim3((unsigned)((n + 255) / 256)), dim3(256), 0, s, (const float *)m_scratch, y,
-                               bias, residual, g, Cout, Tpad, relu, sc, (const unsigned *)amax_in, (unsigned *)amax_out);
+            WINO_LAUNCH(go.wave, (k_wino4_out_s<0, true>), (k_wino4_out_s<0, false>), dim3((unsigned)((n + 255) / 256)), dim3(256), 0, s, (const float *)m_scratch, y,
+                               bias, residual, go, Cout, (long long)m_pitch, wo, relu, sc, (const unsigned *)amax_in, (unsigned *)amax_out);
     }
     SPA_LAUNCH_CHECK();
     return SPA_OK;
diff --git a/superpixel-align_amd/csrc/spa_wino_dev.h b/superpixel-align_amd/csrc/spa_wino_dev.h
--- a/superpixel-align_amd/csrc/spa_wino_dev.h
+++ b/superpixel-align_amd/csrc/spa_wino_dev.h
@@ -1,7 +1,18 @@
 #pragma once
 #include "spa_common.h"
 
-struct WinoGeom { int B, H, W, d, th, tw; long long T; int interleaved; };
+struct WinoDiv { unsigned m, s; };
+struct WinoGeom { int B, H, W, d, th, tw; long long T; int interleaved; int wave; WinoDiv row, sub, rows; };
+static inline WinoDiv wino_div_make(unsigned d)
+{
+    unsigned l = 0;
+    while ((1ull << l) < d) ++l;
+    WinoDiv q;
+    q.s = 31 + l;
+    q.m = (unsigned)(((1ull << q.s) + d - 1) / d);
+    return q;
+}
+__host__ __device__ __forceinline__ unsigned wino_div(unsigned n, WinoDiv q) { return (unsigned)(((unsigned long long)n * q.m) >> q.s); }
 typedef float wino_v4 __attribute__((ext_vector_type(4)));
 __device__ __forceinline__ float4 wino_nt_load(const float4 *p) { const wino_v4 v = __builtin_nontemporal_load((const wino_v4 *)p); return make_float4(v[0], v[1], v[2], v[3]); }
 
@@ -21,6 +32,29 @@
     sx = (int)(t % g.d); t /= g.d;
     sy = (int)(t % g.d);
     b = (int)(t / g.d);
+}
+
+__host__ __device__ __forceinline__ void wino_tile_wave(const WinoGeom &g, unsigned t, int &b, int &sy, int &sx, int &ty, int &tx)
+{
+    const unsigned rw = g.interleaved ? (unsigned)(g.tw * g.d) : (unsigned)g.tw;
+    unsigned q = wino_div(t, g.row);
+    const unsigned gx = t - q * rw;
+    t = q;
+    q = wino_div(t, g.rows);
+    ty = (int)(t - q * (unsigned)g.th);
+    t = q;
+    if (g.interleaved) {
+        tx = (int)wino_div(gx, g.sub);
+        sx = (int)(gx - (unsigned)tx * (unsigned)g.d);
+    } else {
+        tx = (int)gx;
+        q = wino_div(t, g.sub);
+        sx = (int)(t - q * (unsigned)g.d);
+        t = q;
+    }
+    q = wino_div(t, g.sub);
+    sy = (int)(t - q * (unsigned)g.d);
+    b = (int)q;
 }
 
 __device__ __forceinline__ unsigned wino_absmax_bits(float4 v) { return max(max(__float_as_uint(v.x) & 0x7fffffffu, __float_as_uint(v.y) & 0x7fffffffu), max(__float_as_uint(v.z) & 0x7fffffffu, __float_as_uint(v.w) & 0x7fffffffu)); }
@@ -95,4 +129,13 @@
     const int hs = (H + d - 1) / d, ws = (W + d - 1) / d;
     g->th = (hs + 3) / 4; g->tw = (ws + 3) / 4;
     g->T = (long long)B * d * d * g->th * g->tw;
+    g->wave = 0;
+    g->row = g->sub = g->rows = wino_div_make(1);
 }
+
+static inline void wino_wave_setup(WinoGeom *g)
+{
+    g->row = wino_div_make((unsigned)(g->interleaved ? g->tw * g->d : g->tw));
+    g->sub = wino_div_make((unsigned)g->d);
+    g->rows = wino_div_make((unsigned)g->th);
+}
diff --git a/superpixel-align_amd/engine.py b/superpixel-align_amd/engine.py
--- a/superpixel-align_amd/engine.py
+++ b/superpixel-align_amd/engine.py
@@ -29,14 +29,20 @@
     return out
 
 
-def _scratch(scratch, v_shape, m_shape, device):
-    if scratch is None:
-        return (torch.empty(v_shape, dtype=torch.float32, device=device), torch.empty(m_shape, dtype=torch.float32, device=device))
-    v, m = scratch
-    for t, shape in ((v, v_shape), (m, m_shape)):
-        if not (t.is_cuda and t.dtype == torch.float32 and tuple(t.shape) == tuple(shape) and t.is_contiguous()):
-            raise SpalignError('scratch must be two contiguous float32 CUDA tensors of shapes %s, %s' % (v_shape, m_shape))
-    return v, m
+def _plane_buffer(given, shape, pitch, device):
+    npos, T, C = shape
+    if given is None:
+        return torch.empty((npos, pitch), dtype=torch.float32, device=device), pitch
+    if given.is_cuda and given.dtype == torch.float32 and given.is_contiguous():
+        if tuple(given.shape) == tuple(shape):
+            return given, T * C
+        if given.dim() == 2 and given.shape[0] == npos and given.shape[1] >= T * C and given.shape[1] % 64 == 0:
+            return given, int(given.shape[1])
+    raise SpalignError('scratch must be contiguous float32 CUDA tensors of shape %s, or (%d, pitch >= %d)' % (tuple(shape), npos, T * C))
+
+
+def _planes(t, shape):
+    return t if t.dim() == 3 else t.as_strided(shape, (t.stride(0), shape[2], 1))
 
 
 class Engine(object):
@@ -370,7 +376,10 @@
         u = torch.einsum('ij,kcjl,ml->imkc', G, weight.detach().double(), G)
         return u.reshape(G.shape[0] ** 2, weight.shape[0], weight.shape[1]).float().contiguous()
 
-    def conv3x3_wino_f32(self, x, u, bias, residual=None, relu=True, dilation=1, out=None, scratch=None):
+    def wino4_pitch(self, B, H, W, dilation, C):
+        return int(self._lib.spa_wino4_scratch_pitch(self._ctx, int(B), int(H), int(W), int(dilation), int(C)))
+
+    def conv3x3_wino_f32(self, x, u, bias, residual=None, relu=True, dilation=1, out=None, scratch=None, _keep=None):
         B, Cin, H, W = x.shape
         npos, Cout = u.shape[0], u.shape[1]
         assert npos in (16, 36)
@@ -384,9 +393,19 @@
         tiles, fn = (self._lib.spa_wino_tiles, self._lib.spa_conv3x3_wino_f32) if npos == 16 else \
             (self._lib.spa_wino4_tiles, self._lib.spa_conv3x3_wino4_f32)
         T = int(tiles(B, H, W, int(dilation)))
-        v, m = _scratch(scratch, (npos, T, Cin), (npos, T, Cout), x.device)
-        check(fn(self._ctx, _ptr(x), B, H, W, Cin, _ptr(u), Cout, _ptr(bias), _ptr(residual),
-                 1 if relu else 0, int(dilation), _ptr(v), _ptr(m), _ptr(y), self._s()))
+        given = scratch if scratch is not None else (None, None)
+        v, vp = _plane_buffer(given[0], (npos, T, Cin), T * Cin if npos == 16 else self.wino4_pitch(B, H, W, dilation, Cin), x.device)
+        m, mp = _plane_buffer(given[1], (npos, T, Cout), T * Cout if npos == 16 else self.wino4_pitch(B, H, W, dilation, Cout), x.device)
+        if npos == 16 and (vp, mp) != (T * Cin, T * Cout):
+            raise SpalignError('the F(2x2,3x3) scratch is dense')
+        if _keep is not None:
+            _keep['v'], _keep['m'], _keep['v_raw'], _keep['m_raw'] = _planes(v, (npos, T, Cin)), _planes(m, (npos, T, Cout)), v, m
+        if npos == 16:
+            check(fn(self._ctx, _ptr(x), B, H, W, Cin, _ptr(u), Cout, _ptr(bias), _ptr(residual),
+                     1 if relu else 0, int(dilation), _ptr(v), _ptr(m), _ptr(y), self._s()))
+        else:
+            check(fn(self._ctx, _ptr(x), B, H, W, Cin, _ptr(u), Cout, _ptr(bias), _ptr(residual),
+                     1 if relu else 0, int(dilation), _ptr(v), _ptr(m), vp, mp, _ptr(y), self._s()))
         return y
 
     @staticmethod
@@ -424,12 +443,14 @@
             amax_in = self.amax(x)
         amax_out = torch.empty(1, dtype=torch.int32, device=x.device) if track_amax else None
         T = int(self._lib.spa_wino4_tiles(B, H, W, int(dilation)))
-        v, m = _scratch(scratch, (36, T, Cin), (36, T, Cout), x.device)
+        given = scratch if scratch is not None else (None, None)
+        v, vp = _plane_buffer(given[0], (36, T, Cin), self.wino4_pitch(B, H, W, dilation, Cin), x.device)
+        m, mp = _plane_buffer(given[1], (36, T, Cout), self.wino4_pitch(B, H, W, dilation, Cout), x.device)
         if _keep is not None:
-            _keep['v'], _keep['m'] = v, m
+            _keep['v'], _keep['m'], _keep['v_raw'], _keep['m_raw'] = _planes(v, (36, T, Cin)), _planes(m, (36, T, Cout)), v, m
         check(self._lib.spa_conv3x3_wino4_f16s(self._ctx, _ptr(x), B, H, W, Cin, _ptr(u2), cs.ctypes.data, Cout, _ptr(bias),
                                                _ptr(residual), 1 if relu else 0, int(dilation), _ptr(amax_in), _ptr(amax_out),
-                                               _ptr(v), _ptr(m), _ptr(y), self._s()))
+                                               _ptr(v), _ptr(m), vp, mp, _ptr(y), self._s()))
         return y, amax_out
 
     def conv3x3_bf16(self, x, wt, bias, residual=None, relu=True, dilation=1):
```

New measurement: 451.6 (median of 6 runs). 1.02x the previous value.
